# zhizdev/mvdfusion

Hardware: AMD Instinct MI355X
Metric: denoising-steps/sec (higher is better)
Workload: dtype f16x3 (f16 MFMA operands split hi+lo, 3 partial products, fp32 accumulate); 1 GPU; BASELINE.json configs[1]: V=4 views x 256^2 images (32x32 latents), D=1, 50-step DDIM (eta 1), cfg 2.5, SD1.x UNet 320ch + 10 view-aligned transformers + GridAttn, random-init (deterministic fill) weights; views=4, latent=32, depth_samples=1, parallelism=single GPU, CFG pair batched as 2V, hipgraph=True, gemm_tuning=mvdfusion_amd/tuned/gemm_f16.json: 426 problems; 0 problems tuned in this run

## Files before the change

### include/mvd_hip.h

```cpp
#ifndef MVD_HIP_H
#define MVD_HIP_H
#include <stddef.h>
#include <stdint.h>
#ifdef __cplusplus
extern "C" {
#endif

typedef void* mvd_stream_t;

#define MVD_VERSION 100
#define MVD_PREC_X1 1
#define MVD_PREC_X3 3
#define MVD_PREC_X4 4

int mvd_version(void);
const char* mvd_last_error(void);
int mvd_operand_format(void);

size_t mvd_packed_weight_bytes(int N, int K);
int mvd_pack_linear_weight(const float* w, int N, int K, int ldw, int geglu, float scale, void* packed,
                           mvd_stream_t stream);
int mvd_pack_linear_weight_t(const float* wt, int N, int K, int ldw, float scale, void* packed, mvd_stream_t stream);
int mvd_pack_conv3x3_weight(const float* w, int Cout, int Cin, int cin_pad, float scale, void* packed,
                            mvd_stream_t stream);
// ... 22 lines not shown
  int start_after;
  int consumer;
} mvd_prefetch_item;

typedef struct mvd_gemm_desc {
  int M, N, K;
  const void* A;
  int lda;
  int a_mode;
  int B, Hin, Win, Cin, Hout, Wout, stride, upsample;
  int no_pad_tl;
  const void* Wp;
  int b_mode;
  int ldb;
  float acc_scale;
  int prec;
  int epi;
  int act;
  float* out;
  int ldo;
  void* out_sp;
  int ldp;
  int n_store;
  const float* bias;
  const float* bias_b;
  int rows_per_batch;
  int ldbb;
  const float* colscale;
  const float* res;
  int ldr;
  void *q_hi, *q_lo, *k_hi, *k_lo, *vt_hi, *vt_lo;
  int heads, dhead, L, Lpad;
  float qscale;
  int splitk;
  float* workspace;
  size_t workspace_elems;
  int cfg;
  long long* gn_stats;
  int gn_hw, gn_groups;
  float* rs_out;
  int* rs_count;
  int rs_ld;
  const float* ln_stats;
  const int* ln_count;
  const float* ln_colsum;
  int ln_ld, ln_dim;
  float ln_eps;
  void* gna_out_sp;
  const float* gna_gamma;
  const float* gna_beta;
  float gna_eps;
  int gna_flags;
  const float* cat_b;
  int cat_cb;
  void* cat_raw_sp;
  const float* acc_scale_dev;
  const struct mvd_prefetch_item_s* pf_items;
  int pf_n;
  int tap_mode;
  const void* A2;
  int lda2, Cin2;
} mvd_gemm_desc;
#define MVD_TAPS_FULL 0
#define MVD_TAPS_UP4 1
#define MVD_TAPS_CENTRE_TAIL 2
#define MVD_GNA_SILU 1
#define MVD_GNA_ROUND_F16 2
#define MVD_GNA_OUT_UNUSED 4

int mvd_gemm(const mvd_gemm_desc* d, mvd_stream_t stream);
int mvd_gemm_cfg_supported(const mvd_gemm_desc* d, int cfg);

int mvd_split_planes(const float* x, void* sp, size_t rows, int cols, int ldx, int ldp, mvd_stream_t stream);
int mvd_split_planes_scaled(const float* x, void* sp, size_t rows, int cols, int ldx, int ldp, const float* scale_dev, mvd_stream_t stream);

int mvd_gemv(const float* W, const float* bias, const float* x, float* y, int M, int N, int K, int ldx, int ldy,
             int act_in, int act_out, mvd_stream_t stream);

int mvd_groupnorm_chunks(int HW);
int mvd_groupnorm_nhwc(const float* x, void* y_sp, const float* gamma, const float* beta, int B, int HW, int C,
                       int groups, float eps, int silu, double* ws, size_t ws_elems, mvd_stream_t stream);
int mvd_groupnorm_from_stats(const float* x, void* y_sp, const float* gamma, const float* beta, const long long* stats, int B, int HW,
                             int C, int groups, float eps, int silu, mvd_stream_t stream);
int mvd_softmax_rows(const float* x, void* y_sp, int rows, int cols, int ldx, float scale, float out_scale,
                     mvd_stream_t stream);

int mvd_layernorm(const float* x, void* y_sp, float* y_f32, const float* w, const float* b, int rows, int C, float eps,
                  int w_plus_one, mvd_stream_t stream);
int mvd_layernorm_groups(const float* x, void* y_sp, float* y_f32, const float* w, const float* b, int ldw, int rows, int rows_per_group,
                         int C, float eps, int w_plus_one, mvd_stream_t stream);

size_t mvd_attn_qk_plane_elems(int B, int heads, int L, int dhead);
size_t mvd_attn_vt_plane_elems(int B, int heads, int L, int dhead);
int mvd_attn_lpad(int L);
int mvd_attention(const void* q_hi, const void* q_lo, const void* k_hi, const void* k_lo, const void* vt_hi,
                  const void* vt_lo, void* out_sp, int ldo, int B, int heads, int L, int Lkeys, int dhead, int prec,
                  mvd_stream_t stream);

int mvd_pixel_cross_attn(const float* q, const float* k, const float* v, void* out_sp, int P, int D, int heads,
                         int dhead, mvd_stream_t stream);

int mvd_unet_input(const float* x, const float* input_latents, void* out_sp, int V, int S, int cpad, int cfg,
                   mvd_stream_t stream);
int mvd_unet_input_scenes(const float* x, const float* input_latents, void* out_sp, int nscene, int V, int S, int cpad, int cfg,
                          mvd_stream_t stream);
int mvd_concat_channels(const float* a, int Ca, const float* b, int Cb, float* out, void* out_sp, int rows, long long* gn_stats,
                        int gn_hw, int gn_groups, mvd_stream_t stream);
int mvd_concat_groupnorm_fits(int Ca, int Cb, int hw, int groups);
int mvd_concat_groupnorm(const float* a, int Ca, const float* b, int Cb, float* out, void* raw_sp, void* y_sp, const float* gamma,
                         const float* beta, long long* gn_stats, int B, int hw, int groups, float eps, int silu, mvd_stream_t stream);
int mvd_area_pool(const float* vol, void* out_sp, int B, int S, int D, int C, int factor, int ldp, mvd_stream_t stream);
int mvd_fill_zero(float* p, size_t n, mvd_stream_t stream);

#define MVD_STEP_STRIDE 8
int mvd_timestep_embedding(const float* steps, const int* iter, const float* freqs, float* out, int dim,
                           mvd_stream_t stream);
int mvd_timestep_embedding_scenes(const float* steps, const int* iter, const float* freqs, float* out, int dim, int nscene,
                                  int steps_scene_stride, mvd_stream_t stream);
int mvd_advance_iter(int* iter, mvd_stream_t stream);

#define MVD_CAM_RECORD 20
#define MVD_TOKEN_DIM 723
#define MVD_TOKEN_LD 736
int mvd_zembed(const float* lat, const float* w, const float* b, float* feat, int N, int S, mvd_stream_t stream);
int mvd_gridattn_tokens(const float* x, const float* depth_noise, const float* steps, const int* iter,
                        const float* grid_lin ,
                        const float* feat, const float* in_feat, const float* cams, const float* in_cam,
                        void* tokens_sp, int V, int q0, int Vq, int S, int D, float depth_scale, float depth_shift,
                        mvd_stream_t stream);
int mvd_gridattn_tokens_scenes(const float* x, const float* depth_noise, const float* steps, const int* iter, const float* grid_lin,
                               const float* feat, const float* in_feat, const float* cams, const float* in_cam, void* tokens_sp,
                               int nscene, int V, int q0, int Vq, int S, int D, float depth_scale, float depth_shift,
                               mvd_stream_t stream);
int mvd_gridattn_tokens_scenes_t(const float* x, const float* depth_noise, const float* steps, const int* iter, const float* grid_lin,
                                 const float* feat, const float* in_feat, const float* cams, const float* in_cam, void* tokens_sp,
                                 int nscene, int V, int q0, int Vq, int S, int D, float depth_scale, float depth_shift,
                                 int steps_scene_stride, mvd_stream_t stream);
int mvd_gridattn_fused_slots(void);
size_t mvd_gridattn_fused_stream_bytes(void);
size_t mvd_gridattn_fused_vec_floats(void);
int mvd_gridattn_fused(const float* x, const float* depth_noise, const float* steps, const int* iter, const float* grid_lin,
                       const float* feat, const float* in_feat, const float* cams, const float* in_cam, const void* wstream,
                       const float* vecs, void* pooled_sp, int V, int q0, int Vq, int S, int D, float depth_scale,
                       float depth_shift, int prec ,
                       mvd_stream_t stream);
int mvd_gridattn_fused_scenes(const float* x, const float* depth_noise, const float* steps, const int* iter, const float* grid_lin,
                              const float* feat, const float* in_feat, const float* cams, const float* in_cam, const void* wstream,
                              const float* vecs, void* pooled_sp, int nscene, int V, int q0, int Vq, int S, int D, float depth_scale,
                              float depth_shift, int prec, mvd_stream_t stream);
int mvd_gridattn_fused_scenes_t(const float* x, const float* depth_noise, const float* steps, const int* iter, const float* grid_lin,
                                const float* feat, const float* in_feat, const float* cams, const float* in_cam, const void* wstream,
                                const float* vecs, void* pooled_sp, int nscene, int V, int q0, int Vq, int S, int D, float depth_scale,
                                float depth_shift, int prec, int steps_scene_stride, int vecs_scene_stride, mvd_stream_t stream);
int mvd_gridattn_tokens_window(const float* x, const float* depth_noise, const float* steps, const int* iter, const float* grid_lin,
                               const float* feat, const float* in_feat, const float* cams, const float* in_cam, void* tokens_sp,
                               int nscene, int V, int q0, int Vq, int S, int D, float depth_scale, float depth_shift,
                               int steps_scene_stride, int window, mvd_stream_t stream);
int mvd_gridattn_fused_window(const float* x, const float* depth_noise, const float* steps, const int* iter, const float* grid_lin,
                              const float* feat, const float* in_feat, const float* cams, const float* in_cam, const void* wstream,
                              const float* vecs, void* pooled_sp, int nscene, int V, int q0, int Vq, int S, int D, float depth_scale,
                              float depth_shift, int prec, int steps_scene_stride, int vecs_scene_stride, int window,
                              mvd_stream_t stream);
int mvd_view_mha(const float* qkv, void* out_sp, int Nseq, int V, int heads, int dhead,
                 mvd_stream_t stream);
int mvd_view_pool(const float* x, const float* w, const float* b, void* out_sp, int Nseq, int V, int C,
                  mvd_stream_t stream);

int mvd_cfg_ddim_update(const float* eps_nhwc, int ldc, float* x, float* x0, float* eps_out,
                        const float* ddim_noise, size_t noise_stride ,
                        const float* steps, const int* iter, int V, int S, int cfg, float cfg_scale, int do_update,
                        mvd_stream_t stream);

int mvd_pin_views(float* x, float* x0, const float* known, const float* noise, size_t noise_stride ,
                  const float* steps, const int* iter, int groups, int group_views, int K, int S, int mode, mvd_stream_t stream);

#define MVD_FUSE_FOREGROUND 1
#define MVD_FUSE_STAGE_AUTO 0
#define MVD_FUSE_STAGE_GLOBAL 1
#define MVD_FUSE_STAGE_LDS 2
int mvd_fuse_points(const float* lat, const float* rgb, const float* cams, const float* ndc_lin, float* xyz, float* color,
                    uint8_t* support, uint8_t* conflict, uint8_t* flags, int nscene, int V, int S, int up, float depth_scale,
                    float depth_shift, float lo, float hi, float tau, int stage, mvd_stream_t stream);
size_t mvd_compact_points_scratch(size_t npts);
int mvd_compact_points(const float* xyz, const float* color, const uint8_t* support, const uint8_t* conflict, const uint8_t* flags,
                       size_t npts, int min_support, int max_conflicts, float* out_xyz, float* out_color, uint8_t* out_support,
                       int* out_index, unsigned* count, void* scratch, size_t scratch_bytes, mvd_stream_t stream);

#define MVD_SPLAT_MAX_RADIUS 4
#define MVD_RENDER_FILL 1
#define MVD_RENDER_SPLAT 2
#define MVD_RENDER_RESOLVE 4
#define MVD_RENDER_ALL 7
size_t mvd_render_points_scratch(int ncam, int P);
int mvd_render_points(const float* xyz, const float* color, const int* scene_start, const float* cams, size_t n, int nscene, int M, int P,
                      int radius, float znear, float empty_depth, const float* background, int* index, float* depth, float* rgb,
                      void* scratch, size_t scratch_bytes, mvd_stream_t stream);
int mvd_render_points_stages(const float* xyz, const float* color, const int* scene_start, const float* cams, size_t n, int nscene, int M,
                             int P, int radius, float znear, float empty_depth, const float* background, int* index, float* depth,
                             float* rgb, void* scratch, size_t scratch_bytes, int stages, mvd_stream_t stream);

size_t mvd_render_mesh_scratch(int ncam, int P);
int mvd_render_mesh(const float* vertices, const float* colors, const int* faces, const int* vertex_start, const int* face_start,
// ... 106 lines not shown
```

### mvdfusion_amd/csrc/elementwise.hip

```cpp
#include "common.hpp"
#include "../../include/mvd_hip.h"

namespace {

__device__ __forceinline__ float act_apply(float v, int act) {
  if (act == MVD_ACT_GELU) return gelu_erf(v);
  if (act == MVD_ACT_SILU) return silu_f(v);
  return v;
}

template <int MR>
__global__ __launch_bounds__(256) void gemv_kernel(const float* __restrict__ W, const float* __restrict__ bias,
                                                   const float* __restrict__ x, float* __restrict__ y, int M, int N, int K, int ldx,
                                                   int ldy, int act_in, int act_out) {
  const int lane = threadIdx.x & 63;
  const int n = blockIdx.x * 4 + (threadIdx.x >> 6);
  if (n >= N) return;
  float acc[MR];
#pragma unroll
  for (int m = 0; m < MR; ++m) acc[m] = 0.f;
  const float* wr = W + (size_t)n * K;
  if ((K & 3) == 0) {
    for (int k = lane * 4; k < K; k += 256) {
      const float4 w4 = *(const float4*)(wr + k);
// ... 41 lines not shown
    const int b = (int)(e / ((size_t)cpad * SS));
    const int v = b < V ? b : b - V;
    float o = 0.f;
    if (c < 5) {
      o = x[((size_t)v * 5 + c) * SS + pix];
    } else if (c < 10 && b < V) {
      const float t = il[((size_t)(b / Vs) * 5 + (c - 5)) * SS + pix];
      o = (c < 9) ? t / 0.18215f : t;
    }
    store_sp1(out_sp, e / cpad, cpad, c, o);
  }
}

__global__ __launch_bounds__(256) void concat_kernel(const float4* __restrict__ a, int ca4, const float4* __restrict__ b, int cb4,
                                                     float4* __restrict__ out, u16* __restrict__ out_sp, size_t rows) {
  const int c4 = ca4 + cb4;
  const size_t total = rows * c4;
  for (size_t e = (size_t)blockIdx.x * 256 + threadIdx.x; e < total; e += (size_t)gridDim.x * 256) {
    const size_t r = e / c4;
    const int c = (int)(e - r * c4);
    const float4 v = c < ca4 ? a[r * ca4 + c] : b[r * cb4 + (c - ca4)];
    out[e] = v;
    if (out_sp) store_sp4(out_sp, r, c4 * 4, c * 4, v.x, v.y, v.z, v.w);
  }
}

__global__ __launch_bounds__(256) void concat_stats_kernel(const float4* __restrict__ a, int ca4, const float4* __restrict__ b, int cb4,
                                                           float4* __restrict__ out, u16* __restrict__ out_sp, long long* __restrict__ stats,
                                                           int hw, int groups) {
  __shared__ float cs[2][4][256];
  const int c4n = ca4 + cb4, C = c4n * 4;
  const size_t m0 = (size_t)blockIdx.x * 16;
  const int n0 = blockIdx.y * 256;
  const int c4 = blockIdx.y * 64 + (threadIdx.x & 63), rg = threadIdx.x >> 6;
  float4 s = make_float4(0.f, 0.f, 0.f, 0.f), q = make_float4(0.f, 0.f, 0.f, 0.f);
  if (c4 < c4n) {
    float4 v[4];
#pragma unroll
    for (int r = 0; r < 4; ++r) {
      const size_t row = m0 + rg * 4 + r;
      v[r] = c4 < ca4 ? a[row * ca4 + c4] : b[row * cb4 + (c4 - ca4)];
    }
#pragma unroll
    for (int r = 0; r < 4; ++r) {
      const size_t row = m0 + rg * 4 + r;
      out[row * c4n + c4] = v[r];
      if (out_sp) store_sp4(out_sp, row, C, c4 * 4, v[r].x, v[r].y, v[r].z, v[r].w);
      s.x += v[r].x; s.y += v[r].y; s.z += v[r].z; s.w += v[r].w;
      q.x += v[r].x * v[r].x; q.y += v[r].y * v[r].y; q.z += v[r].z * v[r].z; q.w += v[r].w * v[r].w;
    }
  }
  *(float4*)&cs[0][rg][(threadIdx.x & 63) * 4] = s;
  *(float4*)&cs[1][rg][(threadIdx.x & 63) * 4] = q;
  __syncthreads();
  const int c = threadIdx.x, nn = n0 + c;
  const float cs_ = cs[0][0][c] + cs[0][1][c] + cs[0][2][c] + cs[0][3][c];
  const float cq_ = cs[1][0][c] + cs[1][1][c] + cs[1][2][c] + cs[1][3][c];
  __syncthreads();
  cs[0][0][c] = cs_;
  cs[1][0][c] = cq_;
  __syncthreads();
  if (nn >= C) return;
  const int cg = C / groups;
  const int g = nn / cg, pos = nn - g * cg;
  if (c != 0 && pos != 0) return;
  int len = cg - pos;
  if (len > 256 - c) len = 256 - c;
  float ss = 0.f, qq = 0.f;
  for (int j = 0; j < len; ++j) {
    ss += cs[0][0][c + j];
    qq += cs[1][0][c + j];
  }
  gn_stats_add(stats, (int)(m0 / hw), g, groups, ss, qq);
}

#define MVD_CGN_THREADS 1024
__global__ __launch_bounds__(MVD_CGN_THREADS) void concat_gn_kernel(const float* __restrict__ a, int ca, const float* __restrict__ b, int cb,
                                                                    float* __restrict__ out, u16* __restrict__ raw_sp, u16* __restrict__ y_sp,
                                                                    const float* __restrict__ gamma, const float* __restrict__ beta,
                                                                    long long* __restrict__ stats, int hw, int groups, float eps, int flags) {
  constexpr int NT = MVD_CGN_THREADS, NWV = NT / 64, U = 4;
  extern __shared__ float s_val[];
  __shared__ double s_red[2][NWV];
  __shared__ float s_coef[2][128];
  const int C = ca + cb, cg = C / groups, cg2 = cg >> 1;
  int g, img;
  {
    const int bid = blockIdx.x;
    if ((groups & 7) == 0) {
      const int gpx = groups >> 3, x = bid & 7, r = bid >> 3;
      g = x * gpx + r % gpx;
      img = r / gpx;
    } else {
      g = bid % groups;
      img = bid / groups;
    }
  }
  const int tid = threadIdx.x, lane = tid & 63, wave = tid >> 6;
  const int c0 = g * cg;
  const size_t m0 = (size_t)img * hw;
  const int total = hw * cg2;
  const int dq = NT / cg2, dj = NT - dq * cg2;
  const int rs = tid / cg2, js = tid - rs * cg2;
  const int r0 = tid < total ? rs : 0, j0 = tid < total ? js : 0;
  float s = 0.f, q = 0.f;
  {
    int r = rs, j = js;
    for (int e0 = tid; e0 < total; e0 += NT * U) {
      float2 v[U];
      int rr[U], jj[U];
      bool ok[U];
#pragma unroll
      for (int u = 0; u < U; ++u) {
        ok[u] = e0 + u * NT < total;
        rr[u] = ok[u] ? r : r0;
        jj[u] = ok[u] ? j : j0;
        r += dq;
        j += dj;
        if (j >= cg2) {
          j -= cg2;
          ++r;
        }
      }
#pragma unroll
      for (int u = 0; u < U; ++u) {
        const size_t m = m0 + rr[u];
        const int n = c0 + 2 * jj[u];
        v[u] = *(const float2*)(n < ca ? a + m * ca + n : b + m * cb + (n - ca));
      }
#pragma unroll
      for (int u = 0; u < U; ++u) {
        if (ok[u]) {
          const size_t m = m0 + rr[u];
          const int n = c0 + 2 * jj[u];
          if (out) *(float2*)(out + m * C + n) = v[u];
          if (raw_sp) {
            uint32_t hh, ll;
            split_op16x2(v[u].x, v[u].y, hh, ll);
            u16* pp = raw_sp + sp_index(m, C, n);
            *(uint32_t*)pp = hh;
            *(uint32_t*)(pp + 32) = ll;
          }
          *(float2*)(s_val + 2 * (e0 + u * NT)) = v[u];
          s += v[u].x + v[u].y;
          q += v[u].x * v[u].x + v[u].y * v[u].y;
        }
      }
    }
  }
  {
    const double sd = wave_sum_d((double)s), qd = wave_sum_d((double)q);
    if (lane == 0) {
      s_red[0][wave] = sd;
      s_red[1][wave] = qd;
    }
  }
  __syncthreads();
  double S1 = 0.0, S2 = 0.0;
#pragma unroll
  for (int w = 0; w < NWV; ++w) {
    S1 += s_red[0][w];
    S2 += s_red[1][w];
  }
  const double cnt = (double)hw * cg;
  const double mean = S1 / cnt;
  double var = S2 / cnt - mean * mean;
  if (var < 0.0) var = 0.0;
  const float rstd = (float)(1.0 / sqrt(var + (double)eps));
  if (tid < cg) {
    const float aa = rstd * gamma[c0 + tid];
    s_coef[0][tid] = aa;
    s_coef[1][tid] = beta[c0 + tid] - (float)mean * aa;
  }
  if (tid == 0 && stats) gn_stats_add(stats, img, g, groups, (float)S1, (float)S2);
  __syncthreads();
  {
    int r = rs, j = js;
    for (int e = tid; e < total; e += NT) {
      float2 v = *(const float2*)(s_val + 2 * e);
      v.x = v.x * s_coef[0][2 * j] + s_coef[1][2 * j];
      v.y = v.y * s_coef[0][2 * j + 1] + s_coef[1][2 * j + 1];
      if (flags & 2) {
        v.x = (float)(_Float16)v.x;
        v.y = (float)(_Float16)v.y;
      }
      if (flags & 1) {
        v.x = silu_f(v.x);
        v.y = silu_f(v.y);
      }
      uint32_t hh, ll;
      split_op16x2(v.x, v.y, hh, ll);
      u16* pp = y_sp + sp_index(m0 + r, C, c0 + 2 * j);
      *(uint32_t*)pp = hh;
      *(uint32_t*)(pp + 32) = ll;
      r += dq;
      j += dj;
      if (j >= cg2) {
        j -= cg2;
        ++r;
      }
    }
  }
}

__global__ __launch_bounds__(256) void area_pool_kernel(const float4* __restrict__ vol, u16* __restrict__ out_sp, int B, int S,
                                                        int D, int C4, int f, int ldp) {
  const int So = S / f;
  const size_t total = (size_t)B * So * So * D * C4;
  const float inv = 1.0f / (float)(f * f);
  for (size_t e = (size_t)blockIdx.x * 256 + threadIdx.x; e < total; e += (size_t)gridDim.x * 256) {
    const int c = (int)(e % C4);
    size_t r = e / C4;
    const int d = (int)(r % D);
    r /= D;
    const int ox = (int)(r % So);
    r /= So;
    const int oy = (int)(r % So);
    const int b = (int)(r / So);
    float4 acc = make_float4(0.f, 0.f, 0.f, 0.f);
    for (int dy = 0; dy < f; ++dy)
#pragma unroll 8
      for (int dx = 0; dx < f; ++dx) {
        const float4 v = vol[((((size_t)b * S + oy * f + dy) * S + ox * f + dx) * D + d) * C4 + c];
        acc.x += v.x;
        acc.y += v.y;
        acc.z += v.z;
        acc.w += v.w;
      }
    store_sp4(out_sp, e / C4, ldp, c * 4, acc.x * inv, acc.y * inv, acc.z * inv, acc.w * inv);
  }
}

__global__ __launch_bounds__(256) void fill_zero_kernel(float* p, size_t n) {
  for (size_t e = (size_t)blockIdx.x * 256 + threadIdx.x; e < n; e += (size_t)gridDim.x * 256) p[e] = 0.f;
}

__global__ void timestep_embedding_kernel(const float* __restrict__ steps, const int* __restrict__ iter,
                                          const float* __restrict__ freqs, float* __restrict__ out, int dim, int steps_scene_stride) {
  const float t = steps[((size_t)iter[0] + (size_t)blockIdx.x * steps_scene_stride) * MVD_STEP_STRIDE + 0];
  out += (size_t)blockIdx.x * dim;
  const int half = dim / 2;
  for (int i = threadIdx.x; i < half; i += blockDim.x) {
    const float a = t * freqs[i];
    out[i] = cosf(a);
    out[half + i] = sinf(a);
  }
}

__global__ void advance_iter_kernel(int* iter) {
  if (threadIdx.x == 0) iter[0] += 1;
}

__global__ __launch_bounds__(256) void cfg_ddim_kernel(const float* __restrict__ eps_nhwc, int ldc, float* __restrict__ x,
                                                       float* __restrict__ x0, float* __restrict__ eps_out,
                                                       const float* __restrict__ noise, const float* __restrict__ steps,
                                                       const int* __restrict__ iter, int V, int S, int cfg, float cfg_scale,
                                                       int do_update, size_t noise_stride) {
  const int it = iter[0];
  const float* st = steps + (size_t)it * MVD_STEP_STRIDE;
  const float a_t = st[3], a_prev = st[4], sigma = st[5], s1m = st[6], has_noise = st[7];
  const int SS = S * S;
  const size_t total = (size_t)V * 5 * SS;
  for (size_t e = (size_t)blockIdx.x * 256 + threadIdx.x; e < total; e += (size_t)gridDim.x * 256) {
    const int pix = (int)(e % SS);
    const int c = (int)((e / SS) % 5);
    const int b = (int)(e / ((size_t)5 * SS));
    float ep = eps_nhwc[((size_t)b * SS + pix) * ldc + c];
    if (cfg) {
      const float eu = eps_nhwc[((size_t)(V + b) * SS + pix) * ldc + c];
      ep = eu + cfg_scale * (ep - eu);
    }
    if (eps_out) eps_out[e] = ep;
    if (do_update) {
      const float xv = x[e];
      const float px0 = (xv - s1m * ep) / sqrtf(a_t);
      const float dir = sqrtf(fmaxf(1.0f - a_prev - sigma * sigma, 1e-7f)) * ep;
      float xp = sqrtf(a_prev) * px0 + dir;
      if (has_noise != 0.f) xp = xp + sigma * noise[(size_t)it * noise_stride + e];
      x0[e] = px0;
      x[e] = xp;
    }
  }
}

template <typename T>
__device__ __forceinline__ T pin_axpy(float sa, const T& k, float s1, const T& n);
template <>
__device__ __forceinline__ float pin_axpy<float>(float sa, const float& k, float s1, const float& n) {
  return sa * k + s1 * n;
}
template <>
__device__ __forceinline__ float4 pin_axpy<float4>(float sa, const float4& k, float s1, const float4& n) {
  return make_float4(sa * k.x + s1 * n.x, sa * k.y + s1 * n.y, sa * k.z + s1 * n.z, sa * k.w + s1 * n.w);
}

template <typename T>
__global__ __launch_bounds__(256) void pin_views_kernel(T* __restrict__ x, T* __restrict__ x0, const T* __restrict__ known,
                                                        const T* __restrict__ noise, size_t nstride, const float* __restrict__ steps,
                                                        const int* __restrict__ iter, int group_views, int K, size_t rowlen, size_t total,
                                                        int mode) {
  float sa = 1.f, s1 = 0.f;
  size_t nbase = 0;
  if (mode == 1) {
    const int it = iter[0];
    const float* st = steps + (size_t)it * MVD_STEP_STRIDE;
    sa = st[1];
    s1 = st[6];
    nbase = (size_t)it * nstride;
  }
  for (size_t e = (size_t)blockIdx.x * 256 + threadIdx.x; e < total; e += (size_t)gridDim.x * 256) {
    const size_t p = e / rowlen;
    const size_t off = e - p * rowlen;
    const size_t dst = ((p / K) * group_views + p % K) * rowlen + off;
    const T kv = known[e];
    if (mode == 1) {
      x[dst] = pin_axpy<T>(sa, kv, s1, noise[nbase + e]);
      x0[dst] = kv;
    } else {
      x[dst] = kv;
    }
  }
}

inline int grid_for(size_t total, int cap = 2048) {
  size_t b = (total + 255) / 256;
  if (b > (size_t)cap) b = cap;
  if (b < 1) b = 1;
  return (int)b;
}

}

extern "C" int mvd_gemv(const float* W, const float* bias, const float* x, float* y, int M, int N, int K, int ldx, int ldy,
// ... 42 lines not shown
                       (const float4*)b, Cb / 4, (float4*)out, (u16*)out_sp, gn_stats, gn_hw, gn_groups);
    MVD_CHECK_LAUNCH("mvd_concat_channels/stats");
    return 0;
  }
  const size_t total = (size_t)rows * (Ca + Cb) / 4;
  hipLaunchKernelGGL(concat_kernel, dim3(grid_for(total)), dim3(256), 0, (hipStream_t)stream, (const float4*)a, Ca / 4,
                     (const float4*)b, Cb / 4, (float4*)out, (u16*)out_sp, (size_t)rows);
  MVD_CHECK_LAUNCH("mvd_concat_channels");
  return 0;
}

extern "C" int mvd_concat_groupnorm_fits(int Ca, int Cb, int hw, int groups) {
  const int C = Ca + Cb;
  if (groups <= 0 || C % groups || (Ca & 1) || (Cb & 1)) return 0;
  const int cg = C / groups;
  return (cg & 1) == 0 && cg <= 128 && (size_t)hw * cg * 4 <= 128 * 1024 ? 1 : 0;
}

extern "C" int mvd_concat_groupnorm(const float* a, int Ca, const float* b, int Cb, float* out, void* raw_sp, void* y_sp, const float* gamma,
                                    const float* beta, long long* gn_stats, int B, int hw, int groups, float eps, int silu,
                                    mvd_stream_t stream) {
  MVD_CHECK_ARG(a && b && y_sp && gamma && beta && B > 0 && hw > 0, "mvd_concat_groupnorm: null pointer / bad shape");
  MVD_CHECK_ARG((Ca + Cb) % 32 == 0 && mvd_concat_groupnorm_fits(Ca, Cb, hw, groups),
                "mvd_concat_groupnorm: needs (Ca+Cb) %% 32 == 0, even Ca / Cb / group width <= 128 and hw * (C / groups) * 4 <= 128 KiB of LDS "
                "(Ca=%d Cb=%d hw=%d groups=%d): use mvd_concat_channels + mvd_groupnorm_from_stats", Ca, Cb, hw, groups);
  MVD_CHECK_ARG(((uintptr_t)a & 7) == 0 && ((uintptr_t)b & 7) == 0 && ((uintptr_t)out & 7) == 0 && ((uintptr_t)y_sp & 127) == 0 &&
                    ((uintptr_t)raw_sp & 127) == 0, "mvd_concat_groupnorm: alignment");
  const size_t lds = (size_t)hw * ((Ca + Cb) / groups) * 4;
  {
    static unsigned long long raised = 0;
    const hipError_t e = mvd_raise_dynamic_lds((const void*)concat_gn_kernel, 128 * 1024, &raised);
    MVD_CHECK_ARG(e == hipSuccess, "mvd_concat_groupnorm: hipFuncSetAttribute(MaxDynamicSharedMemorySize): %s", hipGetErrorString(e));
  }
  hipLaunchKernelGGL(concat_gn_kernel, dim3(B * groups), dim3(MVD_CGN_THREADS), lds, (hipStream_t)stream, a, Ca, b, Cb, out, (u16*)raw_sp,
                     (u16*)y_sp, gamma, beta, gn_stats, hw, groups, eps, silu);
  MVD_CHECK_LAUNCH("mvd_concat_groupnorm");
  return 0;
}

extern "C" int mvd_area_pool(const float* vol, void* out_sp, int B, int S, int D, int C, int factor, int ldp,
                             mvd_stream_t stream) {
  MVD_CHECK_ARG(vol && out_sp && C % 32 == 0 && B > 0 && S > 0 && D > 0 && C % 4 == 0 && factor >= 1 && S % factor == 0,
                "mvd_area_pool: bad arguments");
  if (ldp == 0) ldp = C;
  MVD_CHECK_ARG(ldp >= C && ldp % 32 == 0 && ((uintptr_t)out_sp & 127) == 0, "mvd_area_pool: ldp=%d must be >= C, %% 32 == 0", ldp);
  const int So = S / factor;
  const size_t total = (size_t)B * So * So * D * (C / 4);
  hipLaunchKernelGGL(area_pool_kernel, dim3(grid_for(total)), dim3(256), 0, (hipStream_t)stream, (const float4*)vol,
                     (u16*)out_sp, B, S, D, C / 4, factor, ldp);
  MVD_CHECK_LAUNCH("mvd_area_pool");
  return 0;
}

extern "C" int mvd_fill_zero(float* p, size_t n, mvd_stream_t stream) {
  MVD_CHECK_ARG(p != nullptr, "mvd_fill_zero: null pointer");
  if (n == 0) return 0;
  hipLaunchKernelGGL(fill_zero_kernel, dim3(grid_for(n)), dim3(256), 0, (hipStream_t)stream, p, n);
  MVD_CHECK_LAUNCH("mvd_fill_zero");
  return 0;
}

extern "C" int mvd_timestep_embedding(const float* steps, const int* iter, const float* freqs, float* out, int dim,
                                      mvd_stream_t stream) {
  MVD_CHECK_ARG(steps && iter && freqs && out && dim > 0 && dim % 2 == 0, "mvd_timestep_embedding: bad arguments");
  hipLaunchKernelGGL(timestep_embedding_kernel, dim3(1), dim3(256), 0, (hipStream_t)stream, steps, iter, freqs, out, dim, 0);
  MVD_CHECK_LAUNCH("mvd_timestep_embedding");
  return 0;
}

extern "C" int mvd_timestep_embedding_scenes(const float* steps, const int* iter, const float* freqs, float* out, int dim, int nscene,
                                             int steps_scene_stride, mvd_stream_t stream) {
  MVD_CHECK_ARG(steps && iter && freqs && out && dim > 0 && dim % 2 == 0, "mvd_timestep_embedding: bad arguments");
  MVD_CHECK_ARG(nscene >= 1 && nscene <= 65535 && steps_scene_stride >= 0 && (nscene > 1 || steps_scene_stride == 0),
                "mvd_timestep_embedding_scenes: nscene=%d (1 ... 65535), steps_scene_stride=%d (>= 0; 0 when nscene = 1)", nscene,
                steps_scene_stride);
  hipLaunchKernelGGL(timestep_embedding_kernel, dim3(nscene), dim3(256), 0, (hipStream_t)stream, steps, iter, freqs, out, dim,
                     steps_scene_stride);
  MVD_CHECK_LAUNCH("mvd_timestep_embedding_scenes");
  return 0;
}

extern "C" int mvd_advance_iter(int* iter, mvd_stream_t stream) {
  MVD_CHECK_ARG(iter != nullptr, "mvd_advance_iter: null pointer");
  hipLaunchKernelGGL(advance_iter_kernel, dim3(1), dim3(64), 0, (hipStream_t)stream, iter);
  MVD_CHECK_LAUNCH("mvd_advance_iter");
  return 0;
}

extern "C" int mvd_cfg_ddim_update(const float* eps_nhwc, int ldc, float* x, float* x0, float* eps_out,
                                   const float* ddim_noise, size_t noise_stride, const float* steps, const int* iter, int V,
                                   int S, int cfg, float cfg_scale, int do_update, mvd_stream_t stream) {
  MVD_CHECK_ARG(eps_nhwc && steps && iter && V > 0 && S > 0 && ldc >= 5, "mvd_cfg_ddim_update: bad arguments");
  if (do_update) MVD_CHECK_ARG(x && x0 && ddim_noise, "mvd_cfg_ddim_update: update needs x, x0, ddim_noise");
  const size_t total = (size_t)V * 5 * S * S;
  hipLaunchKernelGGL(cfg_ddim_kernel, dim3(grid_for(total)), dim3(256), 0, (hipStream_t)stream, eps_nhwc, ldc, x, x0, eps_out,
                     ddim_noise, steps, iter, V, S, cfg, cfg_scale, do_update, noise_stride);
  MVD_CHECK_LAUNCH("mvd_cfg_ddim_update");
  return 0;
}

extern "C" int mvd_pin_views(float* x, float* x0, const float* known, const float* noise, size_t noise_stride, const float* steps,
                             const int* iter, int groups, int group_views, int K, int S, int mode, mvd_stream_t stream) {
  MVD_CHECK_ARG(x && known && groups > 0 && group_views > 0 && S > 0 && (mode == 0 || mode == 1),
                "mvd_pin_views: bad arguments (null x / known, groups=%d, group_views=%d, S=%d, mode=%d)", groups, group_views, S, mode);
  MVD_CHECK_ARG(K > 0 && K <= group_views, "mvd_pin_views: K=%d pinned views of a %d-view group (0 < K <= group_views)", K, group_views);
  MVD_CHECK_ARG((long long)groups * group_views <= 0x3fffffff, "mvd_pin_views: groups * group_views too large");
  const size_t row = (size_t)5 * S * S;
  if (mode == 1)
    MVD_CHECK_ARG(x0 && noise && steps && iter && noise_stride >= (size_t)groups * K * row,
                  "mvd_pin_views: mode 1 needs x0, noise, steps, iter and noise_stride >= groups * K * 5 * S * S");
  const size_t total = (size_t)groups * K * row;
  hipStream_t s = (hipStream_t)stream;
  if (((size_t)S * S) % 4 == 0) {
    MVD_CHECK_ARG(((uintptr_t)x & 15) == 0 && ((uintptr_t)known & 15) == 0, "mvd_pin_views: x / known must be 16-byte aligned");
    if (mode == 1)
      MVD_CHECK_ARG(((uintptr_t)x0 & 15) == 0 && ((uintptr_t)noise & 15) == 0 && noise_stride % 4 == 0,
                    "mvd_pin_views: x0 / noise must be 16-byte aligned and noise_stride a multiple of 4");
    hipLaunchKernelGGL(pin_views_kernel<float4>, dim3(grid_for(total / 4)), dim3(256), 0, s, (float4*)x, (float4*)x0, (const float4*)known,
                       (const float4*)noise, noise_stride / 4, steps, iter, group_views, K, row / 4, total / 4, mode);
  } else {
    hipLaunchKernelGGL(pin_views_kernel<float>, dim3(grid_for(total)), dim3(256), 0, s, x, x0, known, noise, noise_stride, steps, iter,
                       group_views, K, row, total, mode);
  }
  MVD_CHECK_LAUNCH("mvd_pin_views");
  return 0;
}
```

### mvdfusion_amd/csrc/gemm.hip

```cpp
#include "gemm_device.hpp"

namespace {

__global__ __launch_bounds__(256) void splitk_reduce_kernel(GemmParams p) {
  const mvd_gemm_desc& d = p.d;
  const size_t MN = (size_t)d.M * d.N;
  if (d.epi == MVD_EPI_GEGLU) {
    const size_t total = (size_t)d.M * (d.N >> 1);
    for (size_t e = (size_t)blockIdx.x * 256 + threadIdx.x; e < total; e += (size_t)gridDim.x * 256) {
      const int m = (int)(e / (d.N >> 1));
      const int col = (int)(e - (size_t)m * (d.N >> 1));
      const int pv = (col >> 4) * 32 + (col & 15);
      float v = 0.f, g = 0.f;
      for (int z = 0; z < p.splits; ++z) {
        v += d.workspace[z * MN + (size_t)m * d.N + pv];
        g += d.workspace[z * MN + (size_t)m * d.N + pv + 16];
      }
      epi_geglu_elem(d, m, pv, v, g);
    }
    return;
  }
  if (d.epi == MVD_EPI_STORE) {
    const size_t MN4 = MN >> 2;
    const float inv = 1.0f / gemm_acc_scale(d);
// ... 27 lines not shown
}

__global__ __launch_bounds__(256) void splitk_reduce_rows_kernel(GemmParams p) {
  const mvd_gemm_desc& d = p.d;
  const size_t MN = (size_t)d.M * d.N;
  const int lane = threadIdx.x & 63;
  const int m = blockIdx.x * 4 + (threadIdx.x >> 6);
  const int n = blockIdx.y * 256 + lane * 4;
  if (m >= d.M) return;
  float s1 = 0.f, q1 = 0.f;
  if (n < d.N) {
    float4 v = make_float4(0.f, 0.f, 0.f, 0.f);
    const float* w = d.workspace + (size_t)m * d.N + n;
    for (int z = 0; z < p.splits; ++z) {
      const float4 t = *(const float4*)(w + z * MN);
      v.x += t.x; v.y += t.y; v.z += t.z; v.w += t.w;
    }
    const float4 f = epi_store4(d, m, n, v);
    s1 = (f.x + f.y) + (f.z + f.w);
    q1 = (f.x * f.x + f.y * f.y) + (f.z * f.z + f.w * f.w);
  }
  s1 = wave_sum(s1);
  q1 = wave_sum(q1);
  if (lane == 0) *((float2*)d.rs_out + (size_t)m * d.rs_ld + blockIdx.y) = make_float2(s1, q1);
  if (blockIdx.x == 0 && blockIdx.y == 0 && threadIdx.x == 0) d.rs_count[0] = gridDim.y;
}

template <int RPT>
__global__ __launch_bounds__(256) void splitk_reduce_stats_kernel(GemmParams p) {
  __shared__ float cs[2][4][256];
  const mvd_gemm_desc& d = p.d;
  const size_t MN = (size_t)d.M * d.N;
  const int m0 = blockIdx.x * (4 * RPT), n0 = blockIdx.y * 256;
  const int c4 = threadIdx.x & 63, rg = threadIdx.x >> 6;
  const int n = n0 + c4 * 4;
  float4 s = make_float4(0.f, 0.f, 0.f, 0.f), q = make_float4(0.f, 0.f, 0.f, 0.f);
  if (n < d.N) {
    float4 v[RPT];
#pragma unroll
    for (int r = 0; r < RPT; ++r) v[r] = make_float4(0.f, 0.f, 0.f, 0.f);
    const float* w = d.workspace + (size_t)(m0 + rg * RPT) * d.N + n;
#pragma unroll 2
    for (int z = 0; z < p.splits; ++z) {
#pragma unroll
      for (int r = 0; r < RPT; ++r) {
        const float4 t = *(const float4*)(w + z * MN + (size_t)r * d.N);
        v[r].x += t.x; v[r].y += t.y; v[r].z += t.z; v[r].w += t.w;
      }
    }
#pragma unroll
    for (int r = 0; r < RPT; ++r) v[r] = epi_value4(d, m0 + rg * RPT + r, n, v[r]);
#pragma unroll
    for (int r = 0; r < RPT; ++r) {
      const float4 f = v[r];
      epi_put4(d, m0 + rg * RPT + r, n, f);
      s.x += f.x; s.y += f.y; s.z += f.z; s.w += f.w;
      q.x += f.x * f.x; q.y += f.y * f.y; q.z += f.z * f.z; q.w += f.w * f.w;
    }
  }
  *(float4*)&cs[0][rg][c4 * 4] = s;
  *(float4*)&cs[1][rg][c4 * 4] = q;
  __syncthreads();
  const int c = threadIdx.x, nn = n0 + c;
  const float cs_ = cs[0][0][c] + cs[0][1][c] + cs[0][2][c] + cs[0][3][c];
  const float cq_ = cs[1][0][c] + cs[1][1][c] + cs[1][2][c] + cs[1][3][c];
  __syncthreads();
  cs[0][0][c] = cs_;
  cs[1][0][c] = cq_;
  __syncthreads();
  if (nn >= d.N) return;
  const int cg = d.N / d.gn_groups;
  const int g = nn / cg, pos = nn - g * cg;
  if (c != 0 && pos != 0) return;
  int len = cg - pos;
  if (len > 256 - c) len = 256 - c;
  float ss = 0.f, qq = 0.f;
  for (int j = 0; j < len; ++j) {
    ss += cs[0][0][c + j];
    qq += cs[1][0][c + j];
  }
  gn_stats_add(d.gn_stats, m0 / d.gn_hw, g, d.gn_groups, ss, qq);
}

#define MVD_GNK_THREADS 1024
__global__ __launch_bounds__(MVD_GNK_THREADS) void splitk_gn_kernel(GemmParams p) {
  constexpr int NT = MVD_GNK_THREADS, NWV = NT / 64, U = 3, ZC = 4;
  extern __shared__ float s_val[];
  __shared__ double s_red[2][NWV];
  __shared__ float s_coef[2][128];
  const mvd_gemm_desc& d = p.d;
  const int G = d.gn_groups, HW = d.gn_hw;
  const int CT = d.N + (d.cat_b ? d.cat_cb : 0);
  const int cg = CT / G, cg2 = cg >> 1;
  int g, b;
  {
    const int bid = blockIdx.x;
    if ((G & 7) == 0) {
      const int gpx = G >> 3, x = bid & 7, r = bid >> 3;
      g = x * gpx + r % gpx;
      b = r / gpx;
    } else {
      g = bid % G;
      b = bid / G;
    }
  }
  const int tid = threadIdx.x, lane = tid & 63, wave = tid >> 6;
  const int c0 = g * cg, m0 = b * HW;
  const size_t MN = (size_t)d.M * d.N;
  const int total = HW * cg2;
  const bool put_out = d.out != nullptr && !(d.gna_flags & MVD_GNA_OUT_UNUSED);
  const int dq = NT / cg2, dj = NT - dq * cg2;
  const int rs = tid / cg2, js = tid - rs * cg2;
  const int r0 = tid < total ? rs : 0, j0 = tid < total ? js : 0;
  const float* const zero2 = (const float*)g_zero_page;
  const bool has_bias = d.bias != nullptr, has_bb = d.bias_b != nullptr, has_res = d.res != nullptr;
  const float ascale = gemm_acc_scale(d);
  float s = 0.f, q = 0.f;
  {
    int r = rs, j = js;
    for (int e0 = tid; e0 < total; e0 += NT * U) {
      int rr[U], jj[U];
      bool ok[U];
#pragma unroll
      for (int u = 0; u < U; ++u) {
        ok[u] = e0 + u * NT < total;
        rr[u] = ok[u] ? r : r0;
        jj[u] = ok[u] ? j : j0;
        r += dq;
        j += dj;
        if (j >= cg2) {
          j -= cg2;
          ++r;
        }
      }
      float2 acc[U], tb[U], tbb[U], tr[U];
      float2 t[ZC][U];
      const int nz0 = p.splits < ZC ? p.splits : ZC;
      bool own[U];
      float2 tc[U];
#pragma unroll
      for (int u = 0; u < U; ++u) {
        const int m = m0 + rr[u], nn = c0 + 2 * jj[u];
        own[u] = nn < d.N;
        const int n = own[u] ? nn : 0;
        tb[u] = *(const float2*)(has_bias ? d.bias + n : zero2);
        tbb[u] = *(const float2*)(has_bb ? d.bias_b + (size_t)(m / d.rows_per_batch) * d.ldbb + n : zero2);
        tr[u] = *(const float2*)(has_res ? d.res + (size_t)m * d.ldr + n : zero2);
        tc[u] = *(const float2*)(own[u] ? zero2 : d.cat_b + (size_t)m * d.cat_cb + (nn - d.N));
#pragma unroll
        for (int z = 0; z < ZC; ++z) {
          const float* w = d.workspace + (size_t)(z < nz0 ? z : 0) * MN + (size_t)m * d.N + n;
          t[z][u] = *(const float2*)w;
        }
      }
#pragma unroll
      for (int u = 0; u < U; ++u) {
        acc[u] = make_float2(0.f, 0.f);
#pragma unroll
        for (int z = 0; z < ZC; ++z)
          if (z < nz0) {
            acc[u].x += t[z][u].x;
            acc[u].y += t[z][u].y;
          }
      }
      for (int zb = ZC; zb < p.splits; zb += ZC) {
        const int nz = p.splits - zb < ZC ? p.splits - zb : ZC;
#pragma unroll
        for (int u = 0; u < U; ++u) {
          const int m = m0 + rr[u], n = own[u] ? c0 + 2 * jj[u] : 0;
#pragma unroll
          for (int z = 0; z < ZC; ++z) t[z][u] = *(const float2*)(d.workspace + (size_t)(zb + (z < nz ? z : 0)) * MN + (size_t)m * d.N + n);
        }
#pragma unroll
        for (int u = 0; u < U; ++u)
#pragma unroll
          for (int z = 0; z < ZC; ++z)
            if (z < nz) {
              acc[u].x += t[z][u].x;
              acc[u].y += t[z][u].y;
            }
      }
#pragma unroll
      for (int u = 0; u < U; ++u) {
        float2 v = acc[u];
        v.x = v.x * ascale + tb[u].x + tbb[u].x + tr[u].x;
        v.y = v.y * ascale + tb[u].y + tbb[u].y + tr[u].y;
        if (!own[u]) v = tc[u];
        if (ok[u]) {
          const int m = m0 + rr[u], n = c0 + 2 * jj[u];
          if (put_out && own[u]) *(float2*)(d.out + (size_t)m * d.ldo + n) = v;
          if (d.cat_raw_sp) {
            uint32_t hh, ll;
            split_op16x2(v.x, v.y, hh, ll);
            u16* pp = (u16*)d.cat_raw_sp + sp_index((size_t)m, CT, n);
            *(uint32_t*)pp = hh;
            *(uint32_t*)(pp + 32) = ll;
          }
          *(float2*)(s_val + 2 * (e0 + u * NT)) = v;
          s += v.x + v.y;
          q += v.x * v.x + v.y * v.y;
        }
      }
    }
  }
  unsigned pf_sink = 0;
  if (d.pf_items != nullptr) {
    const __attribute__((address_space(4))) mvd_prefetch_item* tab = (const __attribute__((address_space(4))) mvd_prefetch_item*)d.pf_items;
    const int gw = blockIdx.x * NWV + wave, GW = gridDim.x * NWV;
    for (int it = 0; it < d.pf_n; ++it) {
      const unsigned char* base = (const unsigned char*)tab[it].ptr;
      const long lines = (long)((tab[it].bytes + 127) >> 7);
      for (long l = (long)gw * 64 + lane; l < lines; l += (long)GW * 64) {
        const unsigned char* a = base + (l << 7);
        asm volatile("global_load_dword %0, %1, off" : "+v"(pf_sink) : "v"(a) : "memory");
      }
    }
  }
  {
    const double sd = wave_sum_d((double)s), qd = wave_sum_d((double)q);
    if (lane == 0) {
      s_red[0][wave] = sd;
      s_red[1][wave] = qd;
    }
  }
  __syncthreads();
  double S1 = 0.0, S2 = 0.0;
#pragma unroll
  for (int w = 0; w < NWV; ++w) {
    S1 += s_red[0][w];
    S2 += s_red[1][w];
  }
  const double cnt = (double)HW * cg;
  const double mean = S1 / cnt;
  double var = S2 / cnt - mean * mean;
  if (var < 0.0) var = 0.0;
  const float rstd = (float)(1.0 / sqrt(var + (double)d.gna_eps));
  if (tid < cg) {
    const float a = rstd * d.gna_gamma[c0 + tid];
    s_coef[0][tid] = a;
    s_coef[1][tid] = d.gna_beta[c0 + tid] - (float)mean * a;
  }
  if (tid == 0 && d.gn_stats) gn_stats_add(d.gn_stats, b, g, G, (float)S1, (float)S2);
  __syncthreads();
  u16* const ysp = (u16*)d.gna_out_sp;
  const int fl = d.gna_flags;
  {
    int r = rs, j = js;
    for (int e = tid; e < total; e += NT) {
      float2 v = *(const float2*)(s_val + 2 * e);
      v.x = v.x * s_coef[0][2 * j] + s_coef[1][2 * j];
      v.y = v.y * s_coef[0][2 * j + 1] + s_coef[1][2 * j + 1];
      if (fl & MVD_GNA_ROUND_F16) {
        v.x = (float)(_Float16)v.x;
        v.y = (float)(_Float16)v.y;
      }
      if (fl & MVD_GNA_SILU) {
        v.x = silu_f(v.x);
        v.y = silu_f(v.y);
      }
      uint32_t hh, ll;
      split_op16x2(v.x, v.y, hh, ll);
      u16* pp = ysp + sp_index((size_t)(m0 + r), CT, c0 + 2 * j);
      *(uint32_t*)pp = hh;
      *(uint32_t*)(pp + 32) = ll;
      r += dq;
      j += dj;
      if (j >= cg2) {
        j -= cg2;
        ++r;
      }
    }
  }
  asm volatile("" ::"v"(pf_sink));
}

struct TileInfo {
  int bm, bn, waves;
  int cores_plain, cores_pipe;
};
static const TileInfo kTiles[MVD_GEMM_TILES] = {{64, 64, 4, 5, 3}, {128, 128, 8, 2, 1}, {128, 80, 4, 2, 2}, {64, 80, 4, 4, 3},
                                                {128, 160, 8, 1, 1}};

static int choose_splits(long tiles, int nk, const TileInfo& ti, int loop, size_t mn) {
  const double area = (double)ti.bm * ti.bn / (128.0 * 128.0);
  const double t_mfma = 0.75 * area;
  const double t_lat = loop == 0 ? 1.0 : (loop == 1 ? 0.4 : (loop == 2 ? 0.2 : (loop == 5 ? 0.05 : 0.1)));
  const double t_epi = 0.27 + 1.73 * area;
  const int coresident = loop == 0 ? ti.cores_plain : (loop == 1 ? ti.cores_pipe : (loop == 4 && ti.waves == 4 ? 2 : 1));
  const double red_fixed = 6.0, red_per_split = (double)mn * 8.0 / 3.0e12 / 0.7e-6;
  int best = 1;
  double best_t = 1e30;
  const int smax = nk / 8 < 1 ? 1 : (nk / 8 > 32 ? 32 : nk / 8);
  for (int sp = 1; sp <= smax; ++sp) {
    const int iters = (nk + sp - 1) / sp;
    if ((long)iters * (sp - 1) >= nk) continue;
    const long per_cu = (tiles * sp + 255) / 256;
    const long rounds = (per_cu + coresident - 1) / coresident;
    const double busy = (double)per_cu * (iters * t_mfma + t_epi);
    const double lat = (double)rounds * (iters * t_lat + t_epi);
    double t = busy > lat ? busy : lat;
    if (sp > 1) t += red_fixed + sp * red_per_split;
    if (t < best_t * 0.97) {
      best_t = t;
      best = sp;
    }
  }
  return best;
}

static int patch_shares(const mvd_gemm_desc& d, const TileInfo& ti) {
  if (d.a_mode != MVD_A_CONV3X3 || d.b_mode != MVD_B_PACKED || d.stride != 1 || d.upsample || d.no_pad_tl) return 0;
  if (d.tap_mode != MVD_TAPS_FULL) return 0;
  if (d.Hin != d.Hout || d.Win != d.Wout || ti.bm != 128) return 0;
  const int W = d.Wout, HW = d.Hout * d.Wout;
  if (ti.bm % W != 0 || (HW >= ti.bm ? HW % ti.bm != 0 : ti.bm % HW != 0)) return 0;
  const int nseg = HW >= ti.bm ? 1 : ti.bm / HW, Rb = HW >= ti.bm ? ti.bm / W : d.Hout;
  const int P = nseg * (Rb + 2) * (W + 2);
  if (P > MVD_PATCH_SLOTS_MAX) return 0;
  const int PG = (P + 7) / 8, cap = (11 - conv_patch_ring(ti.bn, ti.waves)) * ti.waves;
  return PG <= cap ? 1 : (PG <= 2 * cap ? 2 : 0);
}

static bool cfg_supported(const mvd_gemm_desc& d, int cfg) {
  if (cfg == 0) return true;
  if (cfg < 0 || cfg > MVD_GEMM_CFG_STRIDE * MVD_GEMM_TILES) return false;
  const int tile = (cfg - 1) / MVD_GEMM_CFG_STRIDE, loop = ((cfg - 1) % MVD_GEMM_CFG_STRIDE) >> 1;
  if (loop >= MVD_GEMM_LOOPS) return false;
  if (tile >= 2 && d.epi != MVD_EPI_STORE) return false;
  if (d.a_mode == MVD_A_CONV3X3 && d.tap_mode == MVD_TAPS_UP4 && (d.epi != MVD_EPI_STORE || !d.upsample)) return false;
  const int waves = kTiles[tile].waves;
  if ((loop == 2 || loop == 3) && waves != 8) return false;
  if (loop == 3 || loop >= 8) return false;
  if (loop == 5 && waves != 4) return false;
  if (loop == 6) return (tile == 1 || tile == 2 || tile == 4) && patch_shares(d, kTiles[tile]) > 0;
  if (loop == 7) return tile == 1 || ((tile == 2 || tile == 4) && d.epi == MVD_EPI_STORE);
  return true;
}

}

extern "C" int mvd_gemm_cfg_supported(const mvd_gemm_desc* dp, int cfg) { return dp && cfg_supported(*dp, cfg) ? 1 : 0; }

extern "C" int mvd_gemm(const mvd_gemm_desc* dp, mvd_stream_t stream) {
  MVD_CHECK_ARG(dp != nullptr, "mvd_gemm: null descriptor");
  GemmParams p;
  p.d = *dp;
  p.up4_tpp = p.up4_mq = 0;
  mvd_gemm_desc& d = p.d;
  MVD_CHECK_ARG(d.M > 0 && d.N > 0 && d.K > 0, "mvd_gemm: bad sizes M=%d N=%d K=%d", d.M, d.N, d.K);
  MVD_CHECK_ARG(d.K % 32 == 0, "mvd_gemm: K=%d must be a multiple of 32 (pad the packed weight)", d.K);
  MVD_CHECK_ARG(d.N % 16 == 0, "mvd_gemm: N=%d must be a multiple of 16 (pad the packed weight)", d.N);
  MVD_CHECK_ARG(d.prec == MVD_PREC_X1 || d.prec == MVD_PREC_X3 || d.prec == MVD_PREC_X4, "mvd_gemm: bad prec %d", d.prec);
  MVD_CHECK_ARG(d.A && d.Wp, "mvd_gemm: null operand");
  MVD_CHECK_ARG(((uintptr_t)d.A & 127) == 0 && ((uintptr_t)d.Wp & 127) == 0, "mvd_gemm: operands must be 128-byte aligned");
  if (d.a_mode == MVD_A_CONV3X3) {
    MVD_CHECK_ARG(d.tap_mode == MVD_TAPS_FULL || d.tap_mode == MVD_TAPS_CENTRE_TAIL || d.tap_mode == MVD_TAPS_UP4,
                  "mvd_gemm: tap_mode %d is not served", d.tap_mode);
    const bool tail = d.tap_mode == MVD_TAPS_CENTRE_TAIL, up4 = d.tap_mode == MVD_TAPS_UP4;
    if (up4) {
      MVD_CHECK_ARG(d.upsample == 1 && d.stride == 1 && !d.no_pad_tl && d.b_mode == MVD_B_PACKED,
                    "mvd_gemm: tap_mode MVD_TAPS_UP4 (the four-tap form) serves stride-1 padded convolutions behind a nearest-2x upsample with a packed weight");
      MVD_CHECK_ARG(d.epi == MVD_EPI_STORE, "mvd_gemm: tap_mode MVD_TAPS_UP4 (the four-tap form) serves MVD_EPI_STORE only (epi=%d)", d.epi);
      MVD_CHECK_ARG(!d.res && !d.bias_b && !d.colscale && !d.rs_out,
                    "mvd_gemm: tap_mode MVD_TAPS_UP4 (the four-tap form) takes no res, bias_b, colscale or rs_out (its tile rows are not output rows)");
      if (d.gn_stats)
        MVD_CHECK_ARG((d.Hin * d.Win) % 16 == 0, "mvd_gemm: tap_mode MVD_TAPS_UP4 (the four-tap form) with gn_stats needs Hin * Win %% 16 == 0 (Hin=%d Win=%d)", d.Hin,
                      d.Win);
    }
    if (tail) {
      MVD_CHECK_ARG(d.A2 != nullptr && ((uintptr_t)d.A2 & 127) == 0 && d.Cin2 > 0 && d.Cin2 % 32 == 0 && d.lda2 >= d.Cin2 && d.lda2 % 32 == 0,
                    "mvd_gemm: the centre-tap tail needs A2 (128-byte aligned), Cin2 %% 32 == 0 and lda2 >= Cin2, a multiple of 32 (Cin2=%d lda2=%d)",
                    d.Cin2, d.lda2);
      MVD_CHECK_ARG(d.stride == 1 && !d.upsample && !d.no_pad_tl && d.Hin == d.Hout && d.Win == d.Wout && d.b_mode == MVD_B_PACKED,
                    "mvd_gemm: the centre-tap tail serves stride-1 padded convolutions with Hin == Hout, Win == Wout and a packed weight");
      MVD_CHECK_ARG((long long)d.M * 2 * d.lda2 < (1ll << 31), "mvd_gemm: A2 is addressed with 32-bit offsets (M=%d lda2=%d)", d.M, d.lda2);
    }
    MVD_CHECK_ARG(d.Cin % 32 == 0 && d.K == (up4 ? 4 : 9) * d.Cin + (tail ? d.Cin2 : 0),
                  "mvd_gemm: conv needs Cin %% 32 == 0 and K == 9*Cin (+ Cin2 with a centre-tap tail; 4*Cin in the four-tap form) (Cin=%d Cin2=%d K=%d)",
                  d.Cin, tail ? d.Cin2 : 0, d.K);
    MVD_CHECK_ARG(d.M == d.B * d.Hout * d.Wout, "mvd_gemm: conv M mismatch");
    MVD_CHECK_ARG(d.stride == 1 || d.stride == 2, "mvd_gemm: conv stride must be 1 or 2");
    if (d.upsample) MVD_CHECK_ARG(d.stride == 1 && d.Hout == 2 * d.Hin && d.Wout == 2 * d.Win, "mvd_gemm: upsample geometry");
  } else {
    MVD_CHECK_ARG(d.a_mode == MVD_A_DENSE, "mvd_gemm: bad a_mode");
    MVD_CHECK_ARG(d.tap_mode == MVD_TAPS_FULL, "mvd_gemm: tap_mode %d needs a_mode == MVD_A_CONV3X3", d.tap_mode);
    MVD_CHECK_ARG(d.lda >= d.K && d.lda % 32 == 0, "mvd_gemm: lda=%d must be >= K=%d and a multiple of 32", d.lda, d.K);
  }
  if (d.out_sp) MVD_CHECK_ARG(d.ldp > 0 && d.ldp % 32 == 0 && ((uintptr_t)d.out_sp & 127) == 0,
                              "mvd_gemm: split-plane output needs ldp %% 32 == 0 and 128-byte alignment");
  if (d.out) MVD_CHECK_ARG(d.ldo % 4 == 0 && ((uintptr_t)d.out & 15) == 0, "mvd_gemm: out must be 16-byte aligned with ldo %% 4 == 0");
  if (d.res) MVD_CHECK_ARG(d.ldr % 4 == 0 && ((uintptr_t)d.res & 15) == 0, "mvd_gemm: res must be 16-byte aligned with ldr %% 4 == 0");
  MVD_CHECK_ARG(((uintptr_t)d.bias & 15) == 0 && ((uintptr_t)d.bias_b & 15) == 0 && ((uintptr_t)d.colscale & 15) == 0,
                "mvd_gemm: bias / bias_b / colscale must be 16-byte aligned");
  if (d.epi == MVD_EPI_STORE) {
    MVD_CHECK_ARG(d.out != nullptr || d.out_sp != nullptr, "mvd_gemm: no output");
    if (d.n_store <= 0 || d.n_store > d.N) d.n_store = d.N;
    if (d.bias_b) {
      MVD_CHECK_ARG(d.rows_per_batch > 0, "mvd_gemm: bias_b needs rows_per_batch");
      if (d.ldbb == 0) d.ldbb = d.N;
      MVD_CHECK_ARG(d.ldbb % 4 == 0, "mvd_gemm: ldbb %% 4 != 0");
    }
  } else if (d.epi == MVD_EPI_GEGLU) {
    MVD_CHECK_ARG((d.out != nullptr || d.out_sp != nullptr) && d.N % 32 == 0, "mvd_gemm: GEGLU needs an output and N %% 32 == 0");
    d.bias_b = nullptr;
  } else if (d.epi == MVD_EPI_QKV) {
    MVD_CHECK_ARG(d.q_hi && d.q_lo && d.k_hi && d.k_lo && d.vt_hi && d.vt_lo, "mvd_gemm: QKV planes missing");
    MVD_CHECK_ARG(d.heads > 0 && d.dhead > 0 && d.N == 3 * d.heads * d.dhead, "mvd_gemm: QKV needs N == 3*heads*dhead");
    MVD_CHECK_ARG(d.L > 0 && d.M % d.L == 0 && d.Lpad >= d.L, "mvd_gemm: QKV needs M %% L == 0");
    MVD_CHECK_ARG(d.dhead % 4 == 0 && d.L % 4 == 0, "mvd_gemm: QKV needs dhead %% 4 == 0 and L %% 4 == 0");
  } else {
    MVD_CHECK_ARG(false, "mvd_gemm: bad epilogue %d", d.epi);
  }
  if (d.rs_out)
    MVD_CHECK_ARG(d.epi == MVD_EPI_STORE && d.n_store == d.N && !d.gn_stats && d.rs_count && d.rs_ld >= cdiv(d.N, 32) && ((uintptr_t)d.rs_out & 7) == 0,
                  "mvd_gemm: rs_out needs MVD_EPI_STORE, n_store == N, no gn_stats, rs_count and rs_ld >= N / 32 (N=%d rs_ld=%d)", d.N, d.rs_ld);
  if (d.ln_stats) {
    MVD_CHECK_ARG((d.epi == MVD_EPI_QKV || d.epi == MVD_EPI_GEGLU) && d.ln_count && d.ln_colsum && d.ln_dim > 0 && d.ln_ld > 0 &&
                      ((uintptr_t)d.ln_stats & 7) == 0 && ((uintptr_t)d.ln_colsum & 15) == 0,
                  "mvd_gemm: ln_stats (LayerNorm fold) serves the QKV / GEGLU epilogues and needs ln_count, ln_colsum, ln_dim, ln_ld");
    d.splitk = 1;
  }
  if (d.gn_stats)
    MVD_CHECK_ARG(d.epi == MVD_EPI_STORE && d.n_store == d.N && d.M % 16 == 0 && d.gn_hw > 0 && d.gn_hw % 16 == 0 && d.gn_groups > 0 &&
                      d.N % d.gn_groups == 0,
                  "mvd_gemm: gn_stats needs MVD_EPI_STORE, n_store == N, M %% 16 == 0, gn_hw %% 16 == 0, N %% gn_groups == 0 (N=%d M=%d hw=%d)",
                  d.N, d.M, d.gn_hw);
  if (d.gna_out_sp)
    MVD_CHECK_ARG(d.gn_stats && d.out && d.ldo == d.N && d.gna_gamma && d.gna_beta && d.N % 32 == 0 && d.M % d.gn_hw == 0 &&
                      ((uintptr_t)d.gna_out_sp & 127) == 0,
                  "mvd_gemm: gna_out_sp (GroupNorm apply behind the GEMM) needs gn_stats, out with ldo == N, gamma / beta, N %% 32 == 0, M %% gn_hw == 0");
  if (d.cat_b)
    MVD_CHECK_ARG(d.gna_out_sp && d.cat_cb > 0 && d.cat_cb % 2 == 0 && (d.N + d.cat_cb) % 32 == 0 && (d.N + d.cat_cb) % d.gn_groups == 0 &&
                      ((uintptr_t)d.cat_b & 7) == 0 && ((uintptr_t)d.cat_raw_sp & 127) == 0 &&
                      mvd_concat_groupnorm_fits(d.N, d.cat_cb, d.gn_hw, d.gn_groups),
                  "mvd_gemm: cat_b (GroupNorm over [out | cat_b]) needs gna_out_sp, an even cat_cb, (N + cat_cb) %% 32 == 0 and a shape "
                  "mvd_concat_groupnorm_fits() accepts (N=%d cat_cb=%d hw=%d)", d.N, d.cat_cb, d.gn_hw);
  long long* const gna_stats = d.gn_stats;
  if (d.cat_b) d.gn_stats = nullptr;
  if (d.b_mode == MVD_B_PLANES)
    MVD_CHECK_ARG(d.ldb >= d.K && d.ldb % 32 == 0, "mvd_gemm: B planes need ldb=%d >= K=%d, a multiple of 32", d.ldb, d.K);
  else
    MVD_CHECK_ARG(d.b_mode == MVD_B_PACKED, "mvd_gemm: bad b_mode %d", d.b_mode);
  if (d.acc_scale == 0.f) d.acc_scale = 1.f;
  p.nk = d.K / 32;
  p.nt16 = d.N / 16;
  int tile, loop = 0, order = -1;
  MVD_CHECK_ARG(d.cfg >= 0 && d.cfg <= MVD_GEMM_CFG_STRIDE * MVD_GEMM_TILES, "mvd_gemm: bad cfg %d", d.cfg);
  if (d.cfg >= 1) {
    tile = (d.cfg - 1) / MVD_GEMM_CFG_STRIDE;
    loop = ((d.cfg - 1) % MVD_GEMM_CFG_STRIDE) >> 1;
    order = (d.cfg - 1) & 1;
    MVD_CHECK_ARG(cfg_supported(d, d.cfg), "mvd_gemm: cfg %d (tile %d, loop %d) does not serve this problem (include/mvd_hip.h: cfg)", d.cfg, tile,
                  loop);
  } else {
    const long tiles128 = (long)cdiv(d.M, 128) * cdiv(d.N, 128);
    tile = (tiles128 >= 128 && (d.N >= 512 || d.K >= 2048)) ? 1 : 0;
  }
  const TileInfo& ti = kTiles[tile];
  p.tiles_n = cdiv(d.N, ti.bn);
  p.tiles_m = cdiv(d.M, ti.bm);
  const bool up4 = d.a_mode == MVD_A_CONV3X3 && d.tap_mode == MVD_TAPS_UP4;
  if (up4) {
    p.up4_mq = d.B * d.Hin * d.Win;
    p.up4_tpp = cdiv(p.up4_mq, ti.bm);
    p.tiles_m = 4 * p.up4_tpp;
  }
  if (order < 0) {
    const int est_tm = up4 ? p.up4_tpp : p.tiles_m;
    const double W = (double)d.N * d.K * 4.0;
    const double A = (double)(up4 ? p.up4_mq : d.M) * d.K * 4.0 / (d.a_mode == MVD_A_CONV3X3 ? (up4 ? 4.0 : 9.0) : 1.0);
    const double rep_m = est_tm < 8 ? est_tm : 8, rep_n = p.tiles_n < 8 ? p.tiles_n : 8;
    order = (W + A * rep_n) < (W * rep_m + A) ? 1 : 0;
  }
  p.m_fastest = order;
  int splits = d.splitk;
  const long tiles = (long)p.tiles_m * p.tiles_n;
  if (splits == 0) splits = choose_splits(tiles, p.nk, ti, loop, (size_t)d.M * d.N);
  if (splits < 1) splits = 1;
  if (splits > p.nk) splits = p.nk;
  if (splits > 1) {
    if (d.workspace == nullptr) splits = 1;
    else {
      const size_t cap = d.workspace_elems / ((size_t)d.M * d.N);
      if ((size_t)splits > cap) splits = cap < 1 ? 1 : (int)cap;
    }
  }
  p.kt_per_split = cdiv(p.nk, splits);
  if (loop == 6) p.kt_per_split = 9 * cdiv(p.nk / 9, splits);
  p.splits = cdiv(p.nk, p.kt_per_split);
  hipStream_t s = (hipStream_t)stream;
  bool launched;
  if (loop == 6) launched = mvd_gemm_launch_patch(tile, p, s, patch_shares(d, ti));
  else if (loop == 7) launched = mvd_gemm_launch_ws(tile, p, s);
  else if (tile == 0) launched = mvd_gemm_launch_plain_t0(loop, p, s);
  else if (tile == 1) launched = mvd_gemm_launch_plain_t1(loop, p, s);
  else if (tile == 2) launched = mvd_gemm_launch_plain_t2(loop, p, s);
  else if (tile == 3) launched = mvd_gemm_launch_plain_t3(loop, p, s);
  else launched = mvd_gemm_launch_plain_t4(loop, p, s);
  MVD_CHECK_ARG(launched, "mvd_gemm: no kernel for tile %d loop %d", tile, loop);
  MVD_CHECK_LAUNCH("mvd_gemm");
  const int gna_ct = d.N + (d.cat_b ? d.cat_cb : 0);
  const int gna_cg = d.gna_out_sp ? gna_ct / d.gn_groups : 0;
  const size_t gna_lds = (size_t)d.gn_hw * gna_cg * 4;
  const bool gna_fused = d.gna_out_sp && p.splits > 1 && !d.rs_out && !d.out_sp && !d.colscale && d.act == MVD_ACT_NONE && (gna_cg & 1) == 0 &&
                         gna_cg <= 128 && gna_lds <= 128 * 1024 && d.ldo % 2 == 0 && (!d.res || d.ldr % 2 == 0) && (!d.bias_b || d.ldbb % 2 == 0) &&
                         d.N % 2 == 0;
  if (gna_fused) {
    {
      static unsigned long long raised = 0;
      const hipError_t e = mvd_raise_dynamic_lds((const void*)splitk_gn_kernel, 128 * 1024, &raised);
      MVD_CHECK_ARG(e == hipSuccess, "mvd_gemm: hipFuncSetAttribute(MaxDynamicSharedMemorySize): %s", hipGetErrorString(e));
    }
    p.d.gn_stats = gna_stats;
    if (loop == 7) p.d.pf_items = nullptr;
    hipLaunchKernelGGL(splitk_gn_kernel, dim3((d.M / d.gn_hw) * d.gn_groups), dim3(MVD_GNK_THREADS), gna_lds, s, p);
    MVD_CHECK_LAUNCH("mvd_gemm/splitk_gn");
    return 0;
  }
  if (p.splits > 1) {
    if (d.rs_out) {
      hipLaunchKernelGGL(splitk_reduce_rows_kernel, dim3(cdiv(d.M, 4), cdiv(d.N, 256)), dim3(256), 0, s, p);
    } else if (d.gn_stats) {
      const int spans = (d.N + 255) / 256;
      if ((d.M / 16) * spans >= 1024)
        hipLaunchKernelGGL(splitk_reduce_stats_kernel<4>, dim3(d.M / 16, spans), dim3(256), 0, s, p);
      else
        hipLaunchKernelGGL(splitk_reduce_stats_kernel<2>, dim3(d.M / 8, spans), dim3(256), 0, s, p);
    } else {
      const size_t total = (size_t)d.M * d.N;
      int blocks = (int)((total + 255) / 256);
      if (blocks > 2048) blocks = 2048;
      hipLaunchKernelGGL(splitk_reduce_kernel, dim3(blocks), dim3(256), 0, s, p);
    }
    MVD_CHECK_LAUNCH("mvd_gemm/splitk_reduce");
  }
  if (d.gna_out_sp && d.cat_b)
    return mvd_concat_groupnorm(d.out, d.N, d.cat_b, d.cat_cb, nullptr, d.cat_raw_sp, d.gna_out_sp, d.gna_gamma, d.gna_beta, gna_stats,
                                d.M / d.gn_hw, d.gn_hw, d.gn_groups, d.gna_eps, d.gna_flags & (MVD_GNA_SILU | MVD_GNA_ROUND_F16), stream);
  if (d.gna_out_sp)
    return mvd_groupnorm_from_stats(d.out, d.gna_out_sp, d.gna_gamma, d.gna_beta, d.gn_stats, d.M / d.gn_hw, d.gn_hw, d.N, d.gn_groups,
                                    d.gna_eps, d.gna_flags & (MVD_GNA_SILU | MVD_GNA_ROUND_F16), stream);
  return 0;
}

namespace {
__global__ __launch_bounds__(256) void pack_kernel(const float* __restrict__ w, u16* __restrict__ out, int N, int K,
                                                   int Np, int Kp, int ldw, int geglu, int conv_cin, int trans,
                                                   float scale) {
  const int nt16 = Np >> 4;
  const size_t total = (size_t)(Kp >> 5) * nt16 * 64;
  for (size_t e = (size_t)blockIdx.x * 256 + threadIdx.x; e < total; e += (size_t)gridDim.x * 256) {
    const size_t mt = e >> 6;
    const int l = (int)(e & 63);
    const int kt = (int)(mt / nt16), nt = (int)(mt - (size_t)kt * nt16);
    const int n = nt * 16 + (l & 15);
    const int k = kt * 32 + (l >> 4) * 8;
    int src_n = n;
    if (geglu) {
      const int blk = n >> 5, within = n & 31;
      src_n = within < 16 ? blk * 16 + within : (N >> 1) + blk * 16 + (within - 16);
    }
    float v[8];
#pragma unroll
    for (int j = 0; j < 8; ++j) v[j] = 0.f;
    if (src_n < N) {
      if (conv_cin > 0) {
        const int cb = kt / 9, tap = kt - cb * 9;
        const int ci0 = cb * 32 + (k & 31);
#pragma unroll
        for (int j = 0; j < 8; ++j)
          if (ci0 + j < conv_cin) v[j] = w[((size_t)src_n * conv_cin + ci0 + j) * 9 + tap];
      } else if (trans) {
#pragma unroll
        for (int j = 0; j < 8; ++j)
          if (k + j < K) v[j] = w[(size_t)(k + j) * ldw + src_n];
      } else {
        const float* src = w + (size_t)src_n * ldw + k;
        if (k + 7 < K && (ldw & 3) == 0 && ((uintptr_t)w & 15) == 0) {
          const float4 a = *(const float4*)src, b = *(const float4*)(src + 4);
          v[0] = a.x; v[1] = a.y; v[2] = a.z; v[3] = a.w; v[4] = b.x; v[5] = b.y; v[6] = b.z; v[7] = b.w;
        } else {
#pragma unroll
          for (int j = 0; j < 8; ++j)
            if (k + j < K) v[j] = src[j];
        }
      }
    }
    union { uint4 q; u16 h[8]; } H, Lo;
#pragma unroll
    for (int j = 0; j < 8; ++j) split_op16(v[j] * scale, H.h[j], Lo.h[j]);
    u16* o = out + mt * 1024 + l * 8;
    *(uint4*)o = H.q;
    *(uint4*)(o + 512) = Lo.q;
  }
}

__global__ __launch_bounds__(256) void split_planes_kernel(const float* __restrict__ x, u16* __restrict__ sp, size_t rows, int cols,
                                                           int ldx, int ldp, const float* __restrict__ scale) {
  const float sc = scale != nullptr ? *scale : 1.f;
  const int c4 = ldp >> 2;
  const size_t total = rows * c4;
  for (size_t e = (size_t)blockIdx.x * 256 + threadIdx.x; e < total; e += (size_t)gridDim.x * 256) {
    const size_t r = e / c4;
    const int c = (int)(e - r * c4) * 4;
    float v[4];
#pragma unroll
    for (int j = 0; j < 4; ++j) v[j] = (c + j) < cols ? x[r * ldx + c + j] * sc : 0.f;
    store_sp4(sp, r, ldp, c, v[0], v[1], v[2], v[3]);
  }
}
}

extern "C" size_t mvd_packed_weight_bytes(int N, int K) {
  const size_t Np = (size_t)((N + 15) & ~15), Kp = (size_t)((K + 31) & ~31);
  return Np * Kp * 4;
}

extern "C" int mvd_operand_format(void) { return MVD_OPERAND_FORMAT; }

extern "C" int mvd_pack_linear_weight(const float* w, int N, int K, int ldw, int geglu, float scale, void* packed,
                                      mvd_stream_t stream) {
  MVD_CHECK_ARG(w && packed && N > 0 && K > 0 && ldw >= K, "mvd_pack_linear_weight: bad arguments");
  if (geglu) MVD_CHECK_ARG(N % 32 == 0, "mvd_pack_linear_weight: geglu needs N %% 32 == 0");
  const int Np = (N + 15) & ~15, Kp = (K + 31) & ~31;
// ... 50 lines not shown
```

### mvdfusion_amd/csrc/norm.hip

```cpp
#include <stdlib.h>
#include "common.hpp"
#include "../../include/mvd_hip.h"

namespace {

constexpr int GN_MAX_C = 2560;

__host__ __device__ inline int gn_chunks(int HW) {
  int c = HW / 8;
  if (c < 1) c = 1;
  if (c > 128) c = 128;
  while (HW % c) --c;
  return c;
}

__global__ __launch_bounds__(256) void gn_stats_kernel(const float* __restrict__ x, double* __restrict__ ws, int HW, int C,
                                                       int groups, int chunks) {
  __shared__ float s_sum[GN_MAX_C];
  __shared__ float s_sq[GN_MAX_C];
  __shared__ float s_part[2][4][GN_MAX_C / 4];
  const int chunk = blockIdx.x, b = blockIdx.y;
  const int rows = HW / chunks;
  const int C4 = C >> 2;
  const int TX = C4 < 256 ? C4 : 256;
// ... 40 lines not shown
      q += (double)s_sq[c];
    }
    double* o = ws + (((size_t)b * chunks + chunk) * groups + threadIdx.x) * 2;
    o[0] = s;
    o[1] = q;
  }
}

__global__ __launch_bounds__(256) void gn_apply_kernel(const float* __restrict__ x, u16* __restrict__ y_sp,
                                                       const float* __restrict__ gamma, const float* __restrict__ beta,
                                                       const double* __restrict__ ws, int HW, int C, int groups, int chunks,
                                                       float eps, int silu) {
  __shared__ float s_a[GN_MAX_C];
  __shared__ float s_b[GN_MAX_C];
  __shared__ double s_ps[8][64], s_pq[8][64];
  __shared__ float s_mean[64];
  __shared__ float s_rstd[64];
  const int chunk = blockIdx.x, b = blockIdx.y;
  const int rows = HW / chunks;
  const int cg = C / groups;
  {
    const int g = threadIdx.x % 32, sl = threadIdx.x / 32;
    for (int gg = g; gg < groups; gg += 32) {
      double s = 0.0, q = 0.0;
      for (int k = sl; k < chunks; k += 8) {
        const double* o = ws + (((size_t)b * chunks + k) * groups + gg) * 2;
        s += o[0];
        q += o[1];
      }
      s_ps[sl][gg] = s;
      s_pq[sl][gg] = q;
    }
  }
  __syncthreads();
  if (threadIdx.x < groups) {
    double s = 0.0, q = 0.0;
    for (int sl = 0; sl < 8; ++sl) {
      s += s_ps[sl][threadIdx.x];
      q += s_pq[sl][threadIdx.x];
    }
    const double n = (double)HW * cg;
    const double mean = s / n;
    double var = q / n - mean * mean;
    if (var < 0.0) var = 0.0;
    s_mean[threadIdx.x] = (float)mean;
    s_rstd[threadIdx.x] = (float)(1.0 / sqrt(var + (double)eps));
  }
  __syncthreads();
  for (int c = threadIdx.x; c < C; c += 256) {
    const int g = c / cg;
    const float a = s_rstd[g] * gamma[c];
    s_a[c] = a;
    s_b[c] = beta[c] - s_mean[g] * a;
  }
  __syncthreads();
  const size_t row0 = (size_t)b * HW + (size_t)chunk * rows;
  const int C4 = C >> 2;
  const int n4 = rows * C4;
  const float4* x4 = (const float4*)(x + row0 * C);
  for (int i = threadIdx.x; i < n4; i += 256) {
    const int r = i / C4;
    const int c = (i - r * C4) * 4;
    float4 v = x4[i];
    v.x = v.x * s_a[c] + s_b[c];
    v.y = v.y * s_a[c + 1] + s_b[c + 1];
    v.z = v.z * s_a[c + 2] + s_b[c + 2];
    v.w = v.w * s_a[c + 3] + s_b[c + 3];
    if (silu & 2) {
      v.x = (float)(_Float16)v.x;
      v.y = (float)(_Float16)v.y;
      v.z = (float)(_Float16)v.z;
      v.w = (float)(_Float16)v.w;
    }
    if (silu & 1) {
      v.x = silu_f(v.x);
      v.y = silu_f(v.y);
      v.z = silu_f(v.z);
      v.w = silu_f(v.w);
    }
    store_sp4(y_sp, row0 + r, C, c, v.x, v.y, v.z, v.w);
  }
}

__global__ __launch_bounds__(256) void gn_apply_stats_kernel(const float* __restrict__ x, u16* __restrict__ y_sp,
                                                             const float* __restrict__ gamma, const float* __restrict__ beta,
                                                             const long long* __restrict__ stats, int HW, int C, int groups, int chunks,
                                                             float eps, int silu) {
  __shared__ float s_a[GN_MAX_C];
  __shared__ float s_b[GN_MAX_C];
  __shared__ float s_mean[64];
  __shared__ float s_rstd[64];
  const int chunk = blockIdx.x, b = blockIdx.y;
  const int rows = HW / chunks;
  const int cg = C / groups;
  if (threadIdx.x < groups) {
    const long long* p = stats + ((size_t)b * groups + threadIdx.x) * 2;
    const double inv = 1.0 / (double)MVD_GN_FIXED_SCALE;
    const double n = (double)HW * cg;
    const double mean = (double)p[0] * inv / n;
    double var = (double)p[1] * inv / n - mean * mean;
    if (var < 0.0) var = 0.0;
    s_mean[threadIdx.x] = (float)mean;
    s_rstd[threadIdx.x] = (float)(1.0 / sqrt(var + (double)eps));
  }
  __syncthreads();
  for (int c = threadIdx.x; c < C; c += 256) {
    const int g = c / cg;
    const float a = s_rstd[g] * gamma[c];
    s_a[c] = a;
    s_b[c] = beta[c] - s_mean[g] * a;
  }
  __syncthreads();
  const size_t row0 = (size_t)b * HW + (size_t)chunk * rows;
  const int C4 = C >> 2;
  const int n4 = rows * C4;
  const float4* x4 = (const float4*)(x + row0 * C);
  for (int i = threadIdx.x; i < n4; i += 256) {
    const int r = i / C4;
    const int c = (i - r * C4) * 4;
    float4 v = x4[i];
    v.x = v.x * s_a[c] + s_b[c];
    v.y = v.y * s_a[c + 1] + s_b[c + 1];
    v.z = v.z * s_a[c + 2] + s_b[c + 2];
    v.w = v.w * s_a[c + 3] + s_b[c + 3];
    if (silu & 2) {
      v.x = (float)(_Float16)v.x;
      v.y = (float)(_Float16)v.y;
      v.z = (float)(_Float16)v.z;
      v.w = (float)(_Float16)v.w;
    }
    if (silu & 1) {
      v.x = silu_f(v.x);
      v.y = silu_f(v.y);
      v.z = silu_f(v.z);
      v.w = silu_f(v.w);
    }
    store_sp4(y_sp, row0 + r, C, c, v.x, v.y, v.z, v.w);
  }
}

__global__ __launch_bounds__(256) void gn_apply_stats_cols_kernel(const float* __restrict__ x, u16* __restrict__ y_sp,
                                                             const float* __restrict__ gamma, const float* __restrict__ beta,
                                                             const long long* __restrict__ stats, int HW, int C, int groups, int rows_per_block,
                                                             int TX, float eps, int silu) {
  const int b = blockIdx.y;
  const int tx = threadIdx.x % TX, ty = threadIdx.x / TX, TY = 256 / TX;
  if (ty >= TY) return;
  const int C4 = C >> 2, cg = C / groups;
  const int col4 = blockIdx.z * TX + tx, c = col4 * 4;
  const int r_end = min(HW, ((int)blockIdx.x + 1) * rows_per_block);
  int r = blockIdx.x * rows_per_block + ty;
  const float4* xp = (const float4*)x + ((size_t)b * HW + r) * C4 + col4;
  const size_t xstep = (size_t)TY * C4;
  float4 v = make_float4(0.f, 0.f, 0.f, 0.f);
  if (r < r_end) v = *xp;
  const float4 gm = *(const float4*)(gamma + c), bt = *(const float4*)(beta + c);
  float a[4], bb[4];
  const float gmv[4] = {gm.x, gm.y, gm.z, gm.w}, btv[4] = {bt.x, bt.y, bt.z, bt.w};
  int gprev = -1;
  float mk = 0.f, rk = 0.f;
#pragma unroll
  for (int k = 0; k < 4; ++k) {
    const int g = (c + k) / cg;
    if (g != gprev) {
      const long long* p = stats + ((size_t)b * groups + g) * 2;
      const double inv = 1.0 / (double)MVD_GN_FIXED_SCALE;
      const double n = (double)HW * cg;
      const double m = (double)p[0] * inv / n;
      double var = (double)p[1] * inv / n - m * m;
      if (var < 0.0) var = 0.0;
      mk = (float)m;
      rk = (float)(1.0 / sqrt(var + (double)eps));
      gprev = g;
    }
    a[k] = rk * gmv[k];
    bb[k] = btv[k] - mk * a[k];
  }
  for (; r < r_end; r += TY) {
    float4 vn = make_float4(0.f, 0.f, 0.f, 0.f);
    if (r + TY < r_end) vn = *(xp + xstep);
    xp += xstep;
    v.x = v.x * a[0] + bb[0];
    v.y = v.y * a[1] + bb[1];
    v.z = v.z * a[2] + bb[2];
    v.w = v.w * a[3] + bb[3];
    if (silu & 2) {
      v.x = (float)(_Float16)v.x;
      v.y = (float)(_Float16)v.y;
      v.z = (float)(_Float16)v.z;
      v.w = (float)(_Float16)v.w;
    }
    if (silu & 1) {
      v.x = silu_f(v.x);
      v.y = silu_f(v.y);
      v.z = silu_f(v.z);
      v.w = silu_f(v.w);
    }
    store_sp4(y_sp, (size_t)b * HW + r, C, c, v.x, v.y, v.z, v.w);
    v = vn;
  }
}

__global__ __launch_bounds__(256) void softmax_rows_kernel(const float* __restrict__ x, u16* __restrict__ y_sp, int rows, int cols,
                                                           int ldx, float scale, float out_scale) {
  const int lane = threadIdx.x & 63;
  const int row = blockIdx.x * 4 + (threadIdx.x >> 6);
  if (row >= rows) return;
  const float4* xr = (const float4*)(x + (size_t)row * ldx);
  const int n4 = cols >> 2;
  float4 v[16];
  float mx = -INFINITY;
#pragma unroll
  for (int i = 0; i < 16; ++i) {
    const int idx = lane + i * 64;
    if (idx < n4) {
      v[i] = xr[idx];
      v[i].x *= scale; v[i].y *= scale; v[i].z *= scale; v[i].w *= scale;
      mx = fmaxf(fmaxf(fmaxf(mx, v[i].x), fmaxf(v[i].y, v[i].z)), v[i].w);
    }
  }
#pragma unroll
  for (int o = 32; o > 0; o >>= 1) mx = fmaxf(mx, __shfl_xor(mx, o, 64));
  float sum = 0.f;
#pragma unroll
  for (int i = 0; i < 16; ++i) {
    const int idx = lane + i * 64;
    if (idx < n4) {
      v[i].x = expf(v[i].x - mx); v[i].y = expf(v[i].y - mx); v[i].z = expf(v[i].z - mx); v[i].w = expf(v[i].w - mx);
      sum += (v[i].x + v[i].y) + (v[i].z + v[i].w);
    }
  }
  sum = wave_sum(sum);
  const float inv = out_scale / sum;
#pragma unroll
  for (int i = 0; i < 16; ++i) {
    const int idx = lane + i * 64;
    if (idx < n4) store_sp4(y_sp, (size_t)row, cols, idx * 4, v[i].x * inv, v[i].y * inv, v[i].z * inv, v[i].w * inv);
  }
}

template <int MAXV>
__global__ __launch_bounds__(256) void ln_kernel(const float* __restrict__ x, u16* __restrict__ y_sp, float* __restrict__ y_f32,
                                                 const float* __restrict__ w, const float* __restrict__ bia, int rows, int C, float eps,
                                                 int w_plus_one, int rows_per_group, int ldw) {
  const int lane = threadIdx.x & 63;
  const int row = blockIdx.x * 4 + (threadIdx.x >> 6);
  if (row >= rows) return;
  const size_t goff = (size_t)(row / rows_per_group) * ldw;
  if (w) w += goff;
  if (bia) bia += goff;
  const int n4 = C >> 2;
  const float4* xr = (const float4*)(x + (size_t)row * C);
  float4 v[MAXV];
  float s = 0.f;
#pragma unroll
  for (int i = 0; i < MAXV; ++i) {
    const int idx = lane + 64 * i;
    if (idx < n4) {
      v[i] = xr[idx];
      s += (v[i].x + v[i].y) + (v[i].z + v[i].w);
    } else {
      v[i] = make_float4(0.f, 0.f, 0.f, 0.f);
    }
  }
  const float mean = wave_sum(s) / (float)C;
  float q = 0.f;
#pragma unroll
  for (int i = 0; i < MAXV; ++i) {
    const int idx = lane + 64 * i;
    if (idx < n4) {
      const float a = v[i].x - mean, b = v[i].y - mean, c = v[i].z - mean, d = v[i].w - mean;
      q += (a * a + b * b) + (c * c + d * d);
    }
  }
  const float rstd = rsqrtf(wave_sum(q) / (float)C + eps);
#pragma unroll
  for (int i = 0; i < MAXV; ++i) {
    const int idx = lane + 64 * i;
    if (idx < n4) {
      float4 o;
      o.x = (v[i].x - mean) * rstd;
      o.y = (v[i].y - mean) * rstd;
      o.z = (v[i].z - mean) * rstd;
      o.w = (v[i].w - mean) * rstd;
      if (w) {
        float4 ww = ((const float4*)w)[idx];
        if (w_plus_one) {
          ww.x += 1.f;
          ww.y += 1.f;
          ww.z += 1.f;
          ww.w += 1.f;
        }
        o.x *= ww.x;
        o.y *= ww.y;
        o.z *= ww.z;
        o.w *= ww.w;
      }
      if (bia) {
        const float4 bb = ((const float4*)bia)[idx];
        o.x += bb.x;
        o.y += bb.y;
        o.z += bb.z;
        o.w += bb.w;
      }
      if (y_sp) store_sp4(y_sp, (size_t)row, C, idx * 4, o.x, o.y, o.z, o.w);
      if (y_f32) ((float4*)(y_f32 + (size_t)row * C))[idx] = o;
    }
  }
}

}

extern "C" int mvd_groupnorm_chunks(int HW) { return gn_chunks(HW); }

extern "C" int mvd_groupnorm_nhwc(const float* x, void* y_sp, const float* gamma, const float* beta, int B, int HW, int C,
                                  int groups, float eps, int silu, double* ws, size_t ws_elems, mvd_stream_t stream) {
  MVD_CHECK_ARG(x && y_sp && gamma && beta && ws, "mvd_groupnorm_nhwc: null pointer");
  MVD_CHECK_ARG(C % 32 == 0, "mvd_groupnorm_nhwc: split-planes output needs C %% 32 == 0 (C=%d)", C);
  MVD_CHECK_ARG(B > 0 && HW > 0 && C > 0 && groups > 0 && groups <= 64 && C % groups == 0, "mvd_groupnorm_nhwc: bad shape");
  MVD_CHECK_ARG(C <= GN_MAX_C && C % 4 == 0, "mvd_groupnorm_nhwc: C=%d must be <= %d and a multiple of 4", C, GN_MAX_C);
  const int chunks = gn_chunks(HW);
  MVD_CHECK_ARG((size_t)B * chunks * groups * 2 <= ws_elems,
                "mvd_groupnorm_nhwc: workspace holds %zu doubles, B*chunks*groups*2 = %zu needed (B=%d, chunks=%d, groups=%d)", ws_elems,
                (size_t)B * chunks * groups * 2, B, chunks, groups);
  hipStream_t s = (hipStream_t)stream;
  hipLaunchKernelGGL(gn_stats_kernel, dim3(chunks, B), dim3(256), 0, s, x, ws, HW, C, groups, chunks);
  MVD_CHECK_LAUNCH("mvd_groupnorm_nhwc/stats");
  hipLaunchKernelGGL(gn_apply_kernel, dim3(chunks, B), dim3(256), 0, s, x, (u16*)y_sp, gamma, beta, ws, HW, C, groups, chunks,
                     eps, silu);
  MVD_CHECK_LAUNCH("mvd_groupnorm_nhwc/apply");
  return 0;
}

extern "C" int mvd_groupnorm_from_stats(const float* x, void* y_sp, const float* gamma, const float* beta, const long long* stats, int B,
                                        int HW, int C, int groups, float eps, int silu, mvd_stream_t stream) {
  MVD_CHECK_ARG(x && y_sp && gamma && beta && stats, "mvd_groupnorm_from_stats: null pointer");
  MVD_CHECK_ARG(C % 32 == 0 && B > 0 && HW > 0 && groups > 0 && groups <= 64 && C % groups == 0 && C <= GN_MAX_C,
                "mvd_groupnorm_from_stats: bad shape (C=%d groups=%d)", C, groups);
  if (!(C <= 320 && HW >= 1024)) {
    const int C4 = C / 4;
    int TX = C4 < 256 ? C4 : 256;
    while (C4 % TX) --TX;
    const int TY = 256 / TX;
    const int rows_per_block = TY * 4;
    hipLaunchKernelGGL(gn_apply_stats_cols_kernel, dim3(cdiv(HW, rows_per_block), B, C4 / TX), dim3(256), 0, (hipStream_t)stream, x,
                       (u16*)y_sp, gamma, beta, stats, HW, C, groups, rows_per_block, TX, eps, silu);
  } else {
    const int chunks = gn_chunks(HW);
    hipLaunchKernelGGL(gn_apply_stats_kernel, dim3(chunks, B), dim3(256), 0, (hipStream_t)stream, x, (u16*)y_sp, gamma, beta, stats, HW, C,
                       groups, chunks, eps, silu);
  }
  MVD_CHECK_LAUNCH("mvd_groupnorm_from_stats");
  return 0;
}

extern "C" int mvd_softmax_rows(const float* x, void* y_sp, int rows, int cols, int ldx, float scale, float out_scale,
                                mvd_stream_t stream) {
  MVD_CHECK_ARG(x && y_sp && rows > 0 && cols > 0, "mvd_softmax_rows: bad arguments");
  MVD_CHECK_ARG(cols % 32 == 0 && cols <= 4096 && ldx % 4 == 0 && ldx >= cols, "mvd_softmax_rows: cols=%d must be a multiple of 32, <= 4096", cols);
  hipLaunchKernelGGL(softmax_rows_kernel, dim3(cdiv(rows, 4)), dim3(256), 0, (hipStream_t)stream, x, (u16*)y_sp, rows, cols, ldx, scale,
                     out_scale);
  MVD_CHECK_LAUNCH("mvd_softmax_rows");
  return 0;
}

extern "C" int mvd_layernorm_groups(const float* x, void* y_sp, float* y_f32, const float* w, const float* b, int ldw, int rows,
                                    int rows_per_group, int C, float eps, int w_plus_one, mvd_stream_t stream) {
  MVD_CHECK_ARG(x && (y_sp || y_f32) && rows > 0, "mvd_layernorm: bad arguments");
  MVD_CHECK_ARG(C % 32 == 0, "mvd_layernorm: split-planes output needs C %% 32 == 0 (C=%d)", C);
  u16* yh = (u16*)y_sp;
  MVD_CHECK_ARG(C % 4 == 0 && C >= 4 && C <= 1280, "mvd_layernorm: C=%d must be a multiple of 4 and <= 1280", C);
  MVD_CHECK_ARG(rows_per_group > 0 && rows % rows_per_group == 0 && ldw >= 0 && ldw % 4 == 0,
                "mvd_layernorm_groups: rows=%d, rows_per_group=%d (must divide rows), ldw=%d (>= 0, a multiple of 4)", rows, rows_per_group, ldw);
  hipStream_t s = (hipStream_t)stream;
  const dim3 grid(cdiv(rows, 4));
  if (C <= 256)
    hipLaunchKernelGGL(ln_kernel<1>, grid, dim3(256), 0, s, x, yh, y_f32, w, b, rows, C, eps, w_plus_one, rows_per_group, ldw);
  else if (C <= 512)
    hipLaunchKernelGGL(ln_kernel<2>, grid, dim3(256), 0, s, x, yh, y_f32, w, b, rows, C, eps, w_plus_one, rows_per_group, ldw);
  else
    hipLaunchKernelGGL(ln_kernel<5>, grid, dim3(256), 0, s, x, yh, y_f32, w, b, rows, C, eps, w_plus_one, rows_per_group, ldw);
  MVD_CHECK_LAUNCH("mvd_layernorm");
  return 0;
}

extern "C" int mvd_layernorm(const float* x, void* y_sp, float* y_f32, const float* w, const float* b, int rows, int C, float eps,
                             int w_plus_one, mvd_stream_t stream) {
  return mvd_layernorm_groups(x, y_sp, y_f32, w, b, 0, rows, rows, C, eps, w_plus_one, stream);
}
```

### mvdfusion_amd/engine.py

```python
import os

import torch

from . import hip


GN_SLOTS = 256
GN_SLOT_ELEMS = 64 * 32 * 2


class Workspace:

    def __init__(self, device):
        self.device = torch.device(device)
        self.bufs = {}
        self.frozen = False

    def get(self, tag, shape, dtype=torch.float32, zero=False):
        key = (tag, tuple(int(s) for s in shape), dtype)
        t = self.bufs.get(key)
        if t is None:
            assert not self.frozen, f"workspace buffer {key} requested during graph capture (the eager warm-up step must " \
                                    "allocate every buffer the captured step uses)"
            t = (torch.zeros if zero else torch.empty)(key[1], dtype=dtype, device=self.device)
            self.bufs[key] = t
        return t

    def planes(self, tag, rows, cols):
        assert cols % 32 == 0, (tag, cols)
        return self.get(tag, (rows, 2 * cols), torch.int16)

    def attn_planes(self, B, heads, L, dhead):
        key = ("attn_planes", B, heads, L, dhead)
        t = self.bufs.get(key)
        if t is None:
            assert not self.frozen, f"attention planes {key} requested during graph capture"
            t = hip.alloc_attn_planes(B, heads, L, dhead, self.device)
            self.bufs[key] = t
        return t

    def nbytes(self):
        n = 0
        for v in self.bufs.values():
            for t in (v if isinstance(v, tuple) else (v,)):
                n += t.numel() * t.element_size()
        return n


class Ctx:
    gn_from_producer = True
    ln_fold = True
    gn_fuse = True

    def __init__(self, device, prec=hip.PREC_X4, policy=None):
        self.device = torch.device(device)
        self.ws = Workspace(device)
        self.prec = prec
        self.policy = dict(policy or {})
        self.B = 0
        self.D = 1
        self.context = None
        self.vol_levels = None
        self.emb_bias = None
        self._rot = {}
        self.capturing = False
        self.gemm_ws = torch.empty(64 * 1024 * 1024, dtype=torch.float32, device=self.device)
        self.gn_arena = torch.zeros(GN_SLOTS * GN_SLOT_ELEMS, dtype=torch.int64, device=self.device)
        self._gn_next = 0
        self._gn = {}
        self._rs = {}
        self.next_gn = None
        self._gn_done = {}
        self._unwritten = set()
        self.next_cat = None
        self._cat_done = set()
        self.keep_fp32 = False

    def begin_step(self):
        self._rot.clear()
        self._gn.clear()
        self._gn_done.clear()
        self._unwritten.clear()
        self._cat_done.clear()
        self.next_gn = None
        self.next_cat = None
        self._gn_next = 0
        if self.gn_from_producer:
            hip.check(hip.lib().mvd_fill_zero(hip.ptr(self.gn_arena), self.gn_arena.numel() * 2, hip.stream()))

    def gn_slot(self, out, B, HW, C):
        n = B * 32 * 2
        if n > GN_SLOT_ELEMS or self._gn_next >= GN_SLOTS:
            return None
        st = self.gn_arena[self._gn_next * GN_SLOT_ELEMS:self._gn_next * GN_SLOT_ELEMS + n]
        self._gn_next += 1
        self._gn[out.data_ptr()] = (st, B, HW, C)
        return st

    def _forget(self, out):
        ptr = out.data_ptr()
        self._gn.pop(ptr, None)
        self._unwritten.discard(ptr)
        if self._gn_done:
            for k in [k for k in self._gn_done if k[0] == ptr]:
                del self._gn_done[k]

    def row_stats(self, tag, rows, width):
        key = (tag, int(rows), int(width))
        rs = self._rs.get(key)
        if rs is None:
            assert not self.ws.frozen, f"row statistics {key} requested during graph capture"
            rs = hip.RowStats(rows, width, self.device)
            self._rs[key] = rs
        return rs

    def act(self, shape):
        key = tuple(int(s) for s in shape)
        i = self._rot.get(key, 0)
        self._rot[key] = (i + 1) % 3
        return self.ws.get(f"act{i}", key)

    def prec_of(self, kind):
        return self.policy.get(kind, self.prec)

    def ln_fold_enabled(self):
        return (self.ln_fold and hip.OPERAND_FORMAT == "f16" and self.prec_of("qkv") >= hip.PREC_X3 and
                self.prec_of("geglu") >= hip.PREC_X3 and self.prec_of("proj") >= hip.PREC_X3)

    def gemm(self, A, W, out, gn=None, kind=None, gn_apply=None, **kw):
        kw.setdefault("prec", self.prec_of(kind))
        kw.setdefault("workspace", self.gemm_ws)
        applied = False
        if out is not None:
            self._forget(out)
            handled = False
            if gn is not None and gn_apply is None and self.next_cat is not None and self.gn_fuse and self.gn_from_producer and \
                    gn[1] % 16 == 0 and out.is_contiguous():
                sk, cat, catp, norm, pname, silu = self.next_cat
                N, cb = out.shape[-1], sk.shape[-1]
                if norm.num_groups == 32 and norm.num_channels == N + cb and sk.shape[0] == out.shape[0] == gn[0] * gn[1] and \
                        sk.is_contiguous() and hip.lib().mvd_concat_groupnorm_fits(N, cb, gn[1], 32):
                    st = self.gn_slot(cat, gn[0], gn[1], N + cb)
                    if st is not None:
                        planes = self.ws.planes(pname, out.shape[0], N + cb)
                        kw.update(gn_stats=st, gn_hw=gn[1], gn_groups=32, cat=(sk, catp),
                                  gn_apply=(norm.weight, norm.bias, norm.eps, (hip.GNA_SILU if silu else 0) | hip.GNA_OUT_UNUSED, planes))
                        self._gn.pop(cat.data_ptr(), None)
                        self._gn_done[(cat.data_ptr(), id(norm))] = (planes, bool(silu))
                        self._unwritten.add(cat.data_ptr())
                        self._unwritten.add(out.data_ptr())
                        self._cat_done.add(cat.data_ptr())
                        handled = True
            if not handled and gn is not None and self.gn_from_producer and gn[1] % 16 == 0 and out.shape[-1] % 32 == 0:
                st = self.gn_slot(out, gn[0], gn[1], out.shape[-1])
                if st is not None:
                    kw.update(gn_stats=st, gn_hw=gn[1], gn_groups=32)
                    if gn_apply is not None and self.gn_fuse and gn_apply[0].num_groups == 32 and out.is_contiguous():
                        norm, planes, silu, unused = gn_apply
                        kw["gn_apply"] = (norm.weight, norm.bias, norm.eps, (hip.GNA_SILU if silu else 0) | (hip.GNA_OUT_UNUSED if unused else 0),
                                          planes)
                        applied = True
                    elif gn_apply is None and self.next_gn is not None and self.gn_fuse and out.is_contiguous():
                        norm, pname, silu = self.next_gn
                        if norm.num_groups == 32 and norm.num_channels == out.shape[-1] and out.shape[0] == gn[0] * gn[1]:
                            planes = self.ws.planes(pname, out.shape[0], out.shape[-1])
                            kw["gn_apply"] = (norm.weight, norm.bias, norm.eps, hip.GNA_SILU if silu else 0, planes)
                            self._gn_done[(out.data_ptr(), id(norm))] = (planes, bool(silu))
        if gn is not None:
            if os.environ.get("MVD_GN_DEBUG") and not self.capturing:
                print(f"[gn] kind={kind} M={out.shape[0]} N={out.shape[-1]} explicit={gn_apply is not None} hint={self.next_gn is not None} "
                      f"cat={self.next_cat is not None} -> fused_apply={'gn_apply' in kw} cat={'cat' in kw}", flush=True)
            if gn_apply is None:
                self.next_gn = None
                self.next_cat = None
        r = hip.gemm(A, W, out, **kw)
        if gn_apply is not None and not applied:
            self.groupnorm(out, gn_apply[1], gn_apply[0], gn[0], gn[1], out.shape[-1], gn_apply[2])
        return r

    def groupnorm(self, x, y, norm, B, HW, C, silu):
        done = self._gn_done.pop((x.data_ptr(), id(norm)), None)
        if done is not None and done[0].data_ptr() == y.data_ptr() and done[0].shape == y.shape and done[1] == bool(silu) and silu in (True, False):
            return y
        if x.data_ptr() in self._unwritten:
            raise RuntimeError("GroupNorm of a tensor whose fused producer left the fp32 data unwritten (Ctx.concat(need_out=False))")
        ent = self._gn.get(x.data_ptr())
        if ent is not None and ent[1:] == (B, HW, C) and norm.num_groups == 32:
            return hip.groupnorm_from_stats(x, y, norm.weight, norm.bias, ent[0], B, HW, C, norm.eps, silu)
        ws = self.ws.get("gn_ws", (B * hip.lib().mvd_groupnorm_chunks(HW) * 32 * 2,), torch.float64)
        return hip.groupnorm(x, y, norm.weight, norm.bias, B, HW, C, norm.eps, silu, ws)

    def concat(self, a, ca, b, cb, out, out_planes, B, HW, gn_apply=None, need_out=True):
        self._forget(out)
        st = None
        if gn_apply is not None and self.gn_fuse and self.gn_from_producer and HW % 16 == 0 and (ca + cb) % 32 == 0 and \
                gn_apply[0].num_groups == 32 and gn_apply[0].num_channels == ca + cb and \
                hip.lib().mvd_concat_groupnorm_fits(ca, cb, HW, 32):
            norm, pname, silu = gn_apply
            st = self.gn_slot(out, B, HW, ca + cb)
            planes = self.ws.planes(pname, B * HW, ca + cb)
            hip.check(hip.lib().mvd_concat_groupnorm(hip.ptr(a), ca, hip.ptr(b), cb, hip.ptr(out) if need_out else None, hip.ptr(out_planes),
                                                     hip.ptr(planes), hip.ptr(norm.weight), hip.ptr(norm.bias),
                                                     hip.ptr(st) if st is not None else None, B, HW, 32, norm.eps, 1 if silu else 0,
                                                     hip.stream()))
            if not need_out:
                self._gn.pop(out.data_ptr(), None)
                self._unwritten.add(out.data_ptr())
            self._gn_done[(out.data_ptr(), id(norm))] = (planes, bool(silu))
            return out
        if self.gn_from_producer and HW % 16 == 0 and (ca + cb) % 32 == 0:
            st = self.gn_slot(out, B, HW, ca + cb)
        hip.check(hip.lib().mvd_concat_channels(hip.ptr(a), ca, hip.ptr(b), cb, hip.ptr(out), hip.ptr(out_planes), B * HW,
                                                hip.ptr(st) if st is not None else None, HW, 32, hip.stream()))
        return out

    def layernorm(self, x, y, norm, rows, C):
        return hip.layernorm(x, y, norm.weight, norm.bias, rows, C, norm.eps)

    def gemv_rows(self, W, bias, x, y, act_in=hip.ACT_NONE, act_out=hip.ACT_NONE):
        for r in range(0, x.shape[0], 16):
            hip.gemv(W, bias, x[r:r + 16], y[r:r + 16], act_in, act_out)
        return y


def ddim_step_table(scheduler_tables, ddim, iters):
    rows = []
    for index in iters:
        t = int(ddim["timesteps"][index])
        sac = float(scheduler_tables["sqrt_alphas_cumprod"][t])
        s1m = float(scheduler_tables["sqrt_one_minus_alphas_cumprod"][t])
        dstd = (scheduler_tables["sqrt_one_minus_alphas_cumprod"][t] / scheduler_tables["sqrt_alphas_cumprod"][t] / 10.0)
        rows.append([float(t), sac, float(dstd), float(ddim["alphas"][index]), float(ddim["alphas_prev"][index]),
                     float(ddim["sigmas"][index]), float(ddim["sqrt_one_minus_alphas"][index]),
                     1.0 if index > 0 else 0.0])
        del s1m
    return torch.tensor(rows, dtype=torch.float32)
```

### mvdfusion_amd/hip.py

```python
import ctypes as C
import os

import torch

_HERE = os.path.dirname(os.path.abspath(__file__))
LIB_PATHS = {"f16": os.path.join(_HERE, "csrc", "libmvd_hip.so"), "bf16": os.path.join(_HERE, "csrc", "libmvd_hip_bf16.so")}
if os.environ.get("MVD_HIP_LIB"):
    LIB_PATHS["f16"] = os.environ["MVD_HIP_LIB"]
LIB_PATH = LIB_PATHS["f16"]
OPERAND_FORMAT = os.environ.get("MVD_OPERAND_FORMAT", "f16")

PREC_X1, PREC_X3, PREC_X4 = 1, 3, 4
PREC_KINDS = ("conv", "skip", "proj", "qkv", "attn", "out", "geglu", "ffproj", "xattn", "ga")


def parse_precision(name):
    base, _, over = name.partition(":")
    names = {"f16": ("f16", PREC_X1), "bf16": ("bf16", PREC_X1), "f16x3": ("f16", PREC_X3), "f16x4": ("f16", PREC_X4),
             "bf16x3": ("bf16", PREC_X3), "bf16x4": ("bf16", PREC_X4)}
    if base not in names:
        raise ValueError(f"precision '{name}': base must be one of {sorted(names)}")
    fmt, default = names[base]
    policy = {}
    for item in filter(None, over.split(",")):
# ... 21 lines not shown
ALIGN_SCALE, ALIGN_NO_STEP = 1, 2
ALIGN_CHUNK = 1024
ALIGN_SUMS, ALIGN_HISTORY = 19, 3
ALIGN_MAX_ITERS = 1024

_vp, _i, _f, _sz = C.c_void_p, C.c_int, C.c_float, C.c_size_t
c_void_p = C.c_void_p


class GemmDesc(C.Structure):
    _fields_ = [
        ("M", _i), ("N", _i), ("K", _i),
        ("A", _vp), ("lda", _i), ("a_mode", _i),
        ("B", _i), ("Hin", _i), ("Win", _i), ("Cin", _i), ("Hout", _i), ("Wout", _i), ("stride", _i), ("upsample", _i), ("no_pad_tl", _i),
        ("Wp", _vp), ("b_mode", _i), ("ldb", _i), ("acc_scale", _f), ("prec", _i),
        ("epi", _i), ("act", _i), ("out", _vp), ("ldo", _i), ("out_sp", _vp), ("ldp", _i),
        ("n_store", _i),
        ("bias", _vp), ("bias_b", _vp), ("rows_per_batch", _i), ("ldbb", _i), ("colscale", _vp), ("res", _vp), ("ldr", _i),
        ("q_hi", _vp), ("q_lo", _vp), ("k_hi", _vp), ("k_lo", _vp), ("vt_hi", _vp), ("vt_lo", _vp),
        ("heads", _i), ("dhead", _i), ("L", _i), ("Lpad", _i), ("qscale", _f),
        ("splitk", _i), ("workspace", _vp), ("workspace_elems", _sz), ("cfg", _i),
        ("gn_stats", _vp), ("gn_hw", _i), ("gn_groups", _i),
        ("rs_out", _vp), ("rs_count", _vp), ("rs_ld", _i),
        ("ln_stats", _vp), ("ln_count", _vp), ("ln_colsum", _vp), ("ln_ld", _i), ("ln_dim", _i), ("ln_eps", _f),
        ("gna_out_sp", _vp), ("gna_gamma", _vp), ("gna_beta", _vp), ("gna_eps", _f), ("gna_flags", _i),
        ("cat_b", _vp), ("cat_cb", _i), ("cat_raw_sp", _vp),
        ("acc_scale_dev", _vp), ("pf_items", _vp), ("pf_n", _i),
        ("tap_mode", _i), ("A2", _vp), ("lda2", _i), ("Cin2", _i),
    ]


class PrefetchItem(C.Structure):
    _fields_ = [("ptr", _vp), ("bytes", C.c_ulonglong), ("start_after", _i), ("consumer", _i)]


SIGNATURES = {
    "mvd_version": (_i, []),
    "mvd_last_error": (C.c_char_p, []),
    "mvd_packed_weight_bytes": (_sz, [_i, _i]),
    "mvd_operand_format": (_i, []),
    "mvd_pack_linear_weight": (_i, [_vp, _i, _i, _i, _i, _f, _vp, _vp]),
    "mvd_pack_linear_weight_t": (_i, [_vp, _i, _i, _i, _f, _vp, _vp]),
    "mvd_pack_conv3x3_weight": (_i, [_vp, _i, _i, _i, _f, _vp, _vp]),
    "mvd_gemm": (_i, [C.POINTER(GemmDesc), _vp]),
    "mvd_gemm_cfg_supported": (_i, [C.POINTER(GemmDesc), _i]),
    "mvd_split_planes": (_i, [_vp, _vp, _sz, _i, _i, _i, _vp]),
    "mvd_gemv": (_i, [_vp, _vp, _vp, _vp, _i, _i, _i, _i, _i, _i, _i, _vp]),
    "mvd_groupnorm_chunks": (_i, [_i]),
    "mvd_groupnorm_nhwc": (_i, [_vp, _vp, _vp, _vp, _i, _i, _i, _i, _f, _i, _vp, _sz, _vp]),
    "mvd_layernorm": (_i, [_vp, _vp, _vp, _vp, _vp, _i, _i, _f, _i, _vp]),
    "mvd_layernorm_groups": (_i, [_vp, _vp, _vp, _vp, _vp, _i, _i, _i, _i, _f, _i, _vp]),
    "mvd_softmax_rows": (_i, [_vp, _vp, _i, _i, _i, _f, _f, _vp]),
    "mvd_attn_qk_plane_elems": (_sz, [_i, _i, _i, _i]),
    "mvd_attn_vt_plane_elems": (_sz, [_i, _i, _i, _i]),
    "mvd_attn_lpad": (_i, [_i]),
    "mvd_attention": (_i, [_vp] * 7 + [_i, _i, _i, _i, _i, _i, _i, _vp]),
    "mvd_pixel_cross_attn": (_i, [_vp, _vp, _vp, _vp, _i, _i, _i, _i, _vp]),
    "mvd_unet_input": (_i, [_vp, _vp, _vp, _i, _i, _i, _i, _vp]),
    "mvd_unet_input_scenes": (_i, [_vp, _vp, _vp, _i, _i, _i, _i, _i, _vp]),
    "mvd_concat_channels": (_i, [_vp, _i, _vp, _i, _vp, _vp, _i, _vp, _i, _i, _vp]),
    "mvd_concat_groupnorm_fits": (_i, [_i, _i, _i, _i]),
    "mvd_concat_groupnorm": (_i, [_vp, _i, _vp, _i, _vp, _vp, _vp, _vp, _vp, _vp, _i, _i, _i, _f, _i, _vp]),
    "mvd_transpose_planes": (_i, [_vp, _i, _i, _i, _i, _vp, _i, _vp]),
    "mvd_im2col3x3_t_planes": (_i, [_vp, _i, _i, _i, _i, _vp, _i, _vp]),
    "mvd_col_sum_workspace_doubles": (_sz, [_i, _i]),
    "mvd_col_sum": (_i, [_vp, _i, _i, _i, _vp, _vp, _sz, _vp]),
    "mvd_col_sum_groups_workspace_doubles": (_sz, [_i, _i, _i]),
    "mvd_col_sum_groups": (_i, [_vp, _i, _i, _i, _i, _vp, _vp, _sz, _vp]),
    "mvd_col_sum_pow2": (_i, [_vp, _i, _i, _i, _vp, _vp, _sz, _vp, _vp, _vp]),
    "mvd_gridattn_tokens_backward": (_i, [_vp, _vp, _vp, _vp, _vp, _vp, _vp, _vp, _i, _vp, _vp, _f, _i, _i, _i, _i, _i, _f, _f, _vp]),
    "mvd_gridattn_tokens_backward_scenes": (_i, [_vp, _vp, _vp, _vp, _vp, _vp, _vp, _vp, _i, _vp, _vp, _f, _i, _i, _i, _i, _i, _i, _f, _f, _i,
                                                 _vp]),
    "mvd_gridattn_tokens_backward_window": (_i, [_vp, _vp, _vp, _vp, _vp, _vp, _vp, _vp, _i, _vp, _vp, _f, _i, _i, _i, _i, _i, _i, _f, _f, _i,
                                                 _i, _vp]),
    "mvd_layernorm_backward": (_i, [_vp, _vp, _vp, _i, _i, _f, _vp, _vp, _vp]),
    "mvd_layernorm_backward_groups": (_i, [_vp, _vp, _vp, _i, _i, _i, _i, _f, _vp, _vp, _vp, _vp, _vp, _sz, _vp]),
    "mvd_geglu_backward": (_i, [_vp, _vp, _i, _i, _vp, _vp]),
    "mvd_act_planes": (_i, [_vp, _vp, _vp, _sz, _i, _i, _i, _i, _i, _vp]),
    "mvd_act_backward": (_i, [_vp, _vp, _vp, _sz, _i, _vp]),
    "mvd_attention_backward": (_i, [_vp, _vp, _vp, _vp, _i, _i, _i, _i, _vp, _vp, _vp, _vp, _sz, _vp]),
    "mvd_pixel_cross_attn_backward": (_i, [_vp, _vp, _vp, _vp, _i, _i, _i, _i, _vp, _vp, _vp, _vp]),
    "mvd_groupnorm_backward": (_i, [_vp, _vp, _vp, _vp, _i, _i, _i, _i, _f, _i, _vp, _vp, _vp, _vp, _sz, _vp]),
    "mvd_groupnorm_from_stats": (_i, [_vp, _vp, _vp, _vp, _vp, _i, _i, _i, _i, _f, _i, _vp]),
    "mvd_area_pool": (_i, [_vp, _vp, _i, _i, _i, _i, _i, _i, _vp]),
    "mvd_fill_zero": (_i, [_vp, _sz, _vp]),
    "mvd_pow2_scale": (_i, [_vp, _sz, _vp, _vp, _vp]),
    "mvd_split_planes_scaled": (_i, [_vp, _vp, _sz, _i, _i, _i, _vp, _vp]),
    "mvd_transpose_planes_scaled": (_i, [_vp, _i, _i, _i, _vp, _i, _vp, _vp]),
    "mvd_adamw_multi": (_i, [_vp, _i, _i, _f, _f, _f, _f, _f, _f, _f, _f, _vp]),
    "mvd_timestep_embedding": (_i, [_vp, _vp, _vp, _vp, _i, _vp]),
    "mvd_timestep_embedding_scenes": (_i, [_vp, _vp, _vp, _vp, _i, _i, _i, _vp]),
    "mvd_advance_iter": (_i, [_vp, _vp]),
    "mvd_zembed": (_i, [_vp, _vp, _vp, _vp, _i, _i, _vp]),
    "mvd_gridattn_tokens": (_i, [_vp] * 10 + [_i, _i, _i, _i, _i, _f, _f, _vp]),
    "mvd_gridattn_tokens_scenes": (_i, [_vp] * 10 + [_i, _i, _i, _i, _i, _i, _f, _f, _vp]),
    "mvd_gridattn_tokens_scenes_t": (_i, [_vp] * 10 + [_i, _i, _i, _i, _i, _i, _f, _f, _i, _vp]),
    "mvd_gridattn_fused_slots": (_i, []),
    "mvd_gridattn_fused_stream_bytes": (_sz, []),
    "mvd_gridattn_fused_vec_floats": (_sz, []),
    "mvd_gridattn_fused": (_i, [_vp] * 12 + [_i, _i, _i, _i, _i, _f, _f, _i, _vp]),
    "mvd_gridattn_fused_scenes": (_i, [_vp] * 12 + [_i, _i, _i, _i, _i, _i, _f, _f, _i, _vp]),
    "mvd_gridattn_fused_scenes_t": (_i, [_vp] * 12 + [_i, _i, _i, _i, _i, _i, _f, _f, _i, _i, _i, _vp]),
    "mvd_gridattn_tokens_window": (_i, [_vp] * 10 + [_i, _i, _i, _i, _i, _i, _f, _f, _i, _i, _vp]),
    "mvd_gridattn_fused_window": (_i, [_vp] * 12 + [_i, _i, _i, _i, _i, _i, _f, _f, _i, _i, _i, _i, _vp]),
    "mvd_view_mha": (_i, [_vp, _vp, _i, _i, _i, _i, _vp]),
    "mvd_view_pool": (_i, [_vp, _vp, _vp, _vp, _i, _i, _i, _vp]),
    "mvd_cfg_ddim_update": (_i, [_vp, _i, _vp, _vp, _vp, _vp, _sz, _vp, _vp, _i, _i, _i, _f, _i, _vp]),
    "mvd_pin_views": (_i, [_vp, _vp, _vp, _vp, _sz, _vp, _vp, _i, _i, _i, _i, _i, _vp]),
    "mvd_fuse_points": (_i, [_vp] * 9 + [_i, _i, _i, _i, _f, _f, _f, _f, _f, _i, _vp]),
    "mvd_compact_points_scratch": (_sz, [_sz]),
    "mvd_compact_points": (_i, [_vp] * 5 + [_sz, _i, _i, _vp, _vp, _vp, _vp, _vp, _vp, _sz, _vp]),
    "mvd_render_points_scratch": (_sz, [_i, _i]),
    "mvd_render_points": (_i, [_vp] * 4 + [_sz, _i, _i, _i, _i, _f, _f, C.POINTER(_f), _vp, _vp, _vp, _vp, _sz, _vp]),
    "mvd_render_points_stages": (_i, [_vp] * 4 + [_sz, _i, _i, _i, _i, _f, _f, C.POINTER(_f), _vp, _vp, _vp, _vp, _sz, _i, _vp]),
    "mvd_render_mesh_scratch": (_sz, [_i, _i]),
    "mvd_render_mesh": (_i, [_vp] * 6 + [_sz, _sz, _i, _i, _i, _i, _f, _f, C.POINTER(_f)] + [_vp] * 6 + [_sz, _vp]),
    "mvd_render_mesh_stages": (_i, [_vp] * 6 + [_sz, _sz, _i, _i, _i, _i, _f, _f, C.POINTER(_f)] + [_vp] * 6 + [_sz, _i, _vp]),
    "mvd_nearest_points_scratch": (_sz, [_sz, _i, _i, _i]),
    "mvd_nearest_points": (_i, [_vp] * 4 + [_sz, _sz, _i, _i, _i, _vp, _vp, _vp, _sz, _vp]),
    "mvd_nearest_points_stages": (_i, [_vp] * 4 + [_sz, _sz, _i, _i, _i, _vp, _vp, _vp, _sz, _i, _vp]),
    "mvd_align_scratch": (_sz, [_sz, _sz, _i, _i, _i]),
    "mvd_align_solve": (_i, [_vp, _i, _vp, _vp]),
    "mvd_align_apply": (_i, [_vp, _vp, _sz, _i, _vp, _vp, _vp]),
    "mvd_align_fit": (_i, [_vp] * 5 + [_sz, _sz, _i, _i, _f, _vp, _vp, _vp, _sz, _vp]),
    "mvd_align_icp": (_i, [_vp] * 4 + [_sz, _sz, _i, _i, _i, _i, _i, _f] + [_vp] * 6 + [_sz, _vp]),
    "mvd_tsdf_integrate": (_i, [_vp] * 7 + [_i, _i, _i, _i, _i, _f, _f, _f, _f, _f, _i, _f, _f, _f, _f, _vp]),
    "mvd_mesh_scratch": (_sz, [_i, _i]),
    "mvd_mesh_count": (_i, [_vp, _vp, _i, _i, _vp, _vp, _vp, _sz, _vp]),
    "mvd_mesh_emit": (_i, [_vp] * 4 + [_i, _i, _f, _f, _f, _f, C.POINTER(_f), _vp, _vp, _vp, _sz, _sz, _vp, _sz, _vp]),
    "mvd_graph_begin": (_i, [_vp]),
    "mvd_graph_end": (_i, [_vp, C.POINTER(_vp)]),
    "mvd_graph_launch": (_i, [_vp, _vp]),
    "mvd_graph_destroy": (_i, [_vp]),
    "mvd_event_create": (_i, [C.POINTER(_vp)]),
    "mvd_event_record": (_i, [_vp, _vp]),
    "mvd_event_elapsed_ms": (_i, [_vp, _vp, C.POINTER(_f)]),
    "mvd_event_destroy": (_i, [_vp]),
}

_lib = None


def lib():
    global _lib
    if _lib is None:
        path = LIB_PATHS[OPERAND_FORMAT]
        if not os.path.exists(path):
            raise RuntimeError(
                f"{path} not found: build it with `python -m mvdfusion_amd.csrc.build` "
                "(or `python -c 'import __graft_entry__ as g; g.build()'`). mvdfusion_amd has no CPU fallback.")
        l = C.CDLL(path)
        for name, (res, args) in SIGNATURES.items():
            fn = getattr(l, name)
            fn.restype, fn.argtypes = res, args
        assert l.mvd_operand_format() == {"f16": 0xf16, "bf16": 0xbf16}[OPERAND_FORMAT]
        _lib = l
        load_default_tuned()
    return _lib


def set_operand_format(fmt):
    global OPERAND_FORMAT
    assert fmt in LIB_PATHS
    if _lib is not None and fmt != OPERAND_FORMAT:
        raise RuntimeError(f"operand format already fixed to {OPERAND_FORMAT} for this process")
    OPERAND_FORMAT = fmt


def check(rc):
    if rc != 0:
        raise RuntimeError(f"mvd_hip error {rc}: {lib().mvd_last_error().decode()}")


try:
    _raw_stream = torch._C._cuda_getCurrentRawStream
# ... 285 lines not shown
def sp_cols(p):
    return p.shape[-1] // 2


def split_planes(x, out=None, ldp=None, scale=None):
    rows, cols = x.numel() // x.shape[-1], x.shape[-1]
    ldp = (cols + 31) // 32 * 32 if ldp is None else ldp
    if out is None:
        out = planes_like(rows, ldp, x.device)
    if scale is None:
        check(lib().mvd_split_planes(ptr(x), ptr(out), rows, cols, cols, ldp, stream()))
    else:
        check(lib().mvd_split_planes_scaled(ptr(x), ptr(out), rows, cols, cols, ldp, ptr(scale), stream()))
    return out


def gemm(A, W, out=None, *, prec=PREC_X4, M=None, lda=None, bias=True, act=ACT_NONE, res=None, colscale=None,
         bias_b=None, rows_per_batch=0, epi=EPI_STORE, conv=None, qkv=None, workspace=None, splitk=0, ldo=None,
         out_planes=None, out_planes_col=0, cfg=None, gn_stats=None, gn_hw=0, gn_groups=32, row_stats=None, ln=None, gn_apply=None, cat=None,
         acc_scale_dev=None, a2=None):
    assert A.dtype == torch.int16, "A must be in split-planes format (see hip.split_planes)"
    d = GemmDesc()
    d.N, d.K = W.N, W.K
    d.A = A.data_ptr()
    d.Wp = W.data.data_ptr()
    if isinstance(W, PlanesOperand):
        d.b_mode, d.ldb = 1, W.ld
    d.acc_scale = W.acc_scale
    if acc_scale_dev is not None:
        d.acc_scale_dev = acc_scale_dev.data_ptr()
    d.prec = prec
    if conv is not None:
        d.a_mode = A_CONV3X3
        for k in ("B", "Hin", "Win", "Cin", "Hout", "Wout", "stride", "upsample"):
            setattr(d, k, int(conv[k]))
        d.no_pad_tl = int(conv.get("no_pad_tl", 0))
        d.M = conv["B"] * conv["Hout"] * conv["Wout"]
        tail_cin = getattr(W, "tail_cin", 0)
        assert (a2 is not None) == bool(tail_cin), "a weight of pack_conv3x3_tail needs a2=, and only such a weight takes it"
        if a2 is not None:
            assert a2.dtype == torch.int16 and a2.numel() // a2.shape[-1] == d.M and a2.shape[-1] // 2 >= tail_cin
            d.tap_mode, d.A2, d.lda2, d.Cin2 = TAPS_CENTRE_TAIL, a2.data_ptr(), int(a2.shape[-1] // 2), int(tail_cin)
        if getattr(W, "up4", False):
            assert a2 is None and conv["Cin"] * 4 == W.K, (conv["Cin"], W.K)
            d.tap_mode = TAPS_UP4
        else:
            assert conv["Cin"] * 9 + tail_cin == W.K, (conv["Cin"], tail_cin, W.K)
    else:
        d.a_mode = A_DENSE
        d.M = int(M if M is not None else A.numel() // A.shape[-1])
        d.lda = int(lda if lda is not None else A.shape[-1] // 2)
        assert a2 is None, "a2= (centre-tap tail) belongs to a convolution"
        assert d.lda >= W.K, f"A has {d.lda} columns, packed K is {W.K} (pad A)"
    d.epi, d.act = epi, act
    if out is not None:
        d.out = out.data_ptr()
        d.ldo = int(ldo if ldo is not None else out.shape[-1])
    if out_planes is not None:
        assert out_planes_col % 32 == 0 and out_planes.dtype == torch.int16
        d.out_sp = out_planes.data_ptr() + 4 * int(out_planes_col)
        d.ldp = int(out_planes.shape[-1] // 2)
    d.n_store = W.n_real
    if bias and W.bias is not None:
        d.bias = W.bias.data_ptr()
    if bias_b is not None:
        d.bias_b = bias_b.data_ptr()
        d.rows_per_batch = int(rows_per_batch)
        d.ldbb = bias_b.stride(0) if bias_b.dim() == 2 else 0
    if colscale is not None:
        d.colscale = colscale.data_ptr()
    if res is not None:
        d.res = res.data_ptr()
        d.ldr = int(res.shape[-1])
    if qkv is not None:
        qh, ql, kh, kl, vh, vl = qkv["planes"]
        d.q_hi, d.q_lo, d.k_hi, d.k_lo, d.vt_hi, d.vt_lo = (t.data_ptr() for t in (qh, ql, kh, kl, vh, vl))
        d.heads, d.dhead, d.L = qkv["heads"], qkv["dhead"], qkv["L"]
        d.Lpad = lib().mvd_attn_lpad(qkv["L"])
        d.qscale = float(qkv["dhead"]) ** -0.5 * 1.4426950408889634
    if gn_stats is not None:
        d.gn_stats, d.gn_hw, d.gn_groups = gn_stats.data_ptr(), int(gn_hw), int(gn_groups)
    if gn_apply is not None:
        gamma, beta, eps, flags, planes = gn_apply
        ct = d.N + (cat[0].shape[-1] if cat is not None else 0)
        assert gn_stats is not None and out is not None and planes.dtype == torch.int16 and planes.shape[-1] == 2 * ct
        if cat is not None:
            skip, raw = cat
            assert skip.dtype == torch.float32 and skip.is_contiguous() and skip.shape[0] == d.M and (raw is None or raw.shape[-1] == 2 * ct)
            d.cat_b, d.cat_cb, d.cat_raw_sp = skip.data_ptr(), int(skip.shape[-1]), (raw.data_ptr() if raw is not None else None)
        d.gna_gamma, d.gna_beta, d.gna_eps, d.gna_flags, d.gna_out_sp = gamma.data_ptr(), beta.data_ptr(), float(eps), int(flags), planes.data_ptr()
    if row_stats is not None:
        assert row_stats.slots.shape[0] >= d.M and row_stats.ld >= (d.N + 31) // 32
        d.rs_out, d.rs_count, d.rs_ld = row_stats.slots.data_ptr(), row_stats.count.data_ptr(), row_stats.ld
    if ln is not None:
        rs, fold = ln
        d.ln_stats, d.ln_count, d.ln_ld = rs.slots.data_ptr(), rs.count.data_ptr(), rs.ld
        d.ln_colsum, d.ln_dim, d.ln_eps = fold.colsum.data_ptr(), fold.dim, fold.eps
        splitk = 1
    d.splitk = splitk
    if workspace is not None:
        d.workspace = workspace.data_ptr()
        d.workspace_elems = workspace.numel()
    key = (d.M, d.N, d.K, d.a_mode, d.Cin, d.stride, d.upsample, d.no_pad_tl, d.epi, d.prec, res is not None, out is not None,
           out_planes is not None, splitk, d.b_mode, row_stats is not None, ln is not None, gn_apply is not None, cat[0].shape[-1] if cat is not None else 0,
           d.tap_mode, d.Cin2)
    if cfg is None:
        tuned = _TUNED.get(key)
        if tuned is None and AUTOTUNE and 2.0 * d.M * d.N * d.K >= AUTOTUNE_MIN_FLOPS:
            tuned = _autotune(d, A if A.is_contiguous() else None, W_data=W.data if not isinstance(W, PlanesOperand) else None)
            _TUNED[key] = tuned
            global TUNED_IN_RUN
            TUNED_IN_RUN += 1
        if tuned is not None:
            cfg, d.splitk = tuned
    d.cfg = cfg or 0
    global LAST_CFG
    LAST_CFG = d.cfg
    if GEMM_SEQUENCE is not None:
        GEMM_SEQUENCE.note(d, W)
    check(lib().mvd_gemm(C.byref(d), stream()))
    return out


GEMM_SEQUENCE = None
SELF_PREFETCH_MIN = int(os.environ.get("MVD_SELF_PREFETCH_MIN", "0"))


class WeightPrefetcher:

    def __init__(self, device, window=24 << 20, max_items=24, gn_hosts=0, self_min=None):
        self.device = device
        self.window, self.max_items = int(window), int(max_items)
        self.self_min = int(SELF_PREFETCH_MIN if self_min is None else self_min)
        self.gn_hosts = bool(gn_hosts)
        self.seq, self.recording, self.table, self.n, self.launch_idx, self.shares = [], False, None, 0, 0, {}

    class _Following:
        def __init__(self, pf, record):
            self.pf, self.record = pf, record

        def __enter__(self):
            global GEMM_SEQUENCE
            self.prev, GEMM_SEQUENCE = GEMM_SEQUENCE, self.pf
            self.pf.recording = self.record
            self.pf.launch_idx = 0
            if self.record:
                self.pf.seq = []
            return self.pf

        def __exit__(self, *exc):
            global GEMM_SEQUENCE
            GEMM_SEQUENCE = self.prev
            if self.record and exc[0] is None:
                self.pf._build()
            self.pf.recording = False
            return False

    def following(self, record=False):
        return WeightPrefetcher._Following(self, record)

    def note(self, d, W):
        j = self.launch_idx
        self.launch_idx += 1
        is_ws = bool(d.cfg) and _cfg_parts(d.cfg)[1] == WS_LOOP
        host = 1 if is_ws else (2 if (d.gna_out_sp and d.splitk != 1 and self.gn_hosts) else 0)
        if self.recording:
            packed = not isinstance(W, PlanesOperand)
            self.seq.append((W.data.data_ptr(), W.data.numel() * W.data.element_size(), host) if packed else (0, 0, host))
            return
        if host and j in self.shares:
            first, n = self.shares[j]
            d.pf_items, d.pf_n = self.table.data_ptr() + first * C.sizeof(PrefetchItem), n

    def _build(self):
        items = []
        self.shares = {}
        hosts = [j for j, e in enumerate(self.seq) if e[2]]
        sure = [j for j, e in enumerate(self.seq) if e[2] == 1]
        for j in hosts:
            nxt = [k for k in sure if k > j]
            end = nxt[0] if nxt else len(self.seq) - 1
            first, acc, seen = len(items), 0, set()
            if self.self_min > 0 and self.seq[j][2] == 1 and self.seq[j][1] >= self.self_min:
                items.append((self.seq[j][0], self.seq[j][1], j, j))
                seen.add(self.seq[j][0])
            for k in range(j + 1, end + 1):
                ptr_, nbytes, _ = self.seq[k]
                if not nbytes or ptr_ in seen or acc + nbytes > self.window or len(items) - first >= self.max_items:
                    continue
                seen.add(ptr_)
# ... 156 lines not shown


def release_tuning_buffers():
    global _TRASH
    _TRASH = None


_TUNE_STATS = {}


def _autotune(d, A=None, reps=4, trials=int(os.environ.get("MVD_TUNE_TRIALS", "3")), W_data=None):
    best, best_ms = (0, d.splitk), float("inf")
    e0, e1 = Event(), Event()
    stats_ptr, d.gn_stats = d.gn_stats, None
    if d.gna_out_sp:
        n = (d.M // d.gn_hw) * d.gn_groups * 2
        n = (n, str(A.device) if A is not None else "cuda")
        scratch = _TUNE_STATS.get(n)
        if scratch is None:
            scratch = _TUNE_STATS[n] = torch.zeros(n[0], dtype=torch.int64, device=A.device if A is not None else "cuda")
        d.gn_stats = scratch.data_ptr()
    skip = set()
    skip |= {int(t) for t in os.environ.get("MVD_TUNE_EXCLUDE_LOOPS", "").split(",") if t}
    fixed_split = d.splitk
    cands = [(c, sk) for c in gemm_configs(d.epi, d.b_mode, conv=d.a_mode == A_CONV3X3) if cfg_supported(d, c) and _cfg_parts(c)[1] not in skip
             for sk in ((0, 1) if d.splitk == 0 else (d.splitk,))]
    timed, second_pass = [], False
    wp0 = d.Wp
    rot = [wp0]
    if TUNE_COLD and A is not None and d.b_mode == 0:
        if W_data is not None and W_data.data_ptr() == wp0:
            rot += [W_data.clone(), W_data.clone()]
    ptrs = [wp0] + [t.data_ptr() for t in rot[1:]]
    for cfg, sk in cands:
        d.cfg, d.splitk = cfg, sk
        check(lib().mvd_gemm(C.byref(d), stream()))
        ms = float("inf")
        if TUNE_COLD and A is not None:
            for _ in range(trials + 1):
                _flush_caches()
                A.view(-1)[:A.numel() // 2 * 2].view(torch.int32).sum()
                e0.record()
                for wp in ptrs:
                    d.Wp = wp
                    check(lib().mvd_gemm(C.byref(d), stream()))
                e1.record()
                ms = min(ms, e0.elapsed_ms(e1) / len(ptrs))
            d.Wp = wp0
        else:
            for _ in range(trials):
                e0.record()
                for _ in range(reps):
                    check(lib().mvd_gemm(C.byref(d), stream()))
                e1.record()
                ms = min(ms, e0.elapsed_ms(e1))
        if sk != 1:
            ms += 0.0015
        timed.append((ms, cfg, sk))
        if ms < best_ms * 0.99:
            best, best_ms = (cfg, sk), ms
        if len(timed) == len(cands) and TUNE_SPLITS and fixed_split == 0 and not second_pass:
            second_pass = True
            nk = d.K // 32
            extra = [s_ for s_ in (2, 3, 4, 6, 8, 12, 16, 24, 32) if s_ <= max(1, nk // 2)]
            top = sorted(timed)[:3]
            cands.extend((c, s_) for _, c, _ in top for s_ in extra if (c, s_) not in cands)
    d.gn_stats = stats_ptr
    return best


def gemv(W, bias, x, y, act_in=ACT_NONE, act_out=ACT_NONE):
    M, K = x.shape
    N = W.shape[0]
    check(lib().mvd_gemv(ptr(W), ptr(bias), ptr(x), ptr(y), M, N, K, x.stride(0), y.stride(0), act_in, act_out, stream()))
    return y


def groupnorm(x, y, gamma, beta, B, HW, Cc, eps, silu, ws):
    check(lib().mvd_groupnorm_nhwc(ptr(x), ptr(y), ptr(gamma), ptr(beta), B, HW, Cc, 32, eps, int(silu), ptr(ws), ws.numel(),
                                   stream()))
    return y


def groupnorm_from_stats(x, y, gamma, beta, stats, B, HW, Cc, eps, silu, groups=32):
    check(lib().mvd_groupnorm_from_stats(ptr(x), ptr(y), ptr(gamma), ptr(beta), ptr(stats), B, HW, Cc, groups, eps, int(silu), stream()))
    return y


def layernorm(x, y, w, b, rows, Cc, eps=1e-5, w_plus_one=False, y_f32=None):
    check(lib().mvd_layernorm(ptr(x), ptr(y), ptr(y_f32), ptr(w), ptr(b), rows, Cc, eps, int(w_plus_one), stream()))
    return y


def layernorm_groups(x, y, w, b, rows, Cc, rows_per_group, eps=1e-5, w_plus_one=False, y_f32=None):
    assert w.stride(0) == b.stride(0) and w.stride(-1) == 1 and b.stride(-1) == 1, (w.stride(), b.stride())
    check(lib().mvd_layernorm_groups(ptr(x), ptr(y), ptr(y_f32), ptr(w), ptr(b), w.stride(0), rows, int(rows_per_group), Cc, eps,
                                     int(w_plus_one), stream()))
    return y


def softmax_rows(x, y, scale=1.0, out_scale=1.0):
    rows, cols = x.shape
    check(lib().mvd_softmax_rows(ptr(x), ptr(y), rows, cols, x.stride(0), float(scale), float(out_scale), stream()))
    return y


def attention(planes, out, B, heads, L, dhead, prec=PREC_X4, Lkeys=0):
    qh, ql, kh, kl, vh, vl = planes
    check(lib().mvd_attention(ptr(qh), ptr(ql), ptr(kh), ptr(kl), ptr(vh), ptr(vl), ptr(out), out.shape[-1] // 2, B, heads,
                              L, Lkeys, dhead, prec, stream()))
    return out


def alloc_attn_planes(B, heads, L, dhead, device):
    nqk = lib().mvd_attn_qk_plane_elems(B, heads, L, dhead)
    nvt = lib().mvd_attn_vt_plane_elems(B, heads, L, dhead)
    mk = lambda n: torch.zeros(n, dtype=torch.int16, device=device)
    return (mk(nqk), mk(nqk), mk(nqk), mk(nqk), mk(nvt), mk(nvt))


class Graph:

    def __init__(self):
        self.exec = C.c_void_p()

    def __enter__(self):
        self._side = torch.cuda.Stream()
        self._side.wait_stream(torch.cuda.current_stream())
        self._ctx = torch.cuda.stream(self._side)
        self._ctx.__enter__()
        check(lib().mvd_graph_begin(stream()))
        return self

    def __exit__(self, et, ev, tb):
        rc = lib().mvd_graph_end(stream(), C.byref(self.exec))
        self._ctx.__exit__(et, ev, tb)
        torch.cuda.current_stream().wait_stream(self._side)
        if et is None:
            check(rc)
        return False

    def launch(self):
        check(lib().mvd_graph_launch(self.exec, stream()))

    def __del__(self):
        try:
            if self.exec:
                lib().mvd_graph_destroy(self.exec)
        except Exception:
            pass


class Event:
    def __init__(self):
        self.h = C.c_void_p()
        check(lib().mvd_event_create(C.byref(self.h)))

    def record(self):
        check(lib().mvd_event_record(self.h, stream()))

    def elapsed_ms(self, stop):
        ms = C.c_float()
        check(lib().mvd_event_elapsed_ms(self.h, stop.h, C.byref(ms)))
        return ms.value
```

### mvdfusion_amd/unet.py

```python
import math

import torch
import torch.nn as nn

from . import hip
from .attention import SpatialTransformer, ViewAlignedFeatureTransformer
from .engine import Ctx


class GroupNorm32(nn.GroupNorm):
    pass


def normalization(channels):
    return GroupNorm32(32, channels)


class TimestepBlock(nn.Module):
    pass


class Upsample(nn.Module):
    def __init__(self, channels, use_conv, dims=2, out_channels=None, padding=1):
        super().__init__()
        self.channels, self.out_channels = channels, out_channels or channels
        self.conv = nn.Conv2d(self.channels, self.out_channels, 3, padding=padding)
        self._p = self._p4 = None

    def run(self, ctx, x, H, W, out=None):
        if hip.use_up4(ctx.B, H, W, training=ctx.keep_fp32):
            if self._p4 is None:
                self._p4 = hip.pack_conv3x3_up4(self.conv.weight, self.conv.bias)
            wp = self._p4
        else:
            if self._p is None:
                self._p = hip.pack_conv3x3(self.conv.weight, self.conv.bias)
            wp = self._p
        if out is None:
            out = ctx.act((ctx.B * 4 * H * W, self.out_channels))
        xp = hip.split_planes(x, ctx.ws.planes("updown.x", ctx.B * H * W, self.channels))
        ctx.gemm(xp, wp, out, conv=dict(B=ctx.B, Hin=H, Win=W, Cin=self.channels, Hout=2 * H, Wout=2 * W,
                                            stride=1, upsample=1), gn=(ctx.B, 4 * H * W), kind="conv")
        return out, 2 * H, 2 * W


class Downsample(nn.Module):
    def __init__(self, channels, use_conv, dims=2, out_channels=None, padding=1):
        super().__init__()
        self.channels, self.out_channels = channels, out_channels or channels
        self.op = nn.Conv2d(self.channels, self.out_channels, 3, stride=2, padding=padding)
        self._p = None

    def run(self, ctx, x, H, W, out=None):
        if self._p is None:
            self._p = hip.pack_conv3x3(self.op.weight, self.op.bias)
        Ho, Wo = H // 2, W // 2
        if out is None:
            out = ctx.act((ctx.B * Ho * Wo, self.out_channels))
        xp = hip.split_planes(x, ctx.ws.planes("updown.x", ctx.B * H * W, self.channels))
        ctx.gemm(xp, self._p, out, conv=dict(B=ctx.B, Hin=H, Win=W, Cin=self.channels, Hout=Ho, Wout=Wo, stride=2,
                                            upsample=0), gn=(ctx.B, Ho * Wo), kind="conv")
        return out, Ho, Wo


class ResBlock(TimestepBlock):

    def __init__(self, channels, emb_channels, dropout, out_channels=None, dims=2, use_checkpoint=False,
                 use_scale_shift_norm=False):
        super().__init__()
        assert not use_scale_shift_norm
        self.channels, self.out_channels = channels, out_channels or channels
        self.in_layers = nn.Sequential(normalization(channels), nn.SiLU(),
                                       nn.Conv2d(channels, self.out_channels, 3, padding=1))
        self.emb_layers = nn.Sequential(nn.SiLU(), nn.Linear(emb_channels, self.out_channels))
        self.out_layers = nn.Sequential(normalization(self.out_channels), nn.SiLU(), nn.Dropout(p=dropout),
                                        nn.Conv2d(self.out_channels, self.out_channels, 3, padding=1))
        self.skip_connection = nn.Identity() if self.out_channels == channels else \
            nn.Conv2d(channels, self.out_channels, 1)
        self._p = None

    def packed(self, fuse_skip=True):
        c1, c2, sk = self.in_layers[2], self.out_layers[3], self.skip_connection
        fuse = bool(fuse_skip) and not isinstance(sk, nn.Identity)
        if self._p is None:
            self._p = (hip.pack_conv3x3(c1.weight, None), None, None)
        if self._p[1] is None or bool(self._p[1].tail_cin) != fuse:
            w2 = hip.pack_conv3x3_tail(c2.weight, c2.bias, sk.weight, sk.bias) if fuse else hip.pack_conv3x3(c2.weight, c2.bias)
            wsk = None if fuse or isinstance(sk, nn.Identity) else hip.pack_linear(sk.weight, sk.bias)
            self._p = (self._p[0], w2, wsk)
        return self._p

    def run(self, ctx, x, H, W, out=None, x_planes=None):
        B, Ci, Co = ctx.B, self.channels, self.out_channels
        M = B * H * W
        w1, w2, wsk = self.packed(fuse_skip=ctx.prec_of("skip") == ctx.prec_of("conv"))
        geo = dict(B=B, Hin=H, Win=W, Hout=H, Wout=W, stride=1, upsample=0)
        a = ctx.ws.planes("res.a", M, Ci)
        ctx.groupnorm(x, a, self.in_layers[0], B, H * W, Ci, silu=True)
        h = ctx.ws.get("res.h", (M, Co))
        a2 = ctx.ws.planes("res.a2", M, Co)
        eb = ctx.emb_bias[self]
        ctx.gemm(a, w1, h, conv=dict(Cin=Ci, **geo), bias=False, bias_b=eb, rows_per_batch=M // eb.shape[0],
                 gn=(B, H * W), kind="conv",
                 gn_apply=(self.out_layers[0], a2, True, True))
        if (wsk is not None or w2.tail_cin) and x_planes is None:
            x_planes = hip.split_planes(x, ctx.ws.planes("res.xp", M, Ci))
        if out is None:
            out = ctx.act((M, Co))
        if w2.tail_cin:
            ctx.gemm(a2, w2, out, conv=dict(Cin=Co, **geo), a2=x_planes, gn=(B, H * W), kind="conv")
            return out
        skip = x
        if wsk is not None:
            skip = ctx.ws.get("res.skip", (M, Co))
            ctx.gemm(x_planes, wsk, skip, kind="skip")
        ctx.gemm(a2, w2, out, conv=dict(Cin=Co, **geo), res=skip, gn=(B, H * W), kind="conv")
        return out


def gn_hint(layer):
    from .attention import SpatialTransformer, ViewAlignedFeatureTransformer
    if isinstance(layer, tuple):
        return layer
    if isinstance(layer, ResBlock):
        return layer.in_layers[0], "res.a", True
    if isinstance(layer, SpatialTransformer):
        return layer.norm, "tf.n", False
    if isinstance(layer, ViewAlignedFeatureTransformer):
        return layer.aligned_attn_norm, "tf.n", False
    return None


class TimestepEmbedSequential(nn.Sequential, TimestepBlock):
    def run(self, ctx, x, H, W, out=None, x_planes=None, next_layer=None, next_cat=None):
        n = len(self)
        for i, layer in enumerate(self):
            dst = out if i == n - 1 else None
            ctx.next_gn = gn_hint(self[i + 1] if i + 1 < n else next_layer)
            ctx.next_cat = next_cat if i == n - 1 else None
            if isinstance(layer, (Upsample, Downsample)):
                x, H, W = layer.run(ctx, x, H, W, out=dst)
            elif isinstance(layer, ResBlock):
                x = layer.run(ctx, x, H, W, out=dst, x_planes=x_planes if i == 0 else None)
            else:
                x = layer.run(ctx, x, H, W, out=dst)
            ctx.next_gn = None
            ctx.next_cat = None
        return x, H, W


class _StemConv(nn.Conv2d):
    _p = None

    def run(self, ctx, x, H, W, out):
        if self._p is None:
            self._p = hip.pack_conv3x3(self.weight, self.bias)
        ctx.gemm(x, self._p, out, conv=dict(B=ctx.B, Hin=H, Win=W, Cin=self._p.conv_cin, Hout=H, Wout=W, stride=1,
                                            upsample=0), gn=(ctx.B, H * W), kind="conv")
        return out


class UNetModel(nn.Module):
    def __init__(self, image_size, in_channels, model_channels, out_channels, num_res_blocks, attention_resolutions,
                 dropout=0, channel_mult=(1, 2, 4, 8), conv_resample=True, dims=2, num_classes=None,
                 use_checkpoint=False, use_fp16=False, num_heads=-1, num_head_channels=-1, num_heads_upsample=-1,
                 use_scale_shift_norm=False, resblock_updown=False, use_new_attention_order=False,
                 use_spatial_transformer=True, use_view_aligned_transformer=True, transformer_depth=1,
                 context_dim=None, n_embed=None, legacy=True):
        super().__init__()
        assert use_view_aligned_transformer and use_spatial_transformer and context_dim is not None
        assert dims == 2 and num_classes is None and not resblock_updown and n_embed is None and conv_resample
        assert num_heads != -1 and num_head_channels == -1, "this build supports the num_heads form (configs/*.yaml)"
        if isinstance(context_dim, (list, tuple)) or type(context_dim).__name__ == "ListConfig":
            context_dim = list(context_dim)[0]
        channel_mult = tuple(channel_mult)
        attention_resolutions = tuple(attention_resolutions)
        self.image_size, self.in_channels, self.model_channels = image_size, in_channels, model_channels
        self.out_channels, self.num_res_blocks, self.channel_mult = out_channels, num_res_blocks, channel_mult
        self.attention_resolutions, self.num_heads, self.context_dim = attention_resolutions, num_heads, context_dim
        ted = model_channels * 4
        self.time_embed = nn.Sequential(nn.Linear(model_channels, ted), nn.SiLU(), nn.Linear(ted, ted))

        def res(cin, cout):
            return ResBlock(cin, ted, dropout, out_channels=cout, use_checkpoint=use_checkpoint)

        def st(c):
            return SpatialTransformer(c, num_heads, c // num_heads, depth=transformer_depth, context_dim=context_dim)

        def vaft(c):
            return ViewAlignedFeatureTransformer(c, num_heads, c // num_heads, depth=transformer_depth,
                                                 context_dim=context_dim, image_size=image_size)

        self.input_blocks = nn.ModuleList([TimestepEmbedSequential(_StemConv(in_channels, model_channels, 3, padding=1))])
        skip_chans = [model_channels]
        ch, ds = model_channels, 1
        for level, mult in enumerate(channel_mult):
            for _ in range(num_res_blocks):
                layers = [res(ch, mult * model_channels)]
                ch = mult * model_channels
                if ds in attention_resolutions:
                    layers.append(st(ch))
                self.input_blocks.append(TimestepEmbedSequential(*layers))
                skip_chans.append(ch)
            if level != len(channel_mult) - 1:
                self.input_blocks.append(TimestepEmbedSequential(Downsample(ch, True, out_channels=ch)))
                skip_chans.append(ch)
                ds *= 2
        self.middle_block = TimestepEmbedSequential(res(ch, ch), st(ch), vaft(ch), res(ch, ch))
        self.output_blocks = nn.ModuleList([])
        for level, mult in list(enumerate(channel_mult))[::-1]:
            for i in range(num_res_blocks + 1):
                layers = [res(ch + skip_chans.pop(), model_channels * mult)]
                ch = model_channels * mult
                if ds in attention_resolutions:
                    layers += [st(ch), vaft(ch)]
                if level and i == num_res_blocks:
                    layers.append(Upsample(ch, True, out_channels=ch))
                    ds //= 2
                self.output_blocks.append(TimestepEmbedSequential(*layers))
        self.out = nn.Sequential(normalization(ch), nn.SiLU(), nn.Conv2d(model_channels, out_channels, 3, padding=1))
        self._head = None
        self._temb = None
        self._xattn = None
        self._head_saved = None
        self._record = None

    def get_cross_attn_parameters(self, finetune_cross_attn, finetune_view_attn):
        out = []
        for name, p in self.named_parameters():
            if finetune_cross_attn and any(k in name for k in (".norm.", ".proj_in.", ".transformer_blocks.", ".proj_out.")):
                out.append(p)
            if finetune_view_attn and ".aligned_attn_" in name:
                out.append(p)
        return out

    def disable_unet_grad(self):
        for name, p in self.named_parameters():
            if ".aligned_attn_" not in name:
                p.requires_grad_(False)

    def _resblocks(self):
        return [m for m in self.modules() if isinstance(m, ResBlock)]

    def time_biases(self, ctx, t_sin):
        if self._temb is None:
            blocks = self._resblocks()
            w = torch.cat([b.emb_layers[1].weight.detach() for b in blocks], 0).contiguous()
            bias = torch.cat([b.emb_layers[1].bias.detach() + b.in_layers[2].bias.detach() for b in blocks], 0).contiguous()
            offs, o = {}, 0
            for b in blocks:
                offs[b] = (o, o + b.out_channels)
                o += b.out_channels
            self._temb = (w, bias, offs)
        w, bias, offs = self._temb
        ted = self.model_channels * 4
        R = t_sin.shape[0]
        e1, emb = ctx.ws.get("temb.e1", (R, ted)), ctx.ws.get("temb.emb", (R, ted))
        out = ctx.ws.get("temb.bias", (R, w.shape[0]))
        ctx.gemv_rows(self.time_embed[0].weight, self.time_embed[0].bias, t_sin, e1, act_out=hip.ACT_SILU)
        ctx.gemv_rows(self.time_embed[2].weight, self.time_embed[2].bias, e1, emb)
        ctx.gemv_rows(w, bias, emb, out, act_in=hip.ACT_SILU)
        ctx.emb_bias = {b: out[:, lo:hi] for b, (lo, hi) in offs.items()}

    def cross_attn_vectors(self, ctx):
        if self._xattn is None:
            sts = [m for m in self.modules() if isinstance(m, SpatialTransformer)]
            ws, bs, offs, o = [], [], {}, 0
            for st in sts:
                a2 = st.transformer_blocks[0].attn2
                wo, wv = a2.to_out[0].weight.detach().double(), a2.to_v.weight.detach().double()
                ws.append((wo @ wv).float())
                bs.append(a2.to_out[0].bias.detach().float())
                offs[st] = (o, o + st.in_channels)
                o += st.in_channels
            self._xattn = (torch.cat(ws, 0).contiguous(), torch.cat(bs, 0).contiguous(), offs, o)
        w, bias, offs, total = self._xattn
        out = ctx.ws.get("xattn.vec", (ctx.context.shape[0], total))
        ctx.gemv_rows(w, bias, ctx.context, out)
        ctx.xattn_vec = {st: out[:, lo:hi] for st, (lo, hi) in offs.items()}

    def run(self, ctx, x_in, t_sin, S):
        B = ctx.B
        self.time_biases(ctx, t_sin)
        self.cross_attn_vectors(ctx)
        hs = []
        H = W = S
        h = x_in
        rec = self._record
        for bi, blk in enumerate(self.input_blocks):
            if rec is not None:
                rec.append((blk, h.clone(), H, W, 0))
            if bi == 0:
                o = ctx.ws.get("hs0", (B * H * W, self.model_channels))
                ctx.next_gn = gn_hint(self.input_blocks[1][0])
                h = blk[0].run(ctx, h, H, W, o)
                ctx.next_gn = None
            else:
                last = blk[-1]
                Ho, Wo = (H // 2, W // 2) if isinstance(last, Downsample) else (H, W)
                co = last.out_channels if isinstance(last, (ResBlock, Downsample)) else last.in_channels
                o = ctx.ws.get(f"hs{bi}", (B * Ho * Wo, co))
                nxt = self.input_blocks[bi + 1][0] if bi + 1 < len(self.input_blocks) else self.middle_block[0]
                h, H, W = blk.run(ctx, h, H, W, out=o, next_layer=nxt)
            hs.append((h, H, W))
        if rec is not None:
            rec.append((self.middle_block, h.clone(), H, W, 0))
        keep = rec is not None or ctx.keep_fp32

        def cat_hint(nblk, co, Hn, Wn):
            first = nblk[0]
            if keep or not isinstance(first, ResBlock) or isinstance(first.skip_connection, nn.Identity):
                return None
            nsk = hs[-1][0]
            Mn = B * Hn * Wn
            return (nsk, ctx.ws.get("cat", (Mn, co + nsk.shape[-1])), ctx.ws.planes("catp", Mn, co + nsk.shape[-1])) + gn_hint(first)

        def out_geometry(blk, H, W):
            last = blk[-1]
            co = last.out_channels if isinstance(last, (ResBlock, Upsample)) else last.in_channels
            return (co, 2 * H, 2 * W) if isinstance(last, Upsample) else (co, H, W)

        h, H, W = self.middle_block.run(ctx, h, H, W, next_cat=cat_hint(self.output_blocks[0], *out_geometry(self.middle_block, H, W)))
        for bi, blk in enumerate(self.output_blocks):
            sk, _, _ = hs.pop()
            M = B * H * W
            ca, cb = h.shape[-1], sk.shape[-1]
            cat = ctx.ws.get("cat", (M, ca + cb))
            catp = ctx.ws.planes("catp", M, ca + cb)
            first = blk[0]
            if cat.data_ptr() in ctx._cat_done:
                ctx._cat_done.discard(cat.data_ptr())
            else:
                need_cat = keep or not isinstance(first, ResBlock) or isinstance(first.skip_connection, nn.Identity)
                ctx.concat(h, ca, sk, cb, cat, catp, B, H * W, gn_apply=gn_hint(first), need_out=need_cat)
            if rec is not None:
                rec.append((blk, cat.clone(), H, W, ca))
            last_blk = bi + 1 == len(self.output_blocks)
            h, H, W = blk.run(ctx, cat, H, W, x_planes=catp, next_layer=(self.out[0], "res.a", True) if last_blk else None,
                              next_cat=None if last_blk else cat_hint(self.output_blocks[bi + 1], *out_geometry(blk, H, W)))
        if self._head is None:
            self._head = hip.pack_conv3x3(self.out[2].weight, self.out[2].bias)
        M = B * H * W
        a = ctx.ws.planes("res.a", M, self.model_channels)
        ctx.groupnorm(h, a, self.out[0], B, H * W, self.model_channels, silu=True)
        y = ctx.ws.get("head", (M, 8))
        ctx.gemm(a, self._head, y, conv=dict(B=B, Hin=H, Win=W, Cin=self.model_channels, Hout=H, Wout=W, stride=1,
                                             upsample=0), ldo=8, kind="conv")
        self._head_saved = (h, a)
        return y


class UNetWrapper(nn.Module):

    def __init__(self, unet_config, unet_path=None, drop_conditions=False, drop_scheme="default", use_zero_123=False,
                 finetune_unet=False, finetune_cross_attn=False, finetune_view_attn=True, remove_keys=()):
        super().__init__()
        params = unet_config.get("params", unet_config) if hasattr(unet_config, "get") else unet_config
        self.unet_model = UNetModel(**dict(params))
        if unet_path:
            from .load_model import load_unet_checkpoint
            load_unet_checkpoint(self.unet_model, unet_path, remove_keys=remove_keys)
        if not finetune_unet:
            self.unet_model.disable_unet_grad()
        self.drop_conditions, self.drop_scheme, self.use_zero_123 = drop_conditions, drop_scheme, use_zero_123
        self.finetune_unet, self.finetune_cross_attn, self.finetune_view_attn = \
            finetune_unet, finetune_cross_attn, finetune_view_attn

    def get_trainable_parameters(self):
        if self.finetune_unet:
            return self.unet_model.parameters()
        return self.unet_model.get_cross_attn_parameters(finetune_cross_attn=self.finetune_cross_attn,
                                                         finetune_view_attn=self.finetune_view_attn)

    def level_channels(self):
        u = self.unet_model
        return [u.model_channels * m for m in u.channel_mult]

    def level0_operand(self, ctx, B, S, D):
        rows = B * S * S * D
        if D == 1:
            c0 = self.level_channels()[0]
            return ctx.ws.get("ovol0", (rows, 2 * (c0 + 768)), torch.int16, zero=True), c0
        return ctx.ws.get("vol0", (rows, 2 * 768), torch.int16, zero=True), 0

    def volume_pyramid(self, ctx, vol, B, S, D):
        levels = [self.level0_operand(ctx, B, S, D)]
# ... 15 lines not shown
```

### mvdfusion_amd/viewfusion_zero_depth_rgb.py

```python
import math

import torch
import torch.nn as nn

from . import hip
from .cameras import Cameras, get_camera_slice, get_relative_camera, pack_cameras
from .engine import Ctx, ddim_step_table
from .sampler import DDIMSampler
from .scheduler import DDPMScheduler
from .unet import UNetWrapper
from .view_attn_efficient2 import GridAttn

import os

PREFETCH_WEIGHTS = os.environ.get("MVD_PREFETCH", "ws")
PREFETCH_OPTIONS = {k: int(v) for k, v in (kv.split("=") for kv in os.environ.get("MVD_PREFETCH_OPTS", "").split(",") if kv)}


def _sinusoid_freqs(dim, max_period=10000):
    half = dim // 2
    return torch.exp(-math.log(max_period) * torch.arange(start=0, end=half, dtype=torch.float32) / half)


class StepEngine:
# ... 49 lines not shown
        V, S = self.V, self.S
        for n, (bc, il, ic, ce) in enumerate(conds):
            self.cams[n * V:(n + 1) * V].copy_(pack_cameras(bc).to(self.cams.device))
            self.in_cam[n:n + 1].copy_(pack_cameras(ic).to(self.cams.device))
            self.input_latents[n:n + 1].copy_(il.reshape(1, 5, S, S))
            self.clip_v_embed[n * V:(n + 1) * V].copy_(ce.reshape(V, 796))

    def set_schedule(self, steps_table, depth_noise, ddim_noise):
        self._set_tables(steps_table, depth_noise, ddim_noise, scene_stride=0)

    def set_schedule_scenes(self, steps_table, depth_noise, ddim_noise=None):
        if self.cfg:
            raise ValueError("StepEngine.set_schedule_scenes: per-scene timesteps need a cfg=False engine (the training step); "
                             "guided sampling steps share one timestep")
        if tuple(steps_table.shape) != (self.N, hip.STEP_STRIDE):
            raise ValueError(f"StepEngine.set_schedule_scenes: step table {tuple(steps_table.shape)} for {self.N} scenes "
                             f"(expected ({self.N}, {hip.STEP_STRIDE}))")
        if ddim_noise is None:
            ddim_noise = torch.zeros(1, self.N * self.V, 5, self.S, self.S)
        self._set_tables(steps_table, depth_noise, ddim_noise, scene_stride=1 if self.N > 1 else 0)

    def _set_tables(self, steps_table, depth_noise, ddim_noise, scene_stride):
        dev = self.ctx.device
        if self.steps.shape != steps_table.shape:
            self.graphs.clear()
            self.prefetchers.clear()
            self.steps = steps_table.to(dev).contiguous()
            self.steps_nodiv = self.steps.clone()
            self.depth_noise = depth_noise.to(dev).contiguous()
            self.ddim_noise = ddim_noise.to(dev).contiguous()
        else:
            self.steps.copy_(steps_table)
            self.depth_noise.copy_(depth_noise)
            self.ddim_noise.copy_(ddim_noise)
        self.steps_nodiv.copy_(self.steps)
        self.steps_nodiv[:, 1] = 1.0
        self.steps_scene_stride = scene_stride
        self.n_rows = int(steps_table.shape[0]) - (self.N - 1) * scene_stride
        self.rewind()

    def set_pin(self, mode, known, noise=None):
        dev = self.ctx.device
        nk = int(known.shape[0])
        K = nk // self.N
        if mode not in (0, 1) or K < 1 or K * self.N != nk or K > self.V or tuple(known.shape[1:]) != (5, self.S, self.S):
            raise ValueError(f"StepEngine.set_pin: mode {mode}, known {tuple(known.shape)} for {self.N} scene(s) of {self.V} views at "
                             f"S = {self.S} (expected (N*K, 5, S, S), 1 <= K <= V)")
        if mode == 1 and (noise is None or tuple(noise.shape) != (int(self.steps.shape[0]), nk, 5, self.S, self.S)):
            raise ValueError(f"StepEngine.set_pin: mode 1 needs noise ({int(self.steps.shape[0])}, {nk}, 5, {self.S}, {self.S}), got "
                             f"{None if noise is None else tuple(noise.shape)}")
        if self.known.shape != known.shape:
            self.graphs.clear()
            self.prefetchers.clear()
            self.known = known.to(dev, torch.float32).contiguous().clone()
        else:
            self.known.copy_(known)
        if mode == 1:
            if self.pin_noise is None or self.pin_noise.shape != noise.shape:
                self.graphs.clear()
                self.prefetchers.clear()
                self.pin_noise = noise.to(dev, torch.float32).contiguous().clone()
            else:
                self.pin_noise.copy_(noise)
        self.pin = (int(mode), K)

    def clear_pin(self):
        self.pin = None

    def rewind(self, it=0):
        assert 0 <= it < self.n_rows
        self.iter.fill_(it)
        self.done = it

    def depth_geo(self):
        if self.depth_mode == 0:
            return self.x, self.steps
        return (self.x0 if self.depth_mode == 1 else self.prev), self.steps_nodiv

    def enqueue(self, cfg_scale, do_update, prefetcher=None):
        m, ctx, L = self.m, self.ctx, hip.lib()
        V, S, D, B, q0, Vq, N = self.V, self.S, self.D, self.B, self.q0, self.Vq, self.N
        NVq = N * Vq
        ctx.B, ctx.D = B, D
        ctx.begin_step()
        st = hip.stream
        sst, R = self.steps_scene_stride, self.t_rows
        if sst and do_update:
            raise ValueError("StepEngine: per-scene timesteps (set_schedule_scenes) are a training step: no DDIM update")
        if self.pin is not None:
            mode, K = self.pin
            pn = self.pin_noise if mode == 1 else None
            hip.check(L.mvd_pin_views(hip.ptr(self.x), hip.ptr(self.x0), hip.ptr(self.known), hip.ptr(pn), N * K * 5 * S * S,
                                      hip.ptr(self.steps), hip.ptr(self.iter), N, V, K, S, mode, st()))
        ts = ctx.ws.get("vf.tsin", (R, 256))
        te1 = ctx.ws.get("vf.te1", (R, 256))
        c = ctx.ws.get("vf.c", (R, 256))
        hip.check(L.mvd_timestep_embedding_scenes(hip.ptr(self.steps), hip.ptr(self.iter), hip.ptr(self.f256), hip.ptr(ts), 256, R, sst,
                                                  st()))
        ctx.gemv_rows(m.time_embed[0].weight, m.time_embed[0].bias, ts, te1, act_out=hip.ACT_SILU)
        ctx.gemv_rows(m.time_embed[2].weight, m.time_embed[2].bias, te1, c)
        dsrc, dsteps = self.depth_geo()
        m.view_attn.run(ctx, self.x, self.depth_noise, self.steps, self.iter, self.cams, self.in_cam,
                        self.input_latents, c, self.vol, V, S, D, q0=q0, Vq=Vq, vol_planes=self.vol_planes,
                        vol_planes_col=self.vol_col, depth_src=None if self.depth_mode == 0 else dsrc,
                        depth_steps=None if self.depth_mode == 0 else dsteps, scenes=N, steps_scene_stride=sst)
        p = m.cc_projection
        c1 = ctx.ws.get("vf.cc1", (NVq, 768))
        c2 = ctx.ws.get("vf.cc2", (NVq, 768))
        ctx.gemv_rows(p[0].weight, p[0].bias, self.clip_v_embed[q0:q0 + NVq], c1, act_out=hip.ACT_SILU)
        ctx.gemv_rows(p[2].weight, p[2].bias, c1, c2, act_out=hip.ACT_SILU)
        ctx.gemv_rows(p[4].weight, p[4].bias, c2, self.context[:NVq])
        if self.drop_masks is not None:
            clip_m, vol_m, cat_m = self.drop_masks
            self.context[:NVq] *= clip_m[:, None]
            self.vol.view(B, -1)[:NVq] *= vol_m[:, None]
            vp = self.vol_planes.view(B, S * S * D, -1)
            vp[:NVq, :, 2 * self.vol_col:] *= vol_m.to(torch.int16)[:, None, None]
        ctx.context = self.context
        xq, x0q, epsq = self.x[q0:q0 + NVq], self.x0[q0:q0 + NVq], self.eps[q0:q0 + NVq]
        hip.check(L.mvd_unet_input_scenes(hip.ptr(xq), hip.ptr(self.input_latents), hip.ptr(self.x_in), N, Vq, S, 32,
                                          int(self.cfg), st()))
        if self.drop_masks is not None:
            xin = self.x_in.view(B, S * S, 64)
            cm = self.drop_masks[2].to(torch.int16)[:, None, None]
            xin[:NVq, :, 5:10] *= cm
            xin[:NVq, :, 37:42] *= cm
        unet = m.unet_model.unet_model
        ctx.vol_levels = m.unet_model.volume_pyramid(ctx, self.vol.view(B, S, S, D, 768), B, S, D)
        tsu = ctx.ws.get("vf.tsin_unet", (R, unet.model_channels))
        hip.check(L.mvd_timestep_embedding_scenes(hip.ptr(self.steps), hip.ptr(self.iter), hip.ptr(self.funet), hip.ptr(tsu),
                                                  unet.model_channels, R, sst, st()))
        y = unet.run(ctx, self.x_in, tsu, S)
        hip.check(L.mvd_cfg_ddim_update(hip.ptr(y), 8, hip.ptr(xq), hip.ptr(x0q), hip.ptr(epsq),
                                        hip.ptr(self.ddim_noise[:, q0:q0 + NVq]), N * V * 5 * S * S, hip.ptr(self.steps),
                                        hip.ptr(self.iter), NVq, S, int(self.cfg), float(cfg_scale), int(do_update), st()))
        if do_update:
            hip.check(L.mvd_advance_iter(hip.ptr(self.iter), st()))

    @property
    def t_rows(self):
        return self.N if self.steps_scene_stride else 1

    def step(self, cfg_scale, do_update, use_graph=True):
        key = (float(cfg_scale), bool(do_update), int(self.depth_mode), self.steps_scene_stride, self.pin)
        if self.done >= self.n_rows:
            raise IndexError(f"StepEngine.step: iteration {self.done} is past the {self.n_rows}-row step table "
                             "(set_schedule() / rewind() before stepping again)")
        if do_update:
            self.done += 1
        if not use_graph:
            return self.enqueue(cfg_scale, do_update)
        g = self.graphs.get(key)
        if g is None:
            it0 = self.iter.clone()
            x_keep, x0_keep = self.x.clone(), self.x0.clone()
            hip.AUTOTUNE = True
            try:
                self.enqueue(cfg_scale, do_update)
            finally:
                hip.AUTOTUNE = False
                hip.release_tuning_buffers()
            torch.cuda.synchronize()
            pf = None
            if PREFETCH_WEIGHTS == "ws":
                pf = hip.WeightPrefetcher(self.x.device, **PREFETCH_OPTIONS)
                self.iter.copy_(it0)
                self.x.copy_(x_keep)
                self.x0.copy_(x0_keep)
                with pf.following(record=True):
                    self.enqueue(cfg_scale, do_update)
                torch.cuda.synchronize()
            self.iter.copy_(it0)
            self.x.copy_(x_keep)
            self.x0.copy_(x0_keep)
            g = hip.Graph()
            self.ctx.ws.frozen = True
            try:
                with g:
                    if pf is None:
                        self.enqueue(cfg_scale, do_update)
                    else:
                        with pf.following():
                            self.enqueue(cfg_scale, do_update, prefetcher=pf)
            finally:
                self.ctx.ws.frozen = False
            self.graphs[key] = g
            self.prefetchers[key] = pf
        g.launch()


class _HipTrainingLoss(torch.autograd.Function):

    @staticmethod
    def forward(ctx, model, batch, trainer_config, names, *params):
        loss, grads = model.gradients(batch, trainer_config, noise_source=getattr(model, "_noise_source", None), only_trainable=True)
        ctx.grads = [grads.get(n) for n in names]
        ctx.shapes = [p.shape for p in params]
        return loss.clone()

    @staticmethod
    def backward(ctx, grad_out):
        if getattr(ctx, "_scaled", False):
            raise RuntimeError("_HipTrainingLoss.backward ran twice on one node: the step's gradient buffers were already scaled in place "
                               "(call model(batch, cfg) again instead of retain_graph=True)")
        ctx._scaled = True
        live, seen, spans = [], set(), []
        for g in ctx.grads:
            if g is None:
                continue
            key = (g.untyped_storage().data_ptr(), g.storage_offset(), tuple(g.shape), tuple(g.stride()))
            if key in seen:
                continue
            seen.add(key)
            live.append(g)
            spans.append((g.data_ptr(), g.data_ptr() + g.numel() * g.element_size()) if g.is_contiguous() else None)
        disjoint = all(sp is not None for sp in spans)
        if disjoint:
            srt = sorted(spans)
            disjoint = all(srt[i][1] <= srt[i + 1][0] for i in range(len(srt) - 1))
        if live and disjoint:
            torch._foreach_mul_(live, grad_out.to(live[0].dtype))
            pick = lambda g: g
        else:
            pick = lambda g: g * grad_out.to(g.dtype)
        outs = [torch.zeros(s, dtype=grad_out.dtype, device=grad_out.device) if g is None else pick(g).reshape(s)
                for g, s in zip(ctx.grads, ctx.shapes)]
        return (None, None, None, None, *outs)


class ViewFusion(nn.Module):
    def __init__(self, view_attn_config, unet_config, ddpm_config, vae_config=None, unet_path="", vae_path="",
                 clip_path="", unet_cc_path="", z_scale_factor=0.18215, vae_max_batch=8, objective="noise",
                 loss_type="l2", embed_camera_pose=True, finetune_projection=False, finetune_unet=False,
                 finetune_cross_attn=True, finetune_view_attn=True, feed_prev_depth=False, drop_conditions=False,
                 vae=None, clip_image_encoder=None, precision=None, reference_eval_dropout=False, overwrite_x_noisy=False, **kwargs):
        super().__init__()
        assert embed_camera_pose, "this build implements the embed_camera_pose=True configuration of configs/*.yaml"
        self.finetune_projection, self.finetune_unet, self.z_scale_factor = finetune_projection, finetune_unet, z_scale_factor
        self.vae_max_batch, self.objective, self.loss_type = vae_max_batch, objective, loss_type
        self.embed_camera_pose, self.finetune_cross_attn, self.finetune_view_attn = \
            embed_camera_pose, finetune_cross_attn, finetune_view_attn
        self.feed_prev_depth, self.drop_conditions = feed_prev_depth, drop_conditions
        self.reference_eval_dropout = bool(reference_eval_dropout)
        from .configs import DEFAULT_PRECISION
        precision = precision or DEFAULT_PRECISION
        fmt, self.precision, self.precision_policy = hip.parse_precision(precision)
        hip.set_operand_format(fmt)
        self.precision_name = precision

        def params(cfg):
            return dict(cfg.get("params", cfg)) if hasattr(cfg, "get") else dict(cfg)

        self.view_attn = GridAttn(**params(view_attn_config))
        self.unet_model = UNetWrapper(unet_config, unet_path=unet_path or None, drop_conditions=drop_conditions,
                                      drop_scheme="default", finetune_unet=finetune_unet,
                                      finetune_cross_attn=finetune_cross_attn, finetune_view_attn=finetune_view_attn,
                                      use_zero_123=True,
                                      remove_keys=["input_blocks.0.0.weight", "out.2.weight", "out.2.bias"])
        self.scheduler = DDPMScheduler(**params(ddpm_config))
        if vae is not None:
            self.vae = vae
        elif vae_config is not None:
            from .load_model import instantiate_from_config
            self.vae = instantiate_from_config(vae_config)
            if vae_path:
                sd = torch.load(vae_path, map_location="cpu")
                sd = sd.get("state_dict", sd)
                self.vae.load_state_dict({k.replace("first_stage_model.", ""): v for k, v in sd.items()}, strict=False)
        if clip_image_encoder is not None:
            self.clip_image_encoder = clip_image_encoder
        elif clip_path:
# ... 441 lines not shown
```

Baseline: 121.5 steps/s.

## Fuse raw-plane emission into GroupNorm apply and fold arena zeroing into iter advance

GroupNorm apply kernels can now also write the raw hi/lo planes of their input, so the next conv/up/downsample reuses them instead of running split_planes again. Per-step stats-arena zeroing is folded into the advance-iter kernel, which removes a separate launch. The split-K GroupNorm epilogue is templated on thread count, unroll and split count, with a size-based launcher. Gamma/beta loads are hoisted ahead of the reduction to drop a barrier, and workspace indexing uses 32-bit offsets. This adds state-tracking complexity (arena cleanliness, raw-plane handoff), which risks stale buffers if the hints are wrong.

New measurement: 122.1 steps/s (median of 6 runs). Within noise of the previous version (+0.5%).

```diff
diff --git a/include/mvd_hip.h b/include/mvd_hip.h
--- a/include/mvd_hip.h
+++ b/include/mvd_hip.h
@@ -128,6 +128,8 @@
                        int groups, float eps, int silu, double* ws, size_t ws_elems, mvd_stream_t stream);
 int mvd_groupnorm_from_stats(const float* x, void* y_sp, const float* gamma, const float* beta, const long long* stats, int B, int HW,
                              int C, int groups, float eps, int silu, mvd_stream_t stream);
+int mvd_groupnorm_from_stats_raw(const float* x, void* y_sp, void* raw_sp, const float* gamma, const float* beta, const long long* stats,
+                                 int B, int HW, int C, int groups, float eps, int silu, mvd_stream_t stream);
 int mvd_softmax_rows(const float* x, void* y_sp, int rows, int cols, int ldx, float scale, float out_scale,
                      mvd_stream_t stream);
 
@@ -164,6 +166,7 @@
 int mvd_timestep_embedding_scenes(const float* steps, const int* iter, const float* freqs, float* out, int dim, int nscene,
                                   int steps_scene_stride, mvd_stream_t stream);
 int mvd_advance_iter(int* iter, mvd_stream_t stream);
+int mvd_advance_iter_zero(int* iter, void* zero_p, size_t zero_bytes, mvd_stream_t stream);
 
 #define MVD_CAM_RECORD 20
 #define MVD_TOKEN_DIM 723
diff --git a/mvdfusion_amd/csrc/elementwise.hip b/mvdfusion_amd/csrc/elementwise.hip
--- a/mvdfusion_amd/csrc/elementwise.hip
+++ b/mvdfusion_amd/csrc/elementwise.hip
@@ -147,7 +147,7 @@
   constexpr int NT = MVD_CGN_THREADS, NWV = NT / 64, U = 4;
   extern __shared__ float s_val[];
   __shared__ double s_red[2][NWV];
-  __shared__ float s_coef[2][128];
+  __shared__ __attribute__((aligned(16))) float s_coef[2][128];
   const int C = ca + cb, cg = C / groups, cg2 = cg >> 1;
   int g, img;
   {
@@ -168,6 +168,7 @@
   const int dq = NT / cg2, dj = NT - dq * cg2;
   const int rs = tid / cg2, js = tid - rs * cg2;
   const int r0 = tid < total ? rs : 0, j0 = tid < total ? js : 0;
+  const float gam = gamma[c0 + (tid < cg ? tid : 0)], bet = beta[c0 + (tid < cg ? tid : 0)];
   float s = 0.f, q = 0.f;
   {
     int r = rs, j = js;
@@ -220,6 +221,10 @@
       s_red[1][wave] = qd;
     }
   }
+  if (tid < cg) {
+    s_coef[0][tid] = gam;
+    s_coef[1][tid] = bet;
+  }
   __syncthreads();
   double S1 = 0.0, S2 = 0.0;
 #pragma unroll
@@ -231,20 +236,16 @@
   const double mean = S1 / cnt;
   double var = S2 / cnt - mean * mean;
   if (var < 0.0) var = 0.0;
-  const float rstd = (float)(1.0 / sqrt(var + (double)eps));
-  if (tid < cg) {
-    const float aa = rstd * gamma[c0 + tid];
-    s_coef[0][tid] = aa;
-    s_coef[1][tid] = beta[c0 + tid] - (float)mean * aa;
-  }
+  const float rstd = (float)(1.0 / sqrt(var + (double)eps)), meanf = (float)mean;
   if (tid == 0 && stats) gn_stats_add(stats, img, g, groups, (float)S1, (float)S2);
-  __syncthreads();
   {
     int r = rs, j = js;
     for (int e = tid; e < total; e += NT) {
       float2 v = *(const float2*)(s_val + 2 * e);
-      v.x = v.x * s_coef[0][2 * j] + s_coef[1][2 * j];
-      v.y = v.y * s_coef[0][2 * j + 1] + s_coef[1][2 * j + 1];
+      const float2 cgm = *(const float2*)&s_coef[0][2 * j], cbt = *(const float2*)&s_coef[1][2 * j];
+      const float ax = rstd * cgm.x, ay = rstd * cgm.y;
+      v.x = v.x * ax + (cbt.x - meanf * ax);
+      v.y = v.y * ay + (cbt.y - meanf * ay);
       if (flags & 2) {
         v.x = (float)(_Float16)v.x;
         v.y = (float)(_Float16)v.y;
@@ -312,8 +313,9 @@
   }
 }
 
-__global__ void advance_iter_kernel(int* iter) {
-  if (threadIdx.x == 0) iter[0] += 1;
+__global__ __launch_bounds__(256) void advance_iter_kernel(int* iter, uint4* __restrict__ zero_p, size_t n16) {
+  if (blockIdx.x == 0 && threadIdx.x == 0) iter[0] += 1;
+  for (size_t e = (size_t)blockIdx.x * 256 + threadIdx.x; e < n16; e += (size_t)gridDim.x * 256) zero_p[e] = make_uint4(0u, 0u, 0u, 0u);
 }
 
 __global__ __launch_bounds__(256) void cfg_ddim_kernel(const float* __restrict__ eps_nhwc, int ldc, float* __restrict__ x,
@@ -522,8 +524,18 @@
 
 extern "C" int mvd_advance_iter(int* iter, mvd_stream_t stream) {
   MVD_CHECK_ARG(iter != nullptr, "mvd_advance_iter: null pointer");
-  hipLaunchKernelGGL(advance_iter_kernel, dim3(1), dim3(64), 0, (hipStream_t)stream, iter);
+  hipLaunchKernelGGL(advance_iter_kernel, dim3(1), dim3(64), 0, (hipStream_t)stream, iter, (uint4*)nullptr, (size_t)0);
   MVD_CHECK_LAUNCH("mvd_advance_iter");
+  return 0;
+}
+
+extern "C" int mvd_advance_iter_zero(int* iter, void* zero_p, size_t zero_bytes, mvd_stream_t stream) {
+  MVD_CHECK_ARG(iter != nullptr, "mvd_advance_iter_zero: null pointer");
+  if (zero_p == nullptr) zero_bytes = 0;
+  MVD_CHECK_ARG(((uintptr_t)zero_p & 15) == 0 && zero_bytes % 16 == 0, "mvd_advance_iter_zero: zero_p / zero_bytes must be multiples of 16");
+  const size_t n16 = zero_bytes / 16;
+  hipLaunchKernelGGL(advance_iter_kernel, dim3(n16 ? grid_for(n16) : 1), dim3(256), 0, (hipStream_t)stream, iter, (uint4*)zero_p, n16);
+  MVD_CHECK_LAUNCH("mvd_advance_iter_zero");
   return 0;
 }
 
diff --git a/mvdfusion_amd/csrc/gemm.hip b/mvdfusion_amd/csrc/gemm.hip
--- a/mvdfusion_amd/csrc/gemm.hip
+++ b/mvdfusion_amd/csrc/gemm.hip
@@ -133,12 +133,12 @@
   gn_stats_add(d.gn_stats, m0 / d.gn_hw, g, d.gn_groups, ss, qq);
 }
 
-#define MVD_GNK_THREADS 1024
-__global__ __launch_bounds__(MVD_GNK_THREADS) void splitk_gn_kernel(GemmParams p) {
-  constexpr int NT = MVD_GNK_THREADS, NWV = NT / 64, U = 3, ZC = 4;
+template <int NT, int U, int ZC>
+__global__ __launch_bounds__(NT) void splitk_gn_kernel(GemmParams p) {
+  constexpr int NWV = NT / 64;
   extern __shared__ float s_val[];
   __shared__ double s_red[2][NWV];
-  __shared__ float s_coef[2][128];
+  __shared__ __attribute__((aligned(16))) float s_coef[2][128];
   const mvd_gemm_desc& d = p.d;
   const int G = d.gn_groups, HW = d.gn_hw;
   const int CT = d.N + (d.cat_b ? d.cat_cb : 0);
@@ -166,6 +166,7 @@
   const float* const zero2 = (const float*)g_zero_page;
   const bool has_bias = d.bias != nullptr, has_bb = d.bias_b != nullptr, has_res = d.res != nullptr;
   const float ascale = gemm_acc_scale(d);
+  const float gam = d.gna_gamma[c0 + (tid < cg ? tid : 0)], bet = d.gna_beta[c0 + (tid < cg ? tid : 0)];
   float s = 0.f, q = 0.f;
   {
     int r = rs, j = js;
@@ -188,7 +189,6 @@
       float2 t[ZC][U];
       const int nz0 = p.splits < ZC ? p.splits : ZC;
       bool own[U];
-      float2 tc[U];
 #pragma unroll
       for (int u = 0; u < U; ++u) {
         const int m = m0 + rr[u], nn = c0 + 2 * jj[u];
@@ -196,12 +196,10 @@
         const int n = own[u] ? nn : 0;
         tb[u] = *(const float2*)(has_bias ? d.bias + n : zero2);
         tbb[u] = *(const float2*)(has_bb ? d.bias_b + (size_t)(m / d.rows_per_batch) * d.ldbb + n : zero2);
-        tr[u] = *(const float2*)(has_res ? d.res + (size_t)m * d.ldr + n : zero2);
-        tc[u] = *(const float2*)(own[u] ? zero2 : d.cat_b + (size_t)m * d.cat_cb + (nn - d.N));
+        tr[u] = *(const float2*)(own[u] ? (has_res ? d.res + (size_t)m * d.ldr + n : zero2) : d.cat_b + (size_t)m * d.cat_cb + (nn - d.N));
 #pragma unroll
         for (int z = 0; z < ZC; ++z) {
-          const float* w = d.workspace + (size_t)(z < nz0 ? z : 0) * MN + (size_t)m * d.N + n;
-          t[z][u] = *(const float2*)w;
+          t[z][u] = *(const float2*)((const char*)(d.workspace + (size_t)(z < nz0 ? z : 0) * MN) + ((unsigned)m * (unsigned)d.N + (unsigned)n) * 4u);
         }
       }
 #pragma unroll
@@ -220,7 +218,8 @@
         for (int u = 0; u < U; ++u) {
           const int m = m0 + rr[u], n = own[u] ? c0 + 2 * jj[u] : 0;
 #pragma unroll
-          for (int z = 0; z < ZC; ++z) t[z][u] = *(const float2*)(d.workspace + (size_t)(zb + (z < nz ? z : 0)) * MN + (size_t)m * d.N + n);
+          for (int z = 0; z < ZC; ++z)
+            t[z][u] = *(const float2*)((const char*)(d.workspace + (size_t)(zb + (z < nz ? z : 0)) * MN) + ((unsigned)m * (unsigned)d.N + (unsigned)n) * 4u);
         }
 #pragma unroll
         for (int u = 0; u < U; ++u)
@@ -236,7 +235,7 @@
         float2 v = acc[u];
         v.x = v.x * ascale + tb[u].x + tbb[u].x + tr[u].x;
         v.y = v.y * ascale + tb[u].y + tbb[u].y + tr[u].y;
-        if (!own[u]) v = tc[u];
+        if (!own[u]) v = tr[u];
         if (ok[u]) {
           const int m = m0 + rr[u], n = c0 + 2 * jj[u];
           if (put_out && own[u]) *(float2*)(d.out + (size_t)m * d.ldo + n) = v;
@@ -274,6 +273,10 @@
       s_red[1][wave] = qd;
     }
   }
+  if (tid < cg) {
+    s_coef[0][tid] = gam;
+    s_coef[1][tid] = bet;
+  }
   __syncthreads();
   double S1 = 0.0, S2 = 0.0;
 #pragma unroll
@@ -285,22 +288,18 @@
   const double mean = S1 / cnt;
   double var = S2 / cnt - mean * mean;
   if (var < 0.0) var = 0.0;
-  const float rstd = (float)(1.0 / sqrt(var + (double)d.gna_eps));
-  if (tid < cg) {
-    const float a = rstd * d.gna_gamma[c0 + tid];
-    s_coef[0][tid] = a;
-    s_coef[1][tid] = d.gna_beta[c0 + tid] - (float)mean * a;
-  }
+  const float rstd = (float)(1.0 / sqrt(var + (double)d.gna_eps)), meanf = (float)mean;
   if (tid == 0 && d.gn_stats) gn_stats_add(d.gn_stats, b, g, G, (float)S1, (float)S2);
-  __syncthreads();
   u16* const ysp = (u16*)d.gna_out_sp;
   const int fl = d.gna_flags;
   {
     int r = rs, j = js;
     for (int e = tid; e < total; e += NT) {
       float2 v = *(const float2*)(s_val + 2 * e);
-      v.x = v.x * s_coef[0][2 * j] + s_coef[1][2 * j];
-      v.y = v.y * s_coef[0][2 * j + 1] + s_coef[1][2 * j + 1];
+      const float2 cgm = *(const float2*)&s_coef[0][2 * j], cbt = *(const float2*)&s_coef[1][2 * j];
+      const float ax = rstd * cgm.x, ay = rstd * cgm.y;
+      v.x = v.x * ax + (cbt.x - meanf * ax);
+      v.y = v.y * ay + (cbt.y - meanf * ay);
       if (fl & MVD_GNA_ROUND_F16) {
         v.x = (float)(_Float16)v.x;
         v.y = (float)(_Float16)v.y;
@@ -323,6 +322,24 @@
     }
   }
   asm volatile("" ::"v"(pf_sink));
+}
+
+template <int NT, int U, int ZC>
+static hipError_t splitk_gn_launch_as(const GemmParams& p, int blocks, size_t lds, hipStream_t s) {
+  static unsigned long long raised = 0;
+  const hipError_t e = mvd_raise_dynamic_lds((const void*)splitk_gn_kernel<NT, U, ZC>, 128 * 1024, &raised);
+  if (e != hipSuccess) return e;
+  hipLaunchKernelGGL((splitk_gn_kernel<NT, U, ZC>), dim3(blocks), dim3(NT), lds, s, p);
+  return hipSuccess;
+}
+
+static hipError_t splitk_gn_launch(const GemmParams& p, int blocks, int pairs, size_t lds, hipStream_t s) {
+  const int z = p.splits;
+  if (pairs <= 512) return z <= 8 ? splitk_gn_launch_as<256, 2, 8>(p, blocks, lds, s) : splitk_gn_launch_as<256, 2, 16>(p, blocks, lds, s);
+  if (pairs <= 1536)
+    return z <= 4 ? splitk_gn_launch_as<512, 3, 4>(p, blocks, lds, s)
+                  : (z <= 8 ? splitk_gn_launch_as<512, 3, 8>(p, blocks, lds, s) : splitk_gn_launch_as<1024, 2, 16>(p, blocks, lds, s));
+  return z <= 2 ? splitk_gn_launch_as<1024, 5, 2>(p, blocks, lds, s) : splitk_gn_launch_as<1024, 3, 4>(p, blocks, lds, s);
 }
 
 struct TileInfo {
@@ -486,6 +503,9 @@
                       mvd_concat_groupnorm_fits(d.N, d.cat_cb, d.gn_hw, d.gn_groups),
                   "mvd_gemm: cat_b (GroupNorm over [out | cat_b]) needs gna_out_sp, an even cat_cb, (N + cat_cb) %% 32 == 0 and a shape "
                   "mvd_concat_groupnorm_fits() accepts (N=%d cat_cb=%d hw=%d)", d.N, d.cat_cb, d.gn_hw);
+  if (d.cat_raw_sp && !d.cat_b)
+    MVD_CHECK_ARG(d.gna_out_sp && ((uintptr_t)d.cat_raw_sp & 127) == 0,
+                  "mvd_gemm: cat_raw_sp without cat_b (raw planes of the output) needs gna_out_sp and 128-byte alignment");
   long long* const gna_stats = d.gn_stats;
   if (d.cat_b) d.gn_stats = nullptr;
   if (d.b_mode == MVD_B_PLANES)
@@ -555,16 +575,12 @@
   const size_t gna_lds = (size_t)d.gn_hw * gna_cg * 4;
   const bool gna_fused = d.gna_out_sp && p.splits > 1 && !d.rs_out && !d.out_sp && !d.colscale && d.act == MVD_ACT_NONE && (gna_cg & 1) == 0 &&
                          gna_cg <= 128 && gna_lds <= 128 * 1024 && d.ldo % 2 == 0 && (!d.res || d.ldr % 2 == 0) && (!d.bias_b || d.ldbb % 2 == 0) &&
-                         d.N % 2 == 0;
+                         d.N % 2 == 0 && (size_t)d.M * d.N < ((size_t)1 << 30);
   if (gna_fused) {
-    {
-      static unsigned long long raised = 0;
-      const hipError_t e = mvd_raise_dynamic_lds((const void*)splitk_gn_kernel, 128 * 1024, &raised);
-      MVD_CHECK_ARG(e == hipSuccess, "mvd_gemm: hipFuncSetAttribute(MaxDynamicSharedMemorySize): %s", hipGetErrorString(e));
-    }
     p.d.gn_stats = gna_stats;
     if (loop == 7) p.d.pf_items = nullptr;
-    hipLaunchKernelGGL(splitk_gn_kernel, dim3((d.M / d.gn_hw) * d.gn_groups), dim3(MVD_GNK_THREADS), gna_lds, s, p);
+    const hipError_t e = splitk_gn_launch(p, (d.M / d.gn_hw) * d.gn_groups, d.gn_hw * (gna_cg >> 1), gna_lds, s);
+    MVD_CHECK_ARG(e == hipSuccess, "mvd_gemm: hipFuncSetAttribute(MaxDynamicSharedMemorySize): %s", hipGetErrorString(e));
     MVD_CHECK_LAUNCH("mvd_gemm/splitk_gn");
     return 0;
   }
@@ -589,8 +605,8 @@
     return mvd_concat_groupnorm(d.out, d.N, d.cat_b, d.cat_cb, nullptr, d.cat_raw_sp, d.gna_out_sp, d.gna_gamma, d.gna_beta, gna_stats,
                                 d.M / d.gn_hw, d.gn_hw, d.gn_groups, d.gna_eps, d.gna_flags & (MVD_GNA_SILU | MVD_GNA_ROUND_F16), stream);
   if (d.gna_out_sp)
-    return mvd_groupnorm_from_stats(d.out, d.gna_out_sp, d.gna_gamma, d.gna_beta, d.gn_stats, d.M / d.gn_hw, d.gn_hw, d.N, d.gn_groups,
-                                    d.gna_eps, d.gna_flags & (MVD_GNA_SILU | MVD_GNA_ROUND_F16), stream);
+    return mvd_groupnorm_from_stats_raw(d.out, d.gna_out_sp, d.cat_raw_sp, d.gna_gamma, d.gna_beta, d.gn_stats, d.M / d.gn_hw, d.gn_hw, d.N,
+                                        d.gn_groups, d.gna_eps, d.gna_flags & (MVD_GNA_SILU | MVD_GNA_ROUND_F16), stream);
   return 0;
 }
 
diff --git a/mvdfusion_amd/csrc/norm.hip b/mvdfusion_amd/csrc/norm.hip
--- a/mvdfusion_amd/csrc/norm.hip
+++ b/mvdfusion_amd/csrc/norm.hip
@@ -146,7 +146,7 @@
   }
 }
 
-__global__ __launch_bounds__(256) void gn_apply_stats_kernel(const float* __restrict__ x, u16* __restrict__ y_sp,
+__global__ __launch_bounds__(256) void gn_apply_stats_kernel(const float* __restrict__ x, u16* __restrict__ y_sp, u16* __restrict__ raw_sp,
                                                              const float* __restrict__ gamma, const float* __restrict__ beta,
                                                              const long long* __restrict__ stats, int HW, int C, int groups, int chunks,
                                                              float eps, int silu) {
@@ -157,6 +157,14 @@
   const int chunk = blockIdx.x, b = blockIdx.y;
   const int rows = HW / chunks;
   const int cg = C / groups;
+  const size_t row0 = (size_t)b * HW + (size_t)chunk * rows;
+  const int C4 = C >> 2;
+  const int n4 = rows * C4;
+  const float4* x4 = (const float4*)(x + row0 * C);
+  const int tc0 = threadIdx.x, tc1 = threadIdx.x + 256;
+  const float g0 = gamma[tc0 < C ? tc0 : 0], b0 = beta[tc0 < C ? tc0 : 0];
+  const float g1 = gamma[tc1 < C ? tc1 : 0], b1 = beta[tc1 < C ? tc1 : 0];
+  const float4 vfirst = x4[(int)threadIdx.x < n4 ? threadIdx.x : 0];
   if (threadIdx.x < groups) {
     const long long* p = stats + ((size_t)b * groups + threadIdx.x) * 2;
     const double inv = 1.0 / (double)MVD_GN_FIXED_SCALE;
@@ -170,19 +178,16 @@
   __syncthreads();
   for (int c = threadIdx.x; c < C; c += 256) {
     const int g = c / cg;
-    const float a = s_rstd[g] * gamma[c];
+    const float a = s_rstd[g] * (c == tc0 ? g0 : (c == tc1 ? g1 : gamma[c]));
     s_a[c] = a;
-    s_b[c] = beta[c] - s_mean[g] * a;
-  }
-  __syncthreads();
-  const size_t row0 = (size_t)b * HW + (size_t)chunk * rows;
-  const int C4 = C >> 2;
-  const int n4 = rows * C4;
-  const float4* x4 = (const float4*)(x + row0 * C);
+    s_b[c] = (c == tc0 ? b0 : (c == tc1 ? b1 : beta[c])) - s_mean[g] * a;
+  }
+  __syncthreads();
   for (int i = threadIdx.x; i < n4; i += 256) {
     const int r = i / C4;
     const int c = (i - r * C4) * 4;
-    float4 v = x4[i];
+    float4 v = i == (int)threadIdx.x ? vfirst : x4[i];
+    if (raw_sp) store_sp4(raw_sp, row0 + r, C, c, v.x, v.y, v.z, v.w);
     v.x = v.x * s_a[c] + s_b[c];
     v.y = v.y * s_a[c + 1] + s_b[c + 1];
     v.z = v.z * s_a[c + 2] + s_b[c + 2];
@@ -203,7 +208,7 @@
   }
 }
 
-__global__ __launch_bounds__(256) void gn_apply_stats_cols_kernel(const float* __restrict__ x, u16* __restrict__ y_sp,
+__global__ __launch_bounds__(256) void gn_apply_stats_cols_kernel(const float* __restrict__ x, u16* __restrict__ y_sp, u16* __restrict__ raw_sp,
                                                              const float* __restrict__ gamma, const float* __restrict__ beta,
                                                              const long long* __restrict__ stats, int HW, int C, int groups, int rows_per_block,
                                                              int TX, float eps, int silu) {
@@ -244,6 +249,7 @@
     float4 vn = make_float4(0.f, 0.f, 0.f, 0.f);
     if (r + TY < r_end) vn = *(xp + xstep);
     xp += xstep;
+    if (raw_sp) store_sp4(raw_sp, (size_t)b * HW + r, C, c, v.x, v.y, v.z, v.w);
     v.x = v.x * a[0] + bb[0];
     v.y = v.y * a[1] + bb[1];
     v.z = v.z * a[2] + bb[2];
@@ -396,9 +402,10 @@
   return 0;
 }
 
-extern "C" int mvd_groupnorm_from_stats(const float* x, void* y_sp, const float* gamma, const float* beta, const long long* stats, int B,
-                                        int HW, int C, int groups, float eps, int silu, mvd_stream_t stream) {
+extern "C" int mvd_groupnorm_from_stats_raw(const float* x, void* y_sp, void* raw_sp, const float* gamma, const float* beta,
+                                            const long long* stats, int B, int HW, int C, int groups, float eps, int silu, mvd_stream_t stream) {
   MVD_CHECK_ARG(x && y_sp && gamma && beta && stats, "mvd_groupnorm_from_stats: null pointer");
+  MVD_CHECK_ARG(((uintptr_t)raw_sp & 127) == 0, "mvd_groupnorm_from_stats: raw_sp must be 128-byte aligned");
   MVD_CHECK_ARG(C % 32 == 0 && B > 0 && HW > 0 && groups > 0 && groups <= 64 && C % groups == 0 && C <= GN_MAX_C,
                 "mvd_groupnorm_from_stats: bad shape (C=%d groups=%d)", C, groups);
   if (!(C <= 320 && HW >= 1024)) {
@@ -408,14 +415,19 @@
     const int TY = 256 / TX;
     const int rows_per_block = TY * 4;
     hipLaunchKernelGGL(gn_apply_stats_cols_kernel, dim3(cdiv(HW, rows_per_block), B, C4 / TX), dim3(256), 0, (hipStream_t)stream, x,
-                       (u16*)y_sp, gamma, beta, stats, HW, C, groups, rows_per_block, TX, eps, silu);
+                       (u16*)y_sp, (u16*)raw_sp, gamma, beta, stats, HW, C, groups, rows_per_block, TX, eps, silu);
   } else {
     const int chunks = gn_chunks(HW);
-    hipLaunchKernelGGL(gn_apply_stats_kernel, dim3(chunks, B), dim3(256), 0, (hipStream_t)stream, x, (u16*)y_sp, gamma, beta, stats, HW, C,
+    hipLaunchKernelGGL(gn_apply_stats_kernel, dim3(chunks, B), dim3(256), 0, (hipStream_t)stream, x, (u16*)y_sp, (u16*)raw_sp, gamma, beta, stats, HW, C,
                        groups, chunks, eps, silu);
   }
   MVD_CHECK_LAUNCH("mvd_groupnorm_from_stats");
   return 0;
+}
+
+extern "C" int mvd_groupnorm_from_stats(const float* x, void* y_sp, const float* gamma, const float* beta, const long long* stats, int B,
+                                        int HW, int C, int groups, float eps, int silu, mvd_stream_t stream) {
+  return mvd_groupnorm_from_stats_raw(x, y_sp, nullptr, gamma, beta, stats, B, HW, C, groups, eps, silu, stream);
 }
 
 extern "C" int mvd_softmax_rows(const float* x, void* y_sp, int rows, int cols, int ldx, float scale, float out_scale,
diff --git a/mvdfusion_amd/engine.py b/mvdfusion_amd/engine.py
--- a/mvdfusion_amd/engine.py
+++ b/mvdfusion_amd/engine.py
@@ -74,9 +74,12 @@
         self._unwritten = set()
         self.next_cat = None
         self._cat_done = set()
+        self.next_raw = None
+        self._raw = {}
+        self._arena_clean = True
         self.keep_fp32 = False
 
-    def begin_step(self):
+    def begin_step(self, zero_on_exit=False):
         self._rot.clear()
         self._gn.clear()
         self._gn_done.clear()
@@ -85,8 +88,31 @@
         self.next_gn = None
         self.next_cat = None
         self._gn_next = 0
-        if self.gn_from_producer:
+        self._raw.clear()
+        self.next_raw = None
+        if self.gn_from_producer and not (zero_on_exit and self._arena_clean):
             hip.check(hip.lib().mvd_fill_zero(hip.ptr(self.gn_arena), self.gn_arena.numel() * 2, hip.stream()))
+        self._arena_clean = False
+
+    def end_step(self, iter_counter=None):
+        if iter_counter is not None:
+            hip.check(hip.lib().mvd_advance_iter_zero(hip.ptr(iter_counter), hip.ptr(self.gn_arena) if self.gn_from_producer else None,
+                                                      self.gn_arena.numel() * 8, hip.stream()))
+        elif self.gn_from_producer:
+            hip.check(hip.lib().mvd_fill_zero(hip.ptr(self.gn_arena), self.gn_arena.numel() * 2, hip.stream()))
+        self._gn.clear()
+        self._arena_clean = bool(self.gn_from_producer)
+
+    def ensure_clean_arena(self):
+        if self.gn_from_producer and not self._arena_clean:
+            hip.check(hip.lib().mvd_fill_zero(hip.ptr(self.gn_arena), self.gn_arena.numel() * 2, hip.stream()))
+            self._arena_clean = True
+
+    def take_raw(self, x, C):
+        planes = self._raw.pop(x.data_ptr(), None)
+        if planes is not None and planes.shape == (x.shape[0], 2 * C) and x.shape[-1] == C:
+            return planes
+        return None
 
     def gn_slot(self, out, B, HW, C):
         n = B * 32 * 2
@@ -94,12 +120,14 @@
             return None
         st = self.gn_arena[self._gn_next * GN_SLOT_ELEMS:self._gn_next * GN_SLOT_ELEMS + n]
         self._gn_next += 1
+        self._arena_clean = False
         self._gn[out.data_ptr()] = (st, B, HW, C)
         return st
 
     def _forget(self, out):
         ptr = out.data_ptr()
         self._gn.pop(ptr, None)
+        self._raw.pop(ptr, None)
         self._unwritten.discard(ptr)
         if self._gn_done:
             for k in [k for k in self._gn_done if k[0] == ptr]:
@@ -166,6 +194,14 @@
                             planes = self.ws.planes(pname, out.shape[0], out.shape[-1])
                             kw["gn_apply"] = (norm.weight, norm.bias, norm.eps, hip.GNA_SILU if silu else 0, planes)
                             self._gn_done[(out.data_ptr(), id(norm))] = (planes, bool(silu))
+        if gn is not None and gn_apply is None and self.next_raw is not None and out is not None and "cat" not in kw and \
+                "out_planes" not in kw and out.is_contiguous() and out.shape[-1] % 32 == 0:
+            planes = self.ws.planes(self.next_raw, out.shape[0], out.shape[-1])
+            if "gn_apply" in kw:
+                kw["cat"] = (None, planes)
+            else:
+                kw["out_planes"] = planes
+            self._raw[out.data_ptr()] = planes
         if gn is not None:
             if os.environ.get("MVD_GN_DEBUG") and not self.capturing:
                 print(f"[gn] kind={kind} M={out.shape[0]} N={out.shape[-1]} explicit={gn_apply is not None} hint={self.next_gn is not None} "
@@ -173,6 +209,7 @@
             if gn_apply is None:
                 self.next_gn = None
                 self.next_cat = None
+                self.next_raw = None
         r = hip.gemm(A, W, out, **kw)
         if gn_apply is not None and not applied:
             self.groupnorm(out, gn_apply[1], gn_apply[0], gn[0], gn[1], out.shape[-1], gn_apply[2])
diff --git a/mvdfusion_amd/hip.py b/mvdfusion_amd/hip.py
--- a/mvdfusion_amd/hip.py
+++ b/mvdfusion_amd/hip.py
@@ -127,6 +127,7 @@
     "mvd_pixel_cross_attn_backward": (_i, [_vp, _vp, _vp, _vp, _i, _i, _i, _i, _vp, _vp, _vp, _vp]),
     "mvd_groupnorm_backward": (_i, [_vp, _vp, _vp, _vp, _i, _i, _i, _i, _f, _i, _vp, _vp, _vp, _vp, _sz, _vp]),
     "mvd_groupnorm_from_stats": (_i, [_vp, _vp, _vp, _vp, _vp, _i, _i, _i, _i, _f, _i, _vp]),
+    "mvd_groupnorm_from_stats_raw": (_i, [_vp, _vp, _vp, _vp, _vp, _vp, _i, _i, _i, _i, _f, _i, _vp]),
     "mvd_area_pool": (_i, [_vp, _vp, _i, _i, _i, _i, _i, _i, _vp]),
     "mvd_fill_zero": (_i, [_vp, _sz, _vp]),
     "mvd_pow2_scale": (_i, [_vp, _sz, _vp, _vp, _vp]),
@@ -136,6 +137,7 @@
     "mvd_timestep_embedding": (_i, [_vp, _vp, _vp, _vp, _i, _vp]),
     "mvd_timestep_embedding_scenes": (_i, [_vp, _vp, _vp, _vp, _i, _i, _i, _vp]),
     "mvd_advance_iter": (_i, [_vp, _vp]),
+    "mvd_advance_iter_zero": (_i, [_vp, _vp, _sz, _vp]),
     "mvd_zembed": (_i, [_vp, _vp, _vp, _vp, _i, _i, _vp]),
     "mvd_gridattn_tokens": (_i, [_vp] * 10 + [_i, _i, _i, _i, _i, _f, _f, _vp]),
     "mvd_gridattn_tokens_scenes": (_i, [_vp] * 10 + [_i, _i, _i, _i, _i, _i, _f, _f, _vp]),
@@ -587,12 +589,15 @@
         d.gn_stats, d.gn_hw, d.gn_groups = gn_stats.data_ptr(), int(gn_hw), int(gn_groups)
     if gn_apply is not None:
         gamma, beta, eps, flags, planes = gn_apply
-        ct = d.N + (cat[0].shape[-1] if cat is not None else 0)
+        ct = d.N + (cat[0].shape[-1] if cat is not None and cat[0] is not None else 0)
         assert gn_stats is not None and out is not None and planes.dtype == torch.int16 and planes.shape[-1] == 2 * ct
         if cat is not None:
             skip, raw = cat
-            assert skip.dtype == torch.float32 and skip.is_contiguous() and skip.shape[0] == d.M and (raw is None or raw.shape[-1] == 2 * ct)
-            d.cat_b, d.cat_cb, d.cat_raw_sp = skip.data_ptr(), int(skip.shape[-1]), (raw.data_ptr() if raw is not None else None)
+            assert raw is None or (raw.dtype == torch.int16 and raw.shape[-1] == 2 * ct)
+            if skip is not None:
+                assert skip.dtype == torch.float32 and skip.is_contiguous() and skip.shape[0] == d.M
+                d.cat_b, d.cat_cb = skip.data_ptr(), int(skip.shape[-1])
+            d.cat_raw_sp = raw.data_ptr() if raw is not None else None
         d.gna_gamma, d.gna_beta, d.gna_eps, d.gna_flags, d.gna_out_sp = gamma.data_ptr(), beta.data_ptr(), float(eps), int(flags), planes.data_ptr()
     if row_stats is not None:
         assert row_stats.slots.shape[0] >= d.M and row_stats.ld >= (d.N + 31) // 32
@@ -607,10 +612,12 @@
         d.workspace = workspace.data_ptr()
         d.workspace_elems = workspace.numel()
     key = (d.M, d.N, d.K, d.a_mode, d.Cin, d.stride, d.upsample, d.no_pad_tl, d.epi, d.prec, res is not None, out is not None,
-           out_planes is not None, splitk, d.b_mode, row_stats is not None, ln is not None, gn_apply is not None, cat[0].shape[-1] if cat is not None else 0,
+           out_planes is not None, splitk, d.b_mode, row_stats is not None, ln is not None, gn_apply is not None, cat[0].shape[-1] if cat is not None and cat[0] is not None else 0,
            d.tap_mode, d.Cin2)
     if cfg is None:
         tuned = _TUNED.get(key)
+        if tuned is None and out_planes is not None and out is not None:
+            tuned = _TUNED.get(key[:12] + (False,) + key[13:])
         if tuned is None and AUTOTUNE and 2.0 * d.M * d.N * d.K >= AUTOTUNE_MIN_FLOPS:
             tuned = _autotune(d, A if A.is_contiguous() else None, W_data=W.data if not isinstance(W, PlanesOperand) else None)
             _TUNED[key] = tuned
@@ -933,8 +940,9 @@
     return y
 
 
-def groupnorm_from_stats(x, y, gamma, beta, stats, B, HW, Cc, eps, silu, groups=32):
-    check(lib().mvd_groupnorm_from_stats(ptr(x), ptr(y), ptr(gamma), ptr(beta), ptr(stats), B, HW, Cc, groups, eps, int(silu), stream()))
+def groupnorm_from_stats(x, y, gamma, beta, stats, B, HW, Cc, eps, silu, groups=32, raw=None):
+    check(lib().mvd_groupnorm_from_stats_raw(ptr(x), ptr(y), ptr(raw), ptr(gamma), ptr(beta), ptr(stats), B, HW, Cc, groups, eps, int(silu),
+                                             stream()))
     return y
 
 
diff --git a/mvdfusion_amd/unet.py b/mvdfusion_amd/unet.py
--- a/mvdfusion_amd/unet.py
+++ b/mvdfusion_amd/unet.py
@@ -27,7 +27,7 @@
         self.conv = nn.Conv2d(self.channels, self.out_channels, 3, padding=padding)
         self._p = self._p4 = None
 
-    def run(self, ctx, x, H, W, out=None):
+    def run(self, ctx, x, H, W, out=None, x_planes=None):
         if hip.use_up4(ctx.B, H, W, training=ctx.keep_fp32):
             if self._p4 is None:
                 self._p4 = hip.pack_conv3x3_up4(self.conv.weight, self.conv.bias)
@@ -38,7 +38,7 @@
             wp = self._p
         if out is None:
             out = ctx.act((ctx.B * 4 * H * W, self.out_channels))
-        xp = hip.split_planes(x, ctx.ws.planes("updown.x", ctx.B * H * W, self.channels))
+        xp = x_planes if x_planes is not None else hip.split_planes(x, ctx.ws.planes("updown.x", ctx.B * H * W, self.channels))
         ctx.gemm(xp, wp, out, conv=dict(B=ctx.B, Hin=H, Win=W, Cin=self.channels, Hout=2 * H, Wout=2 * W,
                                             stride=1, upsample=1), gn=(ctx.B, 4 * H * W), kind="conv")
         return out, 2 * H, 2 * W
@@ -51,13 +51,13 @@
         self.op = nn.Conv2d(self.channels, self.out_channels, 3, stride=2, padding=padding)
         self._p = None
 
-    def run(self, ctx, x, H, W, out=None):
+    def run(self, ctx, x, H, W, out=None, x_planes=None):
         if self._p is None:
             self._p = hip.pack_conv3x3(self.op.weight, self.op.bias)
         Ho, Wo = H // 2, W // 2
         if out is None:
             out = ctx.act((ctx.B * Ho * Wo, self.out_channels))
-        xp = hip.split_planes(x, ctx.ws.planes("updown.x", ctx.B * H * W, self.channels))
+        xp = x_planes if x_planes is not None else hip.split_planes(x, ctx.ws.planes("updown.x", ctx.B * H * W, self.channels))
         ctx.gemm(xp, self._p, out, conv=dict(B=ctx.B, Hin=H, Win=W, Cin=self.channels, Hout=Ho, Wout=Wo, stride=2,
                                             upsample=0), gn=(ctx.B, Ho * Wo), kind="conv")
         return out, Ho, Wo
@@ -131,21 +131,32 @@
     return None
 
 
+def raw_hint(layer):
+    if isinstance(layer, (Upsample, Downsample)):
+        return "updown.x"
+    if isinstance(layer, ResBlock) and not isinstance(layer.skip_connection, nn.Identity):
+        return "res.xp"
+    return None
+
+
 class TimestepEmbedSequential(nn.Sequential, TimestepBlock):
     def run(self, ctx, x, H, W, out=None, x_planes=None, next_layer=None, next_cat=None):
         n = len(self)
         for i, layer in enumerate(self):
             dst = out if i == n - 1 else None
+            xp = x_planes if i == 0 else ctx.take_raw(x, x.shape[-1])
             ctx.next_gn = gn_hint(self[i + 1] if i + 1 < n else next_layer)
+            ctx.next_raw = raw_hint(self[i + 1] if i + 1 < n else next_layer)
             ctx.next_cat = next_cat if i == n - 1 else None
             if isinstance(layer, (Upsample, Downsample)):
-                x, H, W = layer.run(ctx, x, H, W, out=dst)
+                x, H, W = layer.run(ctx, x, H, W, out=dst, x_planes=xp)
             elif isinstance(layer, ResBlock):
-                x = layer.run(ctx, x, H, W, out=dst, x_planes=x_planes if i == 0 else None)
+                x = layer.run(ctx, x, H, W, out=dst, x_planes=xp)
             else:
                 x = layer.run(ctx, x, H, W, out=dst)
             ctx.next_gn = None
             ctx.next_cat = None
+            ctx.next_raw = None
         return x, H, W
 
 
@@ -301,7 +312,7 @@
                 co = last.out_channels if isinstance(last, (ResBlock, Downsample)) else last.in_channels
                 o = ctx.ws.get(f"hs{bi}", (B * Ho * Wo, co))
                 nxt = self.input_blocks[bi + 1][0] if bi + 1 < len(self.input_blocks) else self.middle_block[0]
-                h, H, W = blk.run(ctx, h, H, W, out=o, next_layer=nxt)
+                h, H, W = blk.run(ctx, h, H, W, out=o, next_layer=nxt, x_planes=ctx.take_raw(h, h.shape[-1]))
             hs.append((h, H, W))
         if rec is not None:
             rec.append((self.middle_block, h.clone(), H, W, 0))
diff --git a/mvdfusion_amd/viewfusion_zero_depth_rgb.py b/mvdfusion_amd/viewfusion_zero_depth_rgb.py
--- a/mvdfusion_amd/viewfusion_zero_depth_rgb.py
+++ b/mvdfusion_amd/viewfusion_zero_depth_rgb.py
@@ -155,7 +155,7 @@
         V, S, D, B, q0, Vq, N = self.V, self.S, self.D, self.B, self.q0, self.Vq, self.N
         NVq = N * Vq
         ctx.B, ctx.D = B, D
-        ctx.begin_step()
+        ctx.begin_step(zero_on_exit=bool(do_update))
         st = hip.stream
         sst, R = self.steps_scene_stride, self.t_rows
         if sst and do_update:
@@ -208,7 +208,7 @@
                                         hip.ptr(self.ddim_noise[:, q0:q0 + NVq]), N * V * 5 * S * S, hip.ptr(self.steps),
                                         hip.ptr(self.iter), NVq, S, int(self.cfg), float(cfg_scale), int(do_update), st()))
         if do_update:
-            hip.check(L.mvd_advance_iter(hip.ptr(self.iter), st()))
+            ctx.end_step(self.iter)
 
     @property
     def t_rows(self):
@@ -259,7 +259,9 @@
                 self.ctx.ws.frozen = False
             self.graphs[key] = g
             self.prefetchers[key] = pf
+        self.ctx.ensure_clean_arena()
         g.launch()
+        self.ctx._arena_clean = bool(self.ctx.gn_from_producer)
 
 
 class _HipTrainingLoss(torch.autograd.Function):
```
